# ut-amrl/nautilus

Measured on AMD Instinct MI355X. Metric: loop-closure candidate pairs/sec (1081-beam), higher is better.
Workload: dtype u16

## Files before the change

### include/nautilus_hip.h

```cpp
#ifndef NAUTILUS_HIP_H_
#define NAUTILUS_HIP_H_

#include <stddef.h>
#include <stdint.h>

#ifdef __cplusplus
extern "C" {
#endif

#define NHIP_OK 0
#define NHIP_ERR_ARG (-1)
#define NHIP_ERR_NODEV (-2)
#define NHIP_ERR_HIP (-3)
#define NHIP_ERR_ALLOC (-4)
#define NHIP_ERR_STATE (-5)

int nhip_init(int *n_devices);
int nhip_set_device(int device);
const char *nhip_last_error(void);
const char *nhip_version(void);
int nhip_dev_status(void *stream, int32_t info[4]);

typedef struct nhip_grid_spec {
  double range;
// ... 437 lines not shown
                      double max_range, int32_t min_separation, uint8_t *flags );
int nhip_lc_chi_square_gate(const double *poses, int32_t n_poses, const int32_t *pair_src, const int32_t *pair_tgt,
                            const float *cov , int32_t n_pairs, double max_score,
                            double *scores , uint8_t *flags );

int nhip_features_extract(const nhip_scans_t *scans, const nhip_feature_spec_t *spec, int32_t *planar_idx,
                          int32_t *planar_count, int32_t *edge_idx, int32_t *edge_count, double *scores);

int nhip_normals_estimate(const nhip_scans_t *scans, const nhip_normals_spec_t *spec, float *normals, int32_t *info);

int nhip_vectorize(const nhip_scans_t *scans, const double *poses, const nhip_vectorize_spec_t *spec, int32_t max_cells,
                   int32_t max_rounds, int32_t check_every, int64_t *records, int32_t *stats);

int nhip_occupancy(const nhip_scans_t *scans, const double *poses, const nhip_occupancy_spec_t *spec, int32_t *hits,
                   int32_t *misses, int8_t *grid, int64_t *stats);

int nhip_transient_filter(const nhip_scans_t *scans, const double *poses, const nhip_transient_spec_t *spec, const int32_t *hits,
                          const int32_t *misses, uint8_t *labels, float *out_xy, int32_t *out_offsets, int32_t *out_index,
                          int64_t *stats);

int nhip_map_windows(const int8_t *grid, const nhip_mapwin_spec_t *spec, const int32_t *origins, int32_t n_queries, float *out_xy,
                     int64_t capacity, int32_t *out_offsets, int64_t *stats);

int nhip_csm_freespace(const nhip_scans_t *scans, const nhip_grids_t *grids, const int32_t *pair_src, const int32_t *pair_slot,
                       const double *theta0, const int32_t *pair_origin, int32_t n_pairs, const nhip_search_t *search,
                       const nhip_match_t *matches, const nhip_freespace_spec_t *fs_spec, int32_t *counts);

int nhip_place_candidates(const nhip_scans_t *scans, const int32_t *ids, int32_t n_ids, const nhip_place_spec_t *spec,
                          int32_t *records, int64_t *stats, uint64_t *desc, int32_t *bits);

int nhip_place_seq_candidates(const nhip_scans_t *scans, const int32_t *ids, int32_t n_ids, const nhip_place_spec_t *spec,
                              const nhip_place_seq_spec_t *seq, int32_t *records, int64_t *stats);

int nhip_consistency(const double *records, int32_t M, const nhip_consistency_spec_t *spec, int32_t *members, int32_t *n_members,
                     int64_t *stats);

typedef struct nhip_csm_params {
  double scanner_range;
  double trans_range;
  double low_res;
  double high_res;
  double sigma;
  double floor_p;
  int32_t cell_bits;
  int32_t reserved;
} nhip_csm_params_t;
int nhip_csm_cache_configure(int64_t max_bytes);
int nhip_csm_cache_clear(void);
int nhip_csm_cache_stats(int64_t *entries, int64_t *bytes, int64_t *hits, int64_t *misses);
int nhip_csm_get_transformation(const nhip_csm_params_t *params, const float *pc_a, int32_t n_a, const float *pc_b,
                                int32_t n_b, double rot_a, double rot_b, double rot_restriction, double *score,
                                float *tx, float *ty, float *theta);

int nhip_resid_batch_create(int kind, const float *corr, const int32_t *block_offsets,
                            const int32_t *block_src, const int32_t *block_tgt, int32_t n_blocks,
                            int32_t n_poses, nhip_resid_batch_t **out);
int nhip_resid_batch_eval(nhip_resid_batch_t *batch, const double *poses, double *residuals,
                          double *jac_src, double *jac_tgt);
int nhip_resid_batch_eval_compact(nhip_resid_batch_t *batch, const double *poses, double *residuals,
                                  double *jac_src, double *jac_tgt_theta);
int nhip_resid_batch_eval_q(nhip_resid_batch_t *batch, const double *poses, double *residuals, double *q, double *block_consts);
int nhip_resid_jacobians_from_q(int kind, const float *corr, const double *q, const double *block_consts, int64_t n,
                                double *jac_src, double *jac_tgt);
int nhip_resid_batch_eval_block(nhip_resid_batch_t *batch, int32_t block, const double *source_pose,
                                const double *target_pose, double *residuals, double *jac_src, double *jac_tgt);
int nhip_resid_batch_free(nhip_resid_batch_t *batch);

int nhip_host_alloc(size_t bytes, void **out);
int nhip_host_free(void *p);

int nhip_resid_odometry(const float *t_odom, const float *r_odom, const int32_t *pose_i,
                        const int32_t *pose_j, int32_t n_factors, double translation_weight,
                        double rotation_weight, const double *poses, int32_t n_poses,
                        double *residuals, double *jac_i, double *jac_j);
int nhip_resid_point_to_line(const float *segments, const float *points, const int32_t *point_block,
                             int64_t n_points, const int32_t *block_pose, const int32_t *block_line,
                             int32_t n_blocks, const double *poses, int32_t n_poses,
                             const double *line_poses, int32_t n_line_poses, double *residuals,
                             double *jac_pose, double *jac_line);

int nhip_allgather_matches(void *comm, const nhip_match_t *d_local, int32_t n_local,
                           nhip_match_t *d_all, void *stream);

#ifdef __cplusplus
}
#endif
#endif
```

### nautilus_amd/_lib.py

```python
import ctypes as C
import os

_HERE = os.path.dirname(os.path.abspath(__file__))
LIB_PATH = os.environ.get("NHIP_LIB") or os.path.join(_HERE, "lib", "libnautilus_hip.so")

NHIP_OK, NHIP_ERR_ARG, NHIP_ERR_NODEV, NHIP_ERR_HIP, NHIP_ERR_ALLOC, NHIP_ERR_STATE = 0, -1, -2, -3, -4, -5
NHIP_LIDAR_NORMAL, NHIP_LIDAR_POINT = 0, 1
NHIP_SEARCH_EXHAUSTIVE, NHIP_SEARCH_DENSE, NHIP_SEARCH_SHORT_SCANS, NHIP_SEARCH_EXACT_SCORE, NHIP_SEARCH_LATENCY = 1, 2, 4, 8, 16
NHIP_SHORT_SCAN_POINTS = 1088
NHIP_FEATURE_MAX = 64
NHIP_NORMALS_MAX_BINS, NHIP_NORMALS_MAX_SAMPLES = 64, 128
NHIP_GRID_SKIP_MAP, NHIP_GRID_NO_IMAGE = 1, 2
NHIP_TIMER_CSM, NHIP_TIMER_GRID, NHIP_TIMER_RESID, NHIP_TIMER_CORR, NHIP_TIMER_NORMEQ, NHIP_TIMER_GRID_CLEAR = 0, 1, 2, 3, 4, 5
NHIP_TIMER_CSM_BOUNDS, NHIP_TIMER_CSM_CAND, NHIP_TIMER_EXACT_SCORE = 6, 7, 8
NHIP_TIMER_VEC_RASTER, NHIP_TIMER_VEC_VOTES, NHIP_TIMER_VEC_ROUNDS = 9, 10, 11
NHIP_TIMER_OCC_TRACE, NHIP_TIMER_OCC_CLASSIFY = 12, 13
NHIP_OCC_ACCUMULATE = 1
NHIP_PLACE_PAST_ONLY = 1
NHIP_PLACE_WORKSPACE_MAX = 64 << 20
NHIP_CONSISTENCY_STATE_BYTES = 8448
NHIP_LOSS_NONE, NHIP_LOSS_HUBER, NHIP_LOSS_SOFT_L1, NHIP_LOSS_CAUCHY = 0, 1, 2, 3


class NhipError(RuntimeError):
# ... 64 lines not shown
                ("reserved", C.c_int32)]


class MapwinSpec(C.Structure):
    _fields_ = [("res", C.c_double), ("cell_x0", C.c_int32), ("cell_y0", C.c_int32), ("width", C.c_int32), ("height", C.c_int32),
                ("side", C.c_int32), ("occ_min", C.c_int32), ("flags", C.c_int32), ("reserved", C.c_int32)]


class FreespaceSpec(C.Structure):
    _fields_ = [("hit_radius", C.c_int32), ("end_margin", C.c_int32), ("flags", C.c_int32), ("reserved", C.c_int32)]


class PlaceSpec(C.Structure):
    _fields_ = [("n_rings", C.c_int32), ("range_max", C.c_float), ("top_k", C.c_int32), ("min_separation", C.c_int32),
                ("max_permille", C.c_int32), ("flags", C.c_int32)]


class PlaceSeqSpec(C.Structure):
    _fields_ = [("half_window", C.c_int32), ("step", C.c_int32)]


class ConsistencySpec(C.Structure):
    _fields_ = [("t0", C.c_double), ("t_rate", C.c_double), ("t_max", C.c_double), ("r0", C.c_double), ("r_rate", C.c_double),
                ("r_max", C.c_double), ("max_steps", C.c_int32), ("flags", C.c_int32)]


class LossSpec(C.Structure):
    _fields_ = [("kind", C.c_int32), ("flags", C.c_int32), ("scale", C.c_double)]


class HitlSpec(C.Structure):
    _fields_ = [("line_a", C.c_float * 4), ("line_b", C.c_float * 4), ("line_width", C.c_double),
                ("point_threshold", C.c_int32), ("reserved", C.c_int32)]


class PcgStats(C.Structure):
    _fields_ = [("iterations", C.c_int32), ("flag", C.c_int32), ("relative_residual", C.c_double)]


class Match(C.Structure):
    _fields_ = [("itheta", C.c_int32), ("ix", C.c_int32), ("iy", C.c_int32), ("score", C.c_float)]


_vp, _i32, _i64, _f64 = C.c_void_p, C.c_int32, C.c_int64, C.c_double
_P = C.POINTER

PROTOTYPES = {
    "nhip_init": (C.c_int, [_P(C.c_int)]),
    "nhip_set_device": (C.c_int, [C.c_int]),
    "nhip_last_error": (C.c_char_p, []),
    "nhip_version": (C.c_char_p, []),
    "nhip_grid_layout": (C.c_int, [_P(GridSpec), _P(GridLayout)]),
    "nhip_grids_bytes": (_i64, [_P(GridSpec), _i64]),
    "nhip_grid_workspace_bytes": (_i64, [_P(GridSpec), _i32]),
    "nhip_grid_tables": (C.c_int, [_P(GridSpec), _vp, _vp]),
    "nhip_csm_rot0": (C.c_int, [_vp, _vp, _i32, _vp]),
    "nhip_csm_delta_table": (C.c_int, [_P(Search), _vp]),
    "nhip_match_to_transform": (C.c_int, [_P(Match), _P(GridSpec), _P(Search), _f64, _i32, _i32,
                                          _P(C.c_float), _P(C.c_float), _P(C.c_float)]),
    "nhip_score_from_sum": (_f64, [_P(GridSpec), _i64, _i32]),
    "nhip_csm_gate_floor": (C.c_int, [_P(GridSpec), _f64, _i32, _P(_i32)]),
    "nhip_dev_status": (C.c_int, [_vp, _P(_i32)]),
    "nhip_host_phases": (C.c_int, [_P(_f64)]),
    "nhip_device_pool_configure": (C.c_int, [_i64]),
    "nhip_device_pool_release": (C.c_int, []),
    "nhip_device_pool_stats": (C.c_int, [_P(_i64), _P(_i64)]),
    "nhip_grid_build_dev": (C.c_int, [_vp, _vp, _i32, _vp, _i32, _P(GridSpec), _vp, _vp, _i64, _vp]),
    "nhip_grid_rebuild_dev": (C.c_int, [_vp, _vp, _i32, _vp, _i32, _P(GridSpec), _vp, _vp, _i64, _vp]),
    "nhip_csm_match_dev": (C.c_int, [_vp, _vp, _i32, _vp, _i32, _P(GridSpec), _vp, _vp, _vp, _vp, _vp, _i32,
                                     _P(Search), _vp, _vp, _vp, _vp, _i64, _vp]),
    "nhip_csm_match_gated_dev": (C.c_int, [_vp, _vp, _i32, _vp, _i32, _P(GridSpec), _vp, _vp, _vp, _vp, _vp, _i32,
                                           _P(Search), _vp, _vp, _vp, _vp, _i64, _vp, _f64]),
    "nhip_submap_member_affines": (C.c_int, [_vp, _i32, _vp, _vp, _i32, _vp]),
    "nhip_submaps_gather_dev": (C.c_int, [_vp, _vp, _i32, _vp, _vp, _vp, _i32, _vp, _i64, _vp, _vp]),
    "nhip_grids_build_submaps": (C.c_int, [_vp, _vp, _vp, _vp, _i32, _P(GridSpec), _P(_vp)]),
    "nhip_csm_workspace_bytes": (_i64, [_i32]),
    "nhip_csm_last_launch": (C.c_int, [_P(_i32)]),
    "nhip_csm_get_transformation_info": (C.c_int, [_vp]),
    "nhip_bnb_stats": (C.c_int, [_P(C.c_uint64), _P(C.c_uint64)]),
    "nhip_bnb_stats_per_pair": (C.c_int, [_vp, _i32]),
    "nhip_bnb_timeline": (C.c_int, [_vp, _i32]),
    "nhip_bnb_timeline_candidates": (C.c_int, [_vp, _i32]),
    "nhip_bnb_stats_levels": (C.c_int, [_P(C.c_uint64)]),
    "nhip_csm_scores_dev": (C.c_int, [_vp, _vp, _i32, _vp, _i32, _P(GridSpec), _i32, _i32, _vp, _vp, _i32, _i32,
                                      _P(Search), _vp, _vp]),
    "nhip_resid_lidar_dev": (C.c_int, [C.c_int, _vp, _vp, _i64, _vp, _vp, _i32, _vp, _i32, _vp,
                                       _vp, _vp, _vp, _vp]),
    "nhip_resid_lidar_normal_eq_dev": (C.c_int, [C.c_int, _vp, _vp, _vp, _vp, _i32, _vp, _i32, _vp, _vp, _vp]),
    "nhip_pose_affines": (C.c_int, [_vp, _i32, _vp]),
    "nhip_corr_search_dev": (C.c_int, [_vp, _vp, _vp, _i32, _vp, _vp, _i32, _vp, C.c_float, _vp, _vp, _vp, _vp]),
    "nhip_corr_search_normals_dev": (C.c_int, [_vp, _vp, _vp, _i32, _vp, _vp, _i32, _vp, C.c_float, C.c_float, _vp, _vp, _vp,
                                               _vp]),
    "nhip_corr_compact_dev": (C.c_int, [_vp, _vp, _vp, _i32, _vp, _vp, _vp, _vp]),
    "nhip_resid_point_to_line_dev": (C.c_int, [_vp, _vp, _vp, _i64, _vp, _vp, _i32, _vp, _i32, _vp, _i32,
                                               _vp, _vp, _vp, _vp]),
    "nhip_resid_point_to_line_normal_eq_dev": (C.c_int, [_vp, _vp, _vp, _vp, _vp, _i32, _vp, _i32, _vp, _i32, _vp, _vp]),
    "nhip_resid_odometry_dev": (C.c_int, [_vp, _vp, _vp, _vp, _i32, _f64, _f64, _vp, _i32, _vp, _vp,
                                          _vp, _vp]),
    "nhip_resid_odometry_normal_eq_dev": (C.c_int, [_vp, _vp, _vp, _vp, _i32, _f64, _f64, _vp, _i32, _vp, _vp]),
    "nhip_resid_odometry_robust_normal_eq_dev": (C.c_int, [_vp, _vp, _vp, _vp, _i32, _f64, _f64, _P(LossSpec), _vp, _i32, _vp, _vp,
                                                           _vp]),
    "nhip_bsr_assemble_dev": (C.c_int, [_vp, _i32, _vp, _vp, _vp, _vp, _i32, _i32, _i32, _vp, _vp, _vp, _vp]),
    "nhip_bsr_pcg_workspace_bytes": (_i64, [_i32, _i32]),
    "nhip_bsr_pcg_dev": (C.c_int, [_vp, _vp, _vp, _vp, _vp, _i32, _i32, _f64, _f64, _f64, _i32, _i32, _vp, _vp, _i64,
                                   _P(PcgStats), _vp]),
    "nhip_bsr_pcg_columns_workspace_bytes": (_i64, [_i32, _i32, _i32]),
    "nhip_bsr_pcg_columns_dev": (C.c_int, [_vp, _vp, _vp, _vp, _i32, _i32, _vp, _vp, _i32, _f64, _f64, _i32, _i32, _vp, _vp, _i64,
                                           _P(PcgStats), _vp]),
    "nhip_scans_upload": (C.c_int, [_vp, _vp, _i32, _P(_vp)]),
    "nhip_scans_free": (C.c_int, [_vp]),
    "nhip_grids_build": (C.c_int, [_vp, _vp, _i32, _P(GridSpec), _P(_vp)]),
    "nhip_grids_free": (C.c_int, [_vp]),
    "nhip_grids_was_rebuilt": (C.c_int, [_vp]),
    "nhip_grids_download": (C.c_int, [_vp, _i32, _vp]),
    "nhip_grids_download_skip_map": (C.c_int, [_vp, _i32, _vp]),
    "nhip_grids_download_hi_plane": (C.c_int, [_vp, _i32, _vp]),
    "nhip_grids_download_hi_plane_copy": (C.c_int, [_vp, _i32, _i32, _vp]),
    "nhip_grids_download_tiled16": (C.c_int, [_vp, _i32, _vp]),
    "nhip_grids_download_pool": (C.c_int, [_vp, _i32, _vp]),
    "nhip_grids_download_pool4": (C.c_int, [_vp, _i32, _vp]),
    "nhip_grids_download_hits": (C.c_int, [_vp, _i32, _vp]),
    "nhip_csm_match": (C.c_int, [_vp, _vp, _vp, _vp, _vp, _vp, _i32, _P(Search), _vp, _vp]),
    "nhip_csm_match_gated": (C.c_int, [_vp, _vp, _vp, _vp, _vp, _vp, _i32, _P(Search), _vp, _vp, _f64]),
    "nhip_csm_scores": (C.c_int, [_vp, _vp, _i32, _i32, _f64, _i32, _i32, _P(Search), _vp]),
    "nhip_lc_scatter_scores_dev": (C.c_int, [_vp, _vp, _i32, _vp, _vp]),
    "nhip_lc_pair_gate_dev": (C.c_int, [_vp, _i32, _vp, _i32, _f64, _i32, _vp, _vp]),
    "nhip_lc_chi_square_gate_dev": (C.c_int, [_vp, _i32, _vp, _vp, _vp, _i32, _f64, _vp, _vp, _vp]),
    "nhip_feature_spec_default": (C.c_int, [_P(FeatureSpec)]),
    "nhip_features_extract_dev": (C.c_int, [_vp, _vp, _i32, _P(FeatureSpec), _vp, _vp, _vp, _vp, _vp, _vp]),
    "nhip_features_pack_dev": (C.c_int, [_vp, _vp, _vp, _i32, _vp, _vp, _i32, _vp, _vp, _vp, _vp]),
    "nhip_normals_spec_default": (C.c_int, [_P(NormalsSpec)]),
    "nhip_normals_estimate_dev": (C.c_int, [_vp, _vp, _i32, _P(NormalsSpec), _vp, _vp, _vp]),
    "nhip_normals_estimate": (C.c_int, [_vp, _P(NormalsSpec), _vp, _vp]),
    "nhip_vectorize_spec_default": (C.c_int, [_P(VectorizeSpec)]),
    "nhip_vectorize_tables": (C.c_int, [_P(VectorizeSpec), _vp, _vp]),
    "nhip_map_pose_affines": (C.c_int, [_vp, _i32, _vp]),
    "nhip_vectorize_workspace_bytes": (_i64, [_P(VectorizeSpec), _i32]),
    "nhip_vectorize_workspace_layout": (C.c_int, [_P(VectorizeSpec), _i32, _P(VectorizeLayout)]),
    "nhip_vectorize_dev": (C.c_int, [_vp, _vp, _vp, _i32, _P(VectorizeSpec), _i32, _i32, _i32, _vp, _vp, _vp, _i64, _vp]),
    "nhip_vectorize": (C.c_int, [_vp, _vp, _P(VectorizeSpec), _i32, _i32, _i32, _vp, _vp]),
    "nhip_vectorize_endpoints": (C.c_int, [_P(VectorizeSpec), _vp, _i32, _vp]),
    "nhip_occupancy_spec_default": (C.c_int, [_P(OccupancySpec)]),
    "nhip_occupancy_dev": (C.c_int, [_vp, _vp, _vp, _i32, _P(OccupancySpec), _vp, _vp, _vp, _vp, _vp]),
    "nhip_occupancy": (C.c_int, [_vp, _vp, _P(OccupancySpec), _vp, _vp, _vp, _vp]),
    "nhip_transient_spec_default": (C.c_int, [_P(TransientSpec)]),
    "nhip_transient_filter_dev": (C.c_int, [_vp, _vp, _i32, _i32, _vp, _P(TransientSpec), _vp, _vp, _vp, _vp, _vp, _vp, _vp, _vp]),
    "nhip_transient_filter": (C.c_int, [_vp, _vp, _P(TransientSpec), _vp, _vp, _vp, _vp, _vp, _vp, _vp]),
    "nhip_mapwin_spec_default": (C.c_int, [_P(MapwinSpec)]),
    "nhip_mapwin_origins": (C.c_int, [_vp, _i32, _f64, _vp, _vp]),
    "nhip_mapwin_workspace_bytes": (_i64, [_i32]),
    "nhip_mapwin_cells_dev": (C.c_int, [_vp, _P(MapwinSpec), _i32, _vp, _vp, _vp, _vp]),
    "nhip_mapwin_gather_dev": (C.c_int, [_vp, _vp, _P(MapwinSpec), _vp, _i32, _vp, _i64, _vp, _vp, _vp, _i64, _vp]),
    "nhip_map_windows": (C.c_int, [_vp, _P(MapwinSpec), _vp, _i32, _vp, _i64, _vp, _vp]),
    "nhip_freespace_spec_default": (C.c_int, [_P(FreespaceSpec)]),
    "nhip_freespace_planes_bytes": (_i64, [_P(GridSpec), _i64]),
    "nhip_freespace_trace_dev": (C.c_int, [_vp, _vp, _i32, _vp, _i32, _P(GridSpec), _vp, _vp, _vp]),
    "nhip_freespace_check_dev": (C.c_int, [_vp, _vp, _i32, _vp, _i32, _P(GridSpec), _vp, _vp, _vp, _vp, _vp, _i32, _P(Search),
                                           _vp, _vp, _P(FreespaceSpec), _vp, _vp]),
    "nhip_csm_freespace": (C.c_int, [_vp, _vp, _vp, _vp, _vp, _vp, _i32, _P(Search), _vp, _P(FreespaceSpec), _vp]),
    "nhip_place_spec_default": (C.c_int, [_P(PlaceSpec)]),
    "nhip_place_tables": (C.c_int, [_P(PlaceSpec), _vp, _vp]),
    "nhip_place_workspace_bytes": (_i64, [_P(PlaceSpec), _i32]),
    "nhip_place_describe_dev": (C.c_int, [_vp, _vp, _i32, _P(PlaceSpec), _vp, _vp, _vp]),
    "nhip_place_match_dev": (C.c_int, [_vp, _vp, _i32, _vp, _i32, _P(PlaceSpec), _vp, _vp, _vp, _i64, _vp]),
    "nhip_place_candidates": (C.c_int, [_vp, _vp, _i32, _P(PlaceSpec), _vp, _vp, _vp, _vp]),
    "nhip_place_seq_spec_default": (C.c_int, [_P(PlaceSeqSpec)]),
# ... 77 lines not shown
```

### nautilus_amd/csm.py

```python
import ctypes as C
import math

import numpy as np

from . import _lib
from ._lib import GridSpec, GridLayout, Search, Match, check, ptr

MATCH_DTYPE = np.dtype([("itheta", "<i4"), ("ix", "<i4"), ("iy", "<i4"), ("score", "<f4")])
assert MATCH_DTYPE.itemsize == C.sizeof(Match) == 16


def grid_spec(range_m=30.0, res=0.05, sigma=2.0, floor_p=1e-10, max_shift=40, cell_bits=16, skip_map=False, no_image=False):
    return GridSpec(float(range_m), float(res), float(sigma), float(floor_p), int(max_shift), int(cell_bits),
                    (_lib.NHIP_GRID_SKIP_MAP if skip_map else 0) | (_lib.NHIP_GRID_NO_IMAGE if no_image else 0), 0)


def search_spec(n_theta=61, nx=81, ny=81, theta_step=math.radians(1.0), exhaustive=False, dense=False, short_scans=False,
                exact_score=False, latency=False):
    flags = (_lib.NHIP_SEARCH_EXHAUSTIVE if exhaustive else 0) | (_lib.NHIP_SEARCH_DENSE if dense else 0) | \
            (_lib.NHIP_SEARCH_SHORT_SCANS if short_scans else 0) | (_lib.NHIP_SEARCH_EXACT_SCORE if exact_score else 0) | \
            (_lib.NHIP_SEARCH_LATENCY if latency else 0)
    return Search(int(n_theta), int(nx), int(ny), flags, float(theta_step))


# ... 118 lines not shown
            check(_lib.load().nhip_grids_download_pool4(self._h, int(slot), ptr(out)))
        return out

    def hits(self, slot):
        L = self.layout
        raw = np.empty(L.hits_bytes, dtype=np.uint8)
        check(_lib.load().nhip_grids_download_hits(self._h, int(slot), ptr(raw)))
        rows = raw[:L.hits_pitch * (L.side + 64)].reshape(L.side + 64, L.hits_pitch)
        bits = np.unpackbits(rows, axis=1, bitorder="little")
        return bits[32:32 + L.side, 32:32 + L.side]

    def interior(self, slot):
        L = self.layout
        return self.download(slot)[L.pad:L.pad + L.side, L.pad:L.pad + L.side]

    def close(self):
        if self._h:
            _lib.load().nhip_grids_free(self._h)
            self._h = C.c_void_p()

    __del__ = close


def submap_member_affines(poses, anchor_of_member, member_scan):
    P = np.ascontiguousarray(poses, dtype=np.float64).reshape(-1, 3)
    a = np.ascontiguousarray(anchor_of_member, dtype=np.int32)
    m = np.ascontiguousarray(member_scan, dtype=np.int32)
    if a.size != m.size:
        raise ValueError("submap_member_affines: one anchor per member")
    out = np.empty((m.size, 4), dtype=np.float32)
    check(_lib.load().nhip_submap_member_affines(ptr(P), len(P), ptr(a), ptr(m), m.size, ptr(out)))
    return out


def match_pairs(scans, grids, pair_src, pair_slot, theta0, search, pair_origin=None, min_score=None):
    pair_src = np.ascontiguousarray(pair_src, dtype=np.int32)
    pair_slot = np.ascontiguousarray(pair_slot, dtype=np.int32)
    theta0 = np.ascontiguousarray(theta0, dtype=np.float64)
    n = pair_src.size
    if pair_slot.size != n or theta0.size != n:
        raise ValueError("pair arrays differ in length")
    org = None
    if pair_origin is not None:
        org = np.ascontiguousarray(pair_origin, dtype=np.int32).reshape(n, 2)
    out = np.zeros(n, dtype=MATCH_DTYPE)
    sums = np.zeros(n, dtype=np.int32)
    if min_score is None:
        check(_lib.load().nhip_csm_match(scans._h, grids._h, ptr(pair_src), ptr(pair_slot), ptr(theta0),
                                         ptr(org), n, C.byref(search), ptr(out), ptr(sums)))
    else:
        check(_lib.load().nhip_csm_match_gated(scans._h, grids._h, ptr(pair_src), ptr(pair_slot), ptr(theta0),
                                               ptr(org), n, C.byref(search), ptr(out), ptr(sums), float(min_score)))
    return out, sums


def rejected(matches):
    return np.asarray(matches)["itheta"] < 0


def gate_floor(spec, min_score, n_points):
    out = C.c_int32(0)
    check(_lib.load().nhip_csm_gate_floor(C.byref(spec), float(min_score), int(n_points), C.byref(out)))
    return out.value


def bnb_stats():
    a, b = C.c_uint64(0), C.c_uint64(0)
    check(_lib.load().nhip_bnb_stats(C.byref(a), C.byref(b)))
    return a.value, b.value


def bnb_stats_levels():
    v = (C.c_uint64 * 24)()
    check(_lib.load().nhip_bnb_stats_levels(v))
    return {"blocks_whole": v[0], "blocks_total": v[1], "candidates_refined": v[2], "sub_blocks": v[3],
            "clk_wave_phase3": v[4], "clk_origins": v[5], "clk_sub_bounds": v[6], "clk_exact": v[7],
            "clk_slowest_wave": v[8], "clk_seeds": v[9], "clk_bounds": v[10], "clk_wave_phase3_100MHz": v[11],
            "pairs_handed_over": v[12], "clk_wave_second_kernel": v[13], "pose_evals16": v[14],
            "pairs_settled_by_gate": v[15], "passes_l2_runs": v[16], "passes_per_cell_field": v[17],
            "passes_per_cell_capacity": v[18], "edge_blocks_refined": v[19], "sub_blocks_without_pose": v[20],
            "edge_blocks_whole": v[21], "pair_passes": v[22], "pair_passes_across_blocks": v[23]}


def score_volume(scans, grids, src, slot, theta0, search, origin=(0, 0)):
    out = np.zeros((search.n_theta, search.nx, search.ny), dtype=np.int32)
    check(_lib.load().nhip_csm_scores(scans._h, grids._h, int(src), int(slot), float(theta0),
                                      int(origin[0]), int(origin[1]), C.byref(search), ptr(out)))
    return out


def match_to_transform(m, spec, search, theta0, origin=(0, 0)):
    tx = (origin[0] + int(m["ix"]) - (search.nx - 1) // 2) * spec.res
    ty = (origin[1] + int(m["iy"]) - (search.ny - 1) // 2) * spec.res
    th = theta0 + (int(m["itheta"]) - (search.n_theta - 1) // 2) * search.theta_step
    return np.float32(tx), np.float32(ty), np.float32(th)


class CorrelativeScanMatcher:

    def __init__(self, scanner_range, trans_range, low_res, high_res, sigma=2.0, cell_bits=16):
        self.params = _lib.CsmParams(float(scanner_range), float(trans_range), float(low_res), float(high_res),
                                     float(sigma), 1e-10, int(cell_bits), 0)

    def GetTransformation(self, pointcloud_a, pointcloud_b, rotation_a, rotation_b, rotation_restriction):
        a = np.ascontiguousarray(pointcloud_a, dtype=np.float32).reshape(-1, 2)
        b = np.ascontiguousarray(pointcloud_b, dtype=np.float32).reshape(-1, 2)
        score, tx, ty, th = C.c_double(0), C.c_float(0), C.c_float(0), C.c_float(0)
        check(_lib.load().nhip_csm_get_transformation(C.byref(self.params), ptr(a), len(a), ptr(b), len(b),
                                                      float(rotation_a), float(rotation_b), float(rotation_restriction),
                                                      C.byref(score), C.byref(tx), C.byref(ty), C.byref(th)))
        return score.value, ((np.float32(tx.value), np.float32(ty.value)), np.float32(th.value))


def last_launch():
    out = (C.c_int32 * 8)()
    check(_lib.load().nhip_csm_last_launch(out))
    form = {0: "fused", 1: "split, one round", 2: "split, rounds on one stream", 3: "split, rounds overlapped on the helper stream"}
    return {"form": form.get(out[0], "?"), "form_id": out[0], "pairs_per_round": out[1], "rounds_of_state": out[2],
            "rounds": out[3], "short_scans": bool(out[4]), "hand_over_kernel": bool(out[5]), "instrumented": bool(out[6] & 1),
            "l2_runs": bool(out[6] & 2), "pair_subs": bool(out[6] & 4), "n_pairs": out[7]}


def drop_in_cache_stats():
    v = [C.c_int64(0) for _ in range(4)]
    check(_lib.load().nhip_csm_cache_stats(*[C.byref(x) for x in v]))
    return dict(zip(("entries", "bytes", "hits", "misses"), (x.value for x in v)))


def drop_in_cache_clear():
    check(_lib.load().nhip_csm_cache_clear())


def drop_in_cache_configure(max_bytes):
    check(_lib.load().nhip_csm_cache_configure(int(max_bytes)))
```

### nautilus_amd/csrc/nhip_bnb.hip

```cpp
#include <atomic>
#include <mutex>
#include <type_traits>
#include <vector>

#ifndef NHIP_BNB_INSTR
#define NHIP_BNB_INSTR 0
#endif
#if NHIP_BNB_INSTR
#define csm_bnb_kernel csm_bnb_kernel_instr
#define csm_bnb_rot_kernel csm_bnb_rot_kernel_instr
#define launchers_product launchers_instr
#define BNB_STATS(P) ((P).stats)
#define BNB_TIMELINE(P) ((P).timeline)
#else
#define BNB_STATS(P) (static_cast<unsigned long long *>(nullptr))
#define BNB_TIMELINE(P) (static_cast<unsigned long long *>(nullptr))
#endif

#include "nhip_bnb_params.h"
#include "nhip_bnb_wave.h"
#include "nhip_bnb_origin.h"
#include "nhip_bnb_bounds.h"
#include "nhip_bnb_exact.h"

namespace nhip {

namespace {

using namespace bnb;

constexpr int BNB_THREADS = 64 * BNB_WAVES;

constexpr int N_WORK = 9;
struct PairCtx {
  const uint8_t *grid;
  const float2 *pts;
  int32_t n_pts, cx, cy, pair;
};

template <int CB>
__device__ __forceinline__ void process_candidate(const BnbParams &P, const PairCtx &C, int32_t k, int32_t v, int lane,
                                                  unsigned long long *best, uint32_t (&n)[N_WORK]) {
  const int Y = v / NB, X = v - NB * Y;
  const int32_t vx = block_extent(P.nx, X), vy = block_extent(P.ny, Y);
  const bool edge = vx < BNB_B || vy < BNB_B;
  float cf, sf;
  rotation_k(P, C.pair, k, &cf, &sf);
  if (P.levels >= 2) {
    const __amdgpu_buffer_rsrc_t p4 = uniform_rsrc(C.grid + P.grid_bytes + P.skip_bytes + P.pool_bytes, P.pool4_bytes);
    uint32_t sb[4];
    sub_bounds(P, p4, C.pts, C.n_pts, cf, sf, C.cx, C.cy, Y, X, lane, CB == 1 ? 1u : 257u, sb);
    n[1]++;
    n[4] += edge ? 1u : 0u;
    const uint32_t bsum = best_sum<false>(best);
    int alive = 0;
#pragma unroll
    for (int q = 0; q < 4; q++) alive += (sub_valid(vy, vx, q >> 1, q & 1) && sb[q] != 0u && sb[q] >= bsum) ? 1 : 0;
    if (alive == 0) return;
    if (alive <= 2) {
      const __amdgpu_buffer_rsrc_t rsrc = uniform_rsrc(C.grid, P.grid_bytes + P.skip_bytes);
#pragma unroll 1
      for (int q = 0; q < 4; q++) {
        const uint32_t b = q == 0 ? sb[0] : (q == 1 ? sb[1] : (q == 2 ? sb[2] : sb[3]));
        if (!sub_valid(vy, vx, q >> 1, q & 1) || b == 0u || b < best_sum<false>(best)) continue;
        const unsigned long long key = eval_sub<CB>(P, rsrc, C.pts, C.n_pts, cf, sf, C.cx, C.cy, k, Y, X, q >> 1, q & 1, lane);
        wave_atomic_max(best, key, lane);
        n[2]++;
        n[5] += sub_valid(vy, vx, q >> 1, q & 1) ? 0u : 1u;
      }
      return;
    }
  }
  const unsigned long long key = eval_block<CB>(P, C.grid, C.pts, C.n_pts, cf, sf, C.cx, C.cy, k, Y, X, lane);
  wave_atomic_max(best, key, lane);
  n[0]++;
  n[6] += edge ? 1u : 0u;
}

template <int CB, bool GLOBAL, bool PAIR>
__device__ __forceinline__ void process_candidate_c(const BnbParams &P, __amdgpu_buffer_rsrc_t rsrc, uint32_t pitch8,
                                                    __amdgpu_buffer_rsrc_t rsrc16, const uint32_t *org, int32_t nch,
                                                    int32_t n_pts, int32_t k, int32_t Y, int32_t X,
                                                    uint32_t sb0, uint32_t sb1, uint32_t sb2, uint32_t sb3, int lane,
                                                    unsigned long long *best, uint32_t &bcopy, uint32_t (&n)[N_WORK],
                                                    int t, uint32_t &mk0, uint32_t &mk1) {
  const uint32_t bsum = best_sum_cached<GLOBAL>(best, bcopy);
  const int32_t vx = block_extent(P.nx, X), vy = block_extent(P.ny, Y);
  const bool edge = vx < BNB_B || vy < BNB_B;
  n[4] += edge ? 1u : 0u;
  const bool ok0 = sub_valid(vy, vx, 0, 0), ok1 = sub_valid(vy, vx, 0, 1), ok2 = sub_valid(vy, vx, 1, 0), ok3 = sub_valid(vy, vx, 1, 1);
  const int alive = (ok0 && sb0 != 0u && sb0 >= bsum) + (ok1 && sb1 != 0u && sb1 >= bsum) + (ok2 && sb2 != 0u && sb2 >= bsum) +
                    (ok3 && sb3 != 0u && sb3 >= bsum);
  if (alive == 0) return;
  constexpr int WHOLE_MIN = 3;
  if (alive >= WHOLE_MIN) {
    int dy, dx;
    const uint32_t total = block_sums8(rsrc, pitch8, (uint32_t)P.hi_copy_bytes, org, nch, Y, X, lane, &dy, &dx);
    const int32_t ix = BNB_B * X + dx, iy = BNB_B * Y + dy;
    if (CB == 1) {
      const unsigned long long key = best_key(P, k, ix, iy, total, 32);
      wave_atomic_max(best, key, lane);
      if (GLOBAL) bcopy = max(bcopy, (uint32_t)(key >> 32));
    } else {
      n[3] += refine16<GLOBAL>(P, rsrc16, org, nch, n_pts, k, ix, iy, total, true, lane, best, bcopy);
    }
    n[0]++;
    n[6] += __ballot(ix < P.nx && iy < P.ny) != ~0ull ? 1u : 0u;
    return;
  }
  if (!PAIR) {
#pragma unroll 1
    for (int q = 0; q < 4; q++) {
      const uint32_t b = q == 0 ? sb0 : (q == 1 ? sb1 : (q == 2 ? sb2 : sb3));
      if (!sub_valid(vy, vx, q >> 1, q & 1) || b == 0u || b < best_sum_cached<GLOBAL>(best, bcopy)) continue;
      int dy, dx;
      const uint32_t total = sub_sums8(rsrc, pitch8, (uint32_t)P.hi_copy_bytes, org, nch, Y, X, q >> 1, q & 1, lane, &dy, &dx);
      const int32_t ix = BNB_B * X + BNB_B4 * (q & 1) + dx, iy = BNB_B * Y + BNB_B4 * (q >> 1) + dy;
      if (CB == 1) {
        const unsigned long long key = best_key(P, k, ix, iy, total, 8);
        wave_atomic_max(best, key, lane);
        if (GLOBAL) bcopy = max(bcopy, (uint32_t)(key >> 32));
      } else {
        n[3] += refine16<GLOBAL>(P, rsrc16, org, nch, n_pts, k, ix, iy, total, lane < 16, lane, best, bcopy);
      }
      n[2]++;
      n[5] += __ballot(ix < P.nx && iy < P.ny) == 0ull ? 1u : 0u;
    }
    return;
  }
  mk0 |= (uint32_t)((ok0 && sb0 != 0u && sb0 >= bsum) | ((ok1 && sb1 != 0u && sb1 >= bsum) << 1)) << (2 * t);
  mk1 |= (uint32_t)((ok2 && sb2 != 0u && sb2 >= bsum) | ((ok3 && sb3 != 0u && sb3 >= bsum) << 1)) << (2 * t);
}

#ifndef NHIP_BNB_PAIR_CROSS
#define NHIP_BNB_PAIR_CROSS 0
#endif
constexpr bool PAIR_CROSS = NHIP_BNB_PAIR_CROSS != 0;
__device__ __forceinline__ uint32_t pick6(const uint32_t (&r)[6], int c) {
  return c == 0 ? r[0] : (c == 1 ? r[1] : (c == 2 ? r[2] : (c == 3 ? r[3] : (c == 4 ? r[4] : r[5]))));
}
template <int CB, bool GLOBAL>
__device__ __forceinline__ void strip_sub_blocks(const BnbParams &P, __amdgpu_buffer_rsrc_t rsrc, uint32_t pitch8,
                                                 __amdgpu_buffer_rsrc_t rsrc16, const uint32_t *org, int32_t nch, int32_t n_pts,
                                                 int32_t k, int32_t Y, int32_t X0, const uint32_t (&sb)[12], uint32_t mk0,
                                                 uint32_t mk1, int lane, unsigned long long *best, uint32_t &bcopy,
                                                 uint32_t (&n)[N_WORK]) {
#pragma unroll 1
  for (int sy = 0; sy < 2; sy++) {
    uint32_t mk = sy ? mk1 : mk0;
    if (mk == 0u) continue;
    uint32_t row[6];
#pragma unroll
    for (int c = 0; c < 6; c++) row[c] = sy ? sb[4 * (c >> 1) + 2 + (c & 1)] : sb[4 * (c >> 1) + (c & 1)];
#pragma unroll 1
    while (mk != 0u) {
      const int c = (int)__builtin_ctz(mk);
      mk &= mk - 1u;
      const uint32_t bsum = best_sum_cached<GLOBAL>(best, bcopy);
      if (pick6(row, c) < bsum) continue;
      const int32_t X = X0 + (c >> 1), sx = c & 1;
      const bool two = P.pair_subs != 0 && ((mk >> (c + 1)) & 1u) != 0u && (PAIR_CROSS || sx == 0) && pick6(row, c + 1) >= bsum;
      int dy, dx;
      uint32_t total;
      if (two) {
        mk &= ~(1u << (c + 1));
        total = pair_sums8(rsrc, pitch8, (uint32_t)P.hi_copy_bytes, org, nch, Y, X, sy, sx, lane, &dy, &dx);
      } else {
        total = sub_sums8(rsrc, pitch8, (uint32_t)P.hi_copy_bytes, org, nch, Y, X, sy, sx, lane, &dy, &dx);
      }
      const int32_t ix = BNB_B * X + BNB_B4 * sx + dx, iy = BNB_B * Y + BNB_B4 * sy + dy;
      if (CB == 1) {
        const unsigned long long key = best_key(P, k, ix, iy, total, 16);
        wave_atomic_max(best, key, lane);
        if (GLOBAL) bcopy = max(bcopy, (uint32_t)(key >> 32));
      } else {
        n[3] += refine16<GLOBAL>(P, rsrc16, org, nch, n_pts, k, ix, iy, total, lane < (two ? 32 : 16), lane, best, bcopy);
      }
      const bool pose = ix < P.nx && iy < P.ny;
      if (two) {
        n[2] += 2u;
        n[5] += (__ballot(pose && dx < BNB_B4) == 0ull ? 1u : 0u) + (__ballot(pose && dx >= BNB_B4) == 0ull ? 1u : 0u);
        n[7]++;
        n[8] += (uint32_t)sx;
      } else {
        n[2]++;
        n[5] += __ballot(pose) == 0ull ? 1u : 0u;
      }
    }
  }
}

struct PhaseClocks {
  long long org, strip, eval;
  uint32_t run_passes, cell_passes_field, cell_passes_full;
};

__device__ __forceinline__ void flush_stats(unsigned long long *stats, const uint32_t *n, int32_t pair, const PhaseClocks *clk,
                                            const uint32_t *edge = nullptr) {
  if (n) {
    if (n[0]) atomicAdd(&stats[0], (unsigned long long)n[0]);
    if (n[1]) atomicAdd(&stats[2], (unsigned long long)n[1]);
    if (n[2]) atomicAdd(&stats[3], (unsigned long long)n[2]);
    if (n[3]) atomicAdd(&stats[14], (unsigned long long)n[3]);
    if (pair < BNB_STATS_PAIRS) atomicAdd(&stats[BNB_STATS_HEAD + pair], 4ull * n[0] + n[2]);
  }
  if (edge) {
    if (edge[0]) atomicAdd(&stats[19], (unsigned long long)edge[0]);
    if (edge[1]) atomicAdd(&stats[20], (unsigned long long)edge[1]);
    if (edge[2]) atomicAdd(&stats[21], (unsigned long long)edge[2]);
    if (edge[3]) atomicAdd(&stats[22], (unsigned long long)edge[3]);
    if (edge[4]) atomicAdd(&stats[23], (unsigned long long)edge[4]);
  }
  if (clk) {
    atomicAdd(&stats[5], (unsigned long long)clk->org);
    atomicAdd(&stats[6], (unsigned long long)clk->strip);
    atomicAdd(&stats[7], (unsigned long long)clk->eval);
    if (clk->run_passes) atomicAdd(&stats[16], (unsigned long long)clk->run_passes);
    if (clk->cell_passes_field) atomicAdd(&stats[17], (unsigned long long)clk->cell_passes_field);
    if (clk->cell_passes_full) atomicAdd(&stats[18], (unsigned long long)clk->cell_passes_full);
  }
}

template <int CB, bool GLOBAL, bool PAIR, bool RUNS = false>
__device__ __forceinline__ void rotation_pass(const BnbParams &P, const PairCtx &C, int32_t k, uint32_t u0, uint32_t u1,
                                              unsigned long long m0, unsigned long long m1, int lane,
                                              unsigned long long *best, uint32_t *done, uint32_t *org,
                                              uint32_t (&n_work)[N_WORK], PhaseClocks &clk, uint32_t *runs = nullptr) {
  long long t_mark = 0;
  float cf, sf;
  rotation_k(P, C.pair, k, &cf, &sf);
  if (BNB_STATS(P)) t_mark = clock64();
  int32_t nrc = RUNS_NONE;
  const int32_t nch = cache_origins<RUNS>(P, C.pts, C.n_pts, cf, sf, C.cx, C.cy, lane, org, true, runs, RUNS && P.l2_runs != 0, &nrc);
  if (BNB_STATS(P)) clk.org += clock64() - t_mark;
  if (RUNS && BNB_STATS(P)) {
    clk.run_passes += nrc > 0 ? 1u : 0u;
    clk.cell_passes_field += nrc == RUNS_FIELD ? 1u : 0u;
    clk.cell_passes_full += nrc == RUNS_FULL ? 1u : 0u;
  }
  const __amdgpu_buffer_rsrc_t rsrc16 = CB == 1 ? uniform_rsrc(C.grid, P.grid_bytes + P.skip_bytes)
                                                : uniform_rsrc(C.grid + P.hi_offset + 2 * P.hi_copy_bytes, P.t16_bytes);
  const __amdgpu_buffer_rsrc_t rsrc = uniform_rsrc(C.grid + P.hi_offset, 2 * P.hi_copy_bytes);
  const uint32_t pitch8 = (uint32_t)P.hi_tpr;
  const __amdgpu_buffer_rsrc_t p4 = uniform_rsrc(C.grid + P.grid_bytes + P.skip_bytes + P.pool_bytes, P.pool4_bytes);
  while ((m0 | m1) != 0ull) {
    const int b0 = m0 ? (int)__builtin_ctzll(m0) : 64 + (int)__builtin_ctzll(m1);
    const int Y = b0 / NB, X0 = b0 - NB * Y;
    int len = 1;
    while (len < 3 && X0 + len < NB) {
      const int b = b0 + len;
      if (!(((b < 64 ? m0 >> b : m1 >> (b - 64)) & 1ull))) break;
      len++;
    }
    uint32_t sb[12];
    uint32_t bcopy = GLOBAL ? best_sum<true>(best) : 0u;
    if (P.levels >= 2) {
      if (BNB_STATS(P)) t_mark = clock64();
      if (RUNS && nrc > 0) strip_bounds_c<RunList<RUN_CHUNKS>>(P, p4, runs + lane, nrc, Y, X0, len, CB == 1 ? 1u : 257u, sb);
      else strip_bounds_c<CellList>(P, p4, org, nch, Y, X0, len, CB == 1 ? 1u : 257u, sb);
      if (BNB_STATS(P)) clk.strip += clock64() - t_mark;
      n_work[1] += (uint32_t)len;
    } else {
#pragma unroll
      for (int q = 0; q < 12; q++) sb[q] = 0xffffffffu;
    }
    uint32_t mk0 = 0u, mk1 = 0u;
#pragma unroll 1
    for (int t = 0; t < len; t++) {
      const int b = b0 + t;
      if (b < 64) m0 &= ~(1ull << b);
      else m1 &= ~(1ull << (b - 64));
      const uint32_t ub = (uint32_t)__builtin_amdgcn_readlane((int)(b < 64 ? u0 : u1), b & 63);
      if (ub < best_sum_cached<GLOBAL>(best, bcopy)) continue;
      const uint32_t s0 = t == 0 ? sb[0] : (t == 1 ? sb[4] : sb[8]), s1 = t == 0 ? sb[1] : (t == 1 ? sb[5] : sb[9]);
      const uint32_t s2 = t == 0 ? sb[2] : (t == 1 ? sb[6] : sb[10]), s3 = t == 0 ? sb[3] : (t == 1 ? sb[7] : sb[11]);
      if (BNB_STATS(P)) t_mark = clock64();
      process_candidate_c<CB, GLOBAL, PAIR>(P, rsrc, pitch8, rsrc16, org, nch, C.n_pts, k, Y, X0 + t, s0, s1, s2, s3, lane, best,
                                      bcopy, n_work, t, mk0, mk1);
      if (BNB_STATS(P)) clk.eval += clock64() - t_mark;
      if (done && wave_leader(lane)) done[b] = 0u;
    }
    if (PAIR && (mk0 | mk1) != 0u) {
      if (BNB_STATS(P)) t_mark = clock64();
      strip_sub_blocks<CB, GLOBAL>(P, rsrc, pitch8, rsrc16, org, nch, C.n_pts, k, Y, X0, sb, mk0, mk1, lane, best, bcopy, n_work);
      if (BNB_STATS(P)) clk.eval += clock64() - t_mark;
    }
  }
}

__device__ __forceinline__ void read_entry(const RotEntry *ent, int32_t *pair, int32_t *k, unsigned long long *m0,
                                           unsigned long long *m1) {
  const unsigned long long w0 = ent->w[0], w1 = ent->w[1], w2 = ent->w[2], w3 = ent->w[3];
  *pair = (int32_t)(w0 >> 24);
  *k = (int32_t)(w0 & 0xffffffull);
  *m0 = w1 | (w2 << 41);
  *m1 = (w2 >> 23) | (w3 << 18);
}

__device__ __forceinline__ void pair_context(const BnbParams &P, int32_t pair, PairCtx *C) {
  const int32_t src = P.pair_src[pair], slot = P.pair_slot[pair];
  const int32_t beg = P.offsets[src];
  C->grid = P.grids + (size_t)slot * P.slot_bytes;
  C->pts = P.xy + beg;
  C->n_pts = P.offsets[src + 1] - beg;
  C->cx = P.pair_origin ? P.pair_origin[2 * pair] : 0;
  C->cy = P.pair_origin ? P.pair_origin[2 * pair + 1] : 0;
  C->pair = pair;
}

template <int CB, bool POOL_LDS, bool BY_ROT, bool SPLIT = false>
__global__ __launch_bounds__(SPLIT ? 64 * SPLIT_WAVES : BNB_THREADS, SPLIT ? SPLIT_WAVES / 2 : 4) void csm_bnb_kernel(BnbParams P) {
  constexpr int WAVES = SPLIT ? SPLIT_WAVES : BNB_WAVES, THREADS = 64 * WAVES;
  constexpr int QSPACE = lds_qspace(SPLIT);
  extern __shared__ __align__(16) uint8_t smem[];
  uint8_t *s_pool = smem;
  uint32_t *s_org = reinterpret_cast<uint32_t *>(smem);
  uint32_t *s_U = reinterpret_cast<uint32_t *>(smem + P.lds_first);
  unsigned long long *s_queue = reinterpret_cast<unsigned long long *>(s_U + (size_t)P.n_theta * 128);
  LdsTail *s_tail = reinterpret_cast<LdsTail *>(s_queue + QSPACE);
  unsigned long long *s_best = &s_tail->best, *s_slow = &s_tail->slow;
  uint32_t *s_cnt = s_tail->cnt, *s_qn = s_cnt + LDS_QN, *s_qhead = s_cnt + LDS_QHEAD, *s_top = &s_tail->top;
  uint32_t *s_list = reinterpret_cast<uint32_t *>(s_queue);
  static_assert(BNB_WAVES * LIST_ENTRIES * 4 <= QCAP * 4, "the run lists fit the first half of the queue");
  unsigned long long *s_kmax = s_queue + (SPLIT ? WAVES * LIST_ENTRIES / 2 : QCAP / 2);
  uint32_t *s_order = reinterpret_cast<uint32_t *>(s_kmax + MAX_ROT);
  static_assert(SPLIT_WAVES * LIST_ENTRIES * 4 + MAX_ROT * 12 <= QSPACE_SPLIT * 8 && MAX_ROT * 12 <= QCAP * 4, "lists, maxima and order fit");

  const uint32_t bid = blockIdx.x;
  const int32_t pair = (int32_t)((bid & 7u) * (uint32_t)P.pairs_per_xcd + (bid >> 3));
  if ((int32_t)(bid >> 3) >= P.pairs_per_xcd || pair >= P.n_pairs) return;
  const int lane = threadIdx.x & 63, wave = threadIdx.x >> 6;

  int32_t src = P.pair_src[pair], slot = P.pair_slot[pair];
  const bool ids_ok = pair_ids_ok(P.ids, src, slot, pair + P.pair_base, threadIdx.x == 0);
  if (!ids_ok) src = slot = 0;
  const int32_t beg = ids_ok ? P.offsets[src] : 0, n_pts = ids_ok ? P.offsets[src + 1] - beg : 0;
  const float2 *pts = P.xy + beg;
  const uint8_t *grid = P.grids + (size_t)slot * P.slot_bytes;
  const int32_t cx = P.pair_origin ? P.pair_origin[2 * pair] : 0;
  const int32_t cy = P.pair_origin ? P.pair_origin[2 * pair + 1] : 0;
  const bool centre_ok = (abs(cx) + P.hx <= P.max_shift) && (abs(cy) + P.hy <= P.max_shift);
  if (BY_ROT != (n_pts <= 64 * OCL && (uint32_t)P.rows < ORG_LIMIT && !P.general_all)) return;

  const int32_t gfloor = gate_floor(P.gate, n_pts);
  const unsigned long long fkey = gate_floor_key(gfloor);
  unsigned long long *const stats_g = NHIP_BNB_INSTR ? P.stats : nullptr;
  const long long t_start = BNB_STATS(P) ? clock64() : 0;
  if (BNB_TIMELINE(P) && threadIdx.x == 0 && pair < BNB_STATS_PAIRS) BNB_TIMELINE(P)[4 * pair] = wall_clock64();
  if (threadIdx.x == 0) {
    *s_slow = 0ull;
    *s_best = fkey;
    s_cnt[0] = s_cnt[3] = s_cnt[4] = s_cnt[5] = 0u;
    s_top[0] = 0u;
    *s_qn = 0u;
    *s_qhead = 0u;
  }
  if (!centre_ok || n_pts <= 0) {
    if (threadIdx.x == 0) P.keys[pair] = fkey;
    return;
  }
  const RotationTerms terms = rotation_terms_of_wave<WAVES>(P, pair, wave, lane);
  if (POOL_LDS) {
    const uint4 *gp = reinterpret_cast<const uint4 *>(grid + P.grid_bytes + P.skip_bytes);
    uint4 *sp = reinterpret_cast<uint4 *>(s_pool);
    const int32_t n16 = (int32_t)(P.pool_bytes / 16);
    for (int32_t i = threadIdx.x; i < n16; i += 4 * THREADS) {
      uint4 v[4];
// ... 187 lines not shown
      const int32_t k = (int32_t)((uint32_t)wbest >> 8), v = (int32_t)(wbest & 0xffu);
      const int Y = v / NB, X = v - NB * Y;
      float cf, sf;
      rotation_k(P, pair, k, &cf, &sf);
      const unsigned long long key = eval_block<CB>(P, grid, pts, n_pts, cf, sf, cx, cy, k, Y, X, lane);
      if (wave_leader(lane)) {
        atomicMax(s_best, key);
        s_U[k * 128 + v] = 0u;
      }
      n_work[0]++;
    }
    __syncthreads();
    for (int32_t k = wave; k < P.n_theta; k += BNB_WAVES) {
  #pragma unroll
      for (int i = 0; i < 2; i++) {
        const uint32_t u = s_U[k * 128 + lane + 64 * i];
        const uint32_t bsum = (uint32_t)(*(volatile unsigned long long *)s_best >> 32);
        bool cand = u != 0u && u >= bsum;
        const unsigned long long m = __ballot(cand);
        if (m == 0ull) continue;
        const uint32_t base = wave_fetch_add(s_qn, (uint32_t)__builtin_popcountll(m), lane);
        const uint32_t pos = base + (uint32_t)__builtin_popcountll(m & ((1ull << lane) - 1ull));
        const unsigned long long entry = ((unsigned long long)u << 32) | (uint32_t)((k << 8) | (lane + 64 * i));
        if (cand && pos < (uint32_t)QCAP) s_queue[pos] = entry;
        unsigned long long over = __ballot(cand && pos >= (uint32_t)QCAP);
        while (over) {
          const int j = (int)__builtin_ctzll(over);
          over &= over - 1ull;
          const uint32_t lo = (uint32_t)__builtin_amdgcn_readlane((int)(uint32_t)entry, j);
          const uint32_t hi = (uint32_t)__builtin_amdgcn_readlane((int)(uint32_t)(entry >> 32), j);
          if (hi >= best_sum<false>(s_best))
            process_candidate<CB>(P, C, (int32_t)(lo >> 8), (int32_t)(lo & 0xffu), lane, s_best, n_work);
        }
      }
    }
    __syncthreads();
    {
      const uint32_t qn = min(*s_qn, (uint32_t)QCAP);
      for (;;) {
        const uint32_t i = wave_fetch_add(s_qhead, 1u, lane);
        if (i >= qn) break;
        const unsigned long long entry = s_queue[i];
        if ((uint32_t)(entry >> 32) >= best_sum<false>(s_best))
          process_candidate<CB>(P, C, (int32_t)((uint32_t)entry >> 8), (int32_t)(entry & 0xffu), lane, s_best, n_work);
      }
    }
}
  if (stats_g && lane == 0) {
    atomicAdd(&s_cnt[0], n_work[0]);
    atomicAdd(&s_cnt[3], n_work[1]);
    atomicAdd(&s_cnt[4], n_work[2]);
    atomicAdd(&s_cnt[5], n_work[3]);
    flush_stats(stats_g, nullptr, pair, nullptr, n_work + 4);
  }
  __syncthreads();
  if (threadIdx.x == 0) {
    P.keys[pair] = *s_best;
    if (BNB_TIMELINE(P) && pair < BNB_STATS_PAIRS) {
      uint32_t hw;
      asm volatile("s_getreg_b32 %0, hwreg(HW_REG_HW_ID)" : "=s"(hw));
      uint32_t xcc;
      asm volatile("s_getreg_b32 %0, hwreg(HW_REG_XCC_ID)" : "=s"(xcc));
      BNB_TIMELINE(P)[4 * pair + 3] = (wall_clock64() & 0xfffffffffffull) | ((unsigned long long)((hw >> 8) & 0xffu) << 44) |
                                      ((unsigned long long)(xcc & 0xfu) << 52);
    }
    if (BNB_STATS(P) && BY_ROT) atomicAdd(&BNB_STATS(P)[8], *s_slow);
    if (stats_g) {
      const uint32_t n_all[4] = {s_cnt[0], s_cnt[3], s_cnt[4], s_cnt[5]};
      flush_stats(stats_g, n_all, pair, nullptr);
      atomicAdd(&stats_g[1], (unsigned long long)(P.n_theta * P.nbx * P.nby));
    }
  }
}

template <int CB>
__global__ __launch_bounds__(256, CB == 2 && !NHIP_BNB_INSTR ? 5 : 4) void csm_bnb_rot_kernel(BnbParams P) {
  const int lane = threadIdx.x & 63;
  const uint32_t xcd = blockIdx.x & 7u;
  const uint32_t filled = P.rot_count[8 * xcd];
  const uint32_t count = filled < P.rot_cap ? filled : P.rot_cap;
  const RotEntry *list = P.rot_list + (size_t)xcd * P.rot_cap;
  __shared__ uint32_t s_org2[4 * ORG_WAVE];
  __shared__ uint32_t s_run2[4 * RUN_WAVE];
  uint32_t *org = s_org2 + (threadIdx.x >> 6) * ORG_WAVE + lane;
  uint32_t *runs = s_run2 + (threadIdx.x >> 6) * RUN_WAVE;
  PhaseClocks clk = {0, 0, 0, 0u, 0u, 0u};
  const long long t0 = BNB_STATS(P) ? clock64() : 0;
  for (;;) {
    const uint32_t i = wave_fetch_add(P.rot_count + 8 * xcd + 1, 1u, lane);
    if (i >= count) break;
    int32_t pair, k;
    unsigned long long m0, m1;
    read_entry(list + i, &pair, &k, &m0, &m1);
    PairCtx C;
    pair_context(P, pair, &C);
    uint32_t n[N_WORK] = {};
    rotation_pass<CB, true, true, true>(P, C, k, 0xffffffffu, 0xffffffffu, m0, m1, lane, &P.keys[pair], nullptr, org, n, clk, runs);
    if (BNB_STATS(P) && lane == 0) flush_stats(BNB_STATS(P), n, pair, nullptr, n + 4);
  }
  if (BNB_STATS(P) && lane == 0) {
    atomicAdd(&BNB_STATS(P)[13], (unsigned long long)(clock64() - t0));
    flush_stats(BNB_STATS(P), nullptr, 0, &clk);
  }
}

constexpr int SORT_THREADS = 1024;
constexpr int SORT_BUCKETS = 16 * 21;
__device__ __forceinline__ int cand_bucket(uint32_t c) {
  if (c == 0u) return SORT_BUCKETS - 1;
  const int e = 31 - __builtin_clz(c);
  const int f = e >= 4 ? (int)((c >> (e - 4)) & 15u) : (int)((c << (4 - e)) & 15u);
  const int b = 16 * e + f;
  return b >= SORT_BUCKETS - 1 ? 0 : SORT_BUCKETS - 2 - b;
}
__device__ __forceinline__ uint32_t cand_shares(const BnbParams &P, uint32_t c) {
  const uint32_t w = 1u + c / P.split_min;
  return w < P.split_max ? w : P.split_max;
}

__global__ __launch_bounds__(SORT_THREADS) void csm_bnb_order_kernel(BnbParams P) {
  __shared__ uint32_t s_extra[SORT_BUCKETS];
  __shared__ uint32_t s_wave[SORT_THREADS / 64];
  __shared__ uint32_t s_base, s_idle;
  __shared__ int s_grant;
  const int32_t xcd = blockIdx.x;
  const int32_t lo = xcd * P.pairs_per_xcd, hi = min(lo + P.pairs_per_xcd, P.n_pairs);
  int32_t *work = P.ps_work + (size_t)xcd * P.ps_work_stride;
  for (int i = threadIdx.x; i < SORT_BUCKETS; i += SORT_THREADS) s_extra[i] = 0u;
  for (int i = threadIdx.x; i < P.ps_work_stride; i += SORT_THREADS) work[i] = -1;
  if (threadIdx.x == 0) s_base = s_idle = 0u;
  __syncthreads();
  for (int32_t p = lo + (int32_t)threadIdx.x; p < hi; p += SORT_THREADS) {
    const uint32_t c = P.ps_count[p];
    atomicAdd(&s_extra[cand_bucket(c)], cand_shares(P, c) - 1u);
  }
  __syncthreads();
  if (threadIdx.x == 0) {
    uint32_t room = (uint32_t)P.ps_work_stride - (uint32_t)(hi > lo ? hi - lo : 0);
    int grant = 0;
    while (grant < SORT_BUCKETS && s_extra[grant] <= room) room -= s_extra[grant++];
    s_grant = grant;
  }
  __syncthreads();
  const int lane = threadIdx.x & 63, wv = threadIdx.x >> 6;
  for (int pass = P.front_min ? 0 : 1; pass < 2; pass++)
  for (int32_t p0 = lo; p0 < hi; p0 += SORT_THREADS) {
    const int32_t p = p0 + (int32_t)threadIdx.x;
    const uint32_t c = p < hi ? P.ps_count[p] : 0u;
    const bool mine = P.front_min == 0u || ((c >= P.front_min) == (pass == 0));
    const uint32_t w = (c != 0u && mine) ? (cand_bucket(c) < s_grant ? cand_shares(P, c) : 1u) : 0u;
    if (p < hi && mine) P.ps_nw[p] = c != 0u ? w : 1u;
    uint32_t v = w;
#pragma unroll
    for (int off = 1; off < 64; off <<= 1) {
      const uint32_t u = (uint32_t)__shfl_up((int)v, off, 64);
      if (lane >= off) v += u;
    }
    if (lane == 63) s_wave[wv] = v;
    __syncthreads();
    uint32_t before = s_base;
    for (int q = 0; q < wv; q++) before += s_wave[q];
    const uint32_t at = before + v - w;
    for (uint32_t j = 0; j < w; j++) work[at + j] = p;
    __syncthreads();
    if (threadIdx.x == SORT_THREADS - 1) s_base = before + v;
    __syncthreads();
  }
  const uint32_t tail0 = s_base;
  for (int32_t p = lo + (int32_t)threadIdx.x; p < hi; p += SORT_THREADS)
    if (P.ps_count[p] == 0u) work[tail0 + atomicAdd(&s_idle, 1u)] = p;
}

constexpr int ORDER_THREADS = 256;
__global__ __launch_bounds__(ORDER_THREADS) void csm_bnb_order_spread_kernel(BnbParams P) {
  const int32_t p = (int32_t)(blockIdx.x * ORDER_THREADS + threadIdx.x);
  if (p >= P.n_pairs) return;
  const int32_t extra_slots = P.ps_work_stride - P.pairs_per_xcd;
  const int32_t home = p / P.pairs_per_xcd;
  P.ps_work[(size_t)home * P.ps_work_stride + extra_slots + (p - home * P.pairs_per_xcd)] = p;
  const uint32_t want = cand_shares(P, P.ps_count[p]) - 1u;
  uint32_t got = 0u;
  if (want) {
    const uint32_t t0 = atomicAdd(P.ps_ticket, want);
    for (uint32_t j = 0; j < want; j++) {
      const uint32_t e = t0 + j;
      if ((int32_t)(e >> 3) >= extra_slots) break;
      P.ps_work[(size_t)((e + (uint32_t)home + 1u) & 7u) * P.ps_work_stride + (e >> 3)] = p;
      got++;
    }
  }
  P.ps_nw[p] = 1u + got;
}

constexpr int CAND_WAVES = 4;
constexpr int CAND_THREADS = 64 * CAND_WAVES;
template <int CB>
__global__ __launch_bounds__(CAND_THREADS, CB == 2 ? 5 : 4) void csm_bnb_cand_kernel(BnbParams P) {
  __shared__ uint32_t s_org2[CAND_WAVES * ORG_WAVE];
  __shared__ uint32_t s_run2[CAND_WAVES * RUN_WAVE];
  __shared__ unsigned long long s_best2;
  __shared__ uint32_t s_next2;
  const int lane = threadIdx.x & 63;
  const uint32_t xcd = blockIdx.x & 7u, slot = blockIdx.x >> 3;
  if ((int32_t)slot >= P.ps_work_stride) return;
  const int32_t pair = P.ps_work[(size_t)xcd * P.ps_work_stride + slot];
  if (pair < 0) return;
  const uint32_t live = P.ps_live[pair];
  if (live == 0u) return;
  const bool shared = P.ps_nw[pair] > 1u;
  if (BNB_TIMELINE(P) && threadIdx.x == 0 && pair < BNB_STATS_PAIRS)
    atomicMin(&BNB_TIMELINE(P)[4 * (size_t)BNB_STATS_PAIRS + 2 + pair], wall_clock64());
  if (threadIdx.x == 0) {
    s_best2 = P.keys[pair];
    s_next2 = 0u;
  }
  __syncthreads();
  unsigned long long *best = shared ? &P.keys[pair] : &s_best2;
  uint32_t *next = shared ? &P.ps_next[pair] : &s_next2;
  const uint32_t *rows = P.ps_rows + (size_t)pair * (size_t)P.n_theta * 128u;
  uint32_t *org = s_org2 + (threadIdx.x >> 6) * ORG_WAVE + lane;
  uint32_t *runs = s_run2 + (threadIdx.x >> 6) * RUN_WAVE;
  PairCtx C;
  pair_context(P, pair, &C);
  uint32_t n_work[N_WORK] = {};
  PhaseClocks clk = {0, 0, 0, 0u, 0u, 0u};
  const long long t0 = BNB_STATS(P) ? clock64() : 0;
  for (;;) {
    const uint32_t rank = wave_fetch_add(next, 1u, lane);
    if (rank >= live) break;
    const uint32_t u0 = rows[(size_t)rank * 128u + lane], u1 = rows[(size_t)rank * 128u + 64 + lane];
    const uint32_t kmax = (uint32_t)__builtin_amdgcn_readlane((int)u1, 62);
    const int32_t k = __builtin_amdgcn_readlane((int)u1, 63);
    const uint32_t bsum = best_sum<true>(best);
    if (kmax < bsum) break;
    const unsigned long long m0 = __ballot(u0 != 0u && u0 >= bsum);
    const unsigned long long m1 = __ballot(u1 != 0u && u1 >= bsum && lane + 64 < NB * NB);
    if ((m0 | m1) == 0ull) continue;
    rotation_pass<CB, true, true, true>(P, C, k, u0, u1, m0, m1, lane, best, nullptr, org, n_work, clk, runs);
  }
  if (BNB_STATS(P) && lane == 0) {
    atomicAdd(&BNB_STATS(P)[13], (unsigned long long)(clock64() - t0));
    flush_stats(BNB_STATS(P), n_work, pair, &clk, n_work + 4);
  }
  if (BNB_TIMELINE(P) && lane == 0 && pair < BNB_STATS_PAIRS)
    atomicMax(&BNB_TIMELINE(P)[5 * (size_t)BNB_STATS_PAIRS + 2 + pair], wall_clock64());
  if (!shared) {
    __syncthreads();
    if (threadIdx.x == 0) P.keys[pair] = s_best2;
  }
}

}

namespace bnb {

namespace {
template <int CB, bool PL, bool BR, bool SP = false>
int launch_main(const BnbParams &P, const BnbPlan &plan, hipStream_t s) {
  constexpr int THREADS = SP ? 64 * SPLIT_WAVES : BNB_THREADS;
  const size_t lds = lds_bytes((size_t)plan.lds_first, P.n_theta, SP);
  const int64_t blocks = (int64_t)P.pairs_per_xcd * 8;
  constexpr int MAX_DEV = 64;
  static std::atomic<size_t> lds_set[MAX_DEV];
  int dev = 0;
  if (hipGetDevice(&dev) != hipSuccess || dev < 0 || dev >= MAX_DEV) dev = -1;
  if (dev < 0 || lds > lds_set[dev].load(std::memory_order_relaxed)) {
    NHIP_TRY_HIP(hipFuncSetAttribute(reinterpret_cast<const void *>(csm_bnb_kernel<CB, PL, BR, SP>),
                                     hipFuncAttributeMaxDynamicSharedMemorySize, (int)lds));
    if (dev >= 0) lds_set[dev].store(lds, std::memory_order_relaxed);
  }
  hipLaunchKernelGGL((csm_bnb_kernel<CB, PL, BR, SP>), dim3((uint32_t)blocks), dim3(THREADS), lds, s, P);
  return NHIP_OK;
}

template <int CB, bool PL>
int launch_split_a(const BnbParams &P, const BnbPlan &plan, hipStream_t s) {
  int rc = launch_main<CB, PL, true, true>(P, plan, s);
  if (rc) return rc;
  if (!P.short_scans && (rc = launch_main<CB, PL, false>(P, plan, s))) return rc;
  if (P.ps_ticket)
    hipLaunchKernelGGL(csm_bnb_order_spread_kernel, dim3((uint32_t)((P.n_pairs + ORDER_THREADS - 1) / ORDER_THREADS)), dim3(ORDER_THREADS), 0, s, P);
  else
    hipLaunchKernelGGL(csm_bnb_order_kernel, dim3(8), dim3(SORT_THREADS), 0, s, P);
  return NHIP_OK;
}

template <int CB, bool PL>
int launch_both(const BnbParams &P, const BnbPlan &plan, hipStream_t s) {
  if (!P.general_all) {
    int rc = launch_main<CB, PL, true>(P, plan, s);
    if (rc) return rc;
    if (P.short_scans) return NHIP_OK;
  }
  return launch_main<CB, PL, false>(P, plan, s);
}

template <class F>
int with_instantiation(const BnbPlan &plan, F f) {
  using CB1 = std::integral_constant<int, 1>;
  using CB2 = std::integral_constant<int, 2>;
  if (plan.cb == 1) return plan.pool_lds ? f(CB1{}, std::true_type{}) : f(CB1{}, std::false_type{});
  return plan.pool_lds ? f(CB2{}, std::true_type{}) : f(CB2{}, std::false_type{});
}

int launch_fused(const BnbParams &P, const BnbPlan &plan, hipStream_t s) {
  return with_instantiation(plan, [&](auto cb, auto pl) {
    const int rc = launch_both<decltype(cb)::value, decltype(pl)::value>(P, plan, s);
    if (rc) return rc;
    if (plan.second) {
      const uint32_t rot_blocks = 256 * 4;
      hipLaunchKernelGGL(csm_bnb_rot_kernel<decltype(cb)::value>, dim3(rot_blocks), dim3(256), 0, s, P);
    }
    return NHIP_OK;
  });
}

int launch_split_bounds(const BnbParams &P, const BnbPlan &plan, hipStream_t s) {
  return with_instantiation(plan, [&](auto cb, auto pl) { return launch_split_a<decltype(cb)::value, decltype(pl)::value>(P, plan, s); });
}

int launch_split_cands(const BnbParams &P, const BnbPlan &plan, hipStream_t s) {
  return with_instantiation(plan, [&](auto cb, auto) {
    hipLaunchKernelGGL(csm_bnb_cand_kernel<decltype(cb)::value>, dim3((uint32_t)(8 * P.ps_work_stride)), dim3(CAND_THREADS), 0, s, P);
    return NHIP_OK;
  });
// ... 10 lines not shown
```

### nautilus_amd/csrc/nhip_bnb_bounds.h

```cpp
#pragma once
#include <type_traits>

#include "nhip_bnb_origin.h"

namespace nhip {
namespace {

constexpr uint32_t LANE_WEIGHT = 64u;

struct PointSlots {
  float2 q0, q1;
};
__device__ __forceinline__ void prime_slots(const float2 *pts, int32_t n_pts, int lane, PointSlots &S) {
  S.q0 = S.q1 = make_float2(0.f, 0.f);
  if (n_pts > 0) {
    const int32_t last = n_pts - 1;
    S.q0 = pts[min(lane, last)];
    __builtin_amdgcn_sched_barrier(0);
    S.q1 = pts[min(64 + lane, last)];
  }
}

template <bool POOL_LDS>
__device__ __forceinline__ void coarse_rotation(const BnbParams &P, const uint8_t *pool, __amdgpu_buffer_rsrc_t prs,
// ... 145 lines not shown
      {
        float2 pt = S.q1;
        asm volatile("" : "+v"(pt.x), "+v"(pt.y));
        S.q1 = pts[min(cn + 64 + lane, last)];
        if (c + 64 < n_pts) feed(offsets(pt, c + 64), c + 64, true);
      }
    }
  }
  feed(zero_a, 0, false);
}

__device__ __forceinline__ bool slot_block(int v, int *Y, int *X) {
  const int lane = v & 63, i = v >> 6;
  const int r = 32 * i + 16 * ((lane >> 5) & 1) + 8 * ((lane >> 4) & 1) + 4 * ((lane >> 3) & 1) + 2 * ((lane >> 1) & 1) + (lane & 1);
  const int f = (lane >> 2) & 1;
  if (r >= 60) {
    *Y = 10;
    *X = r == 63 ? 1 + 2 * f : 4 * (r - 60) + 2 * f;
    return true;
  }
  const int y = r / 6, d = r % 6;
  if (d == 5 && f == 1) {
    *Y = 10;
    *X = 5 + 2 * y;
    return y < 3;
  }
  *Y = y;
  *X = d < 3 ? 4 * d + 2 * f : 4 * (d - 3) + 1 + 2 * f;
  return true;
}

__device__ __forceinline__ void sub_bounds(const BnbParams &P, __amdgpu_buffer_rsrc_t p4, const float2 *pts, int32_t n_pts,
                                           float cf, float sf, int32_t cx, int32_t cy, int32_t Y, int32_t X, int lane,
                                           uint32_t scale, uint32_t (&out)[4]) {
  const int32_t DP = P.pool4_pitch;
  uint32_t A[4] = {0u, 0u, 0u, 0u};
  constexpr int U = 4;
  for (int32_t c = 0; c < n_pts; c += 64 * U) {
    uint32_t a[U];
    u32x2 w[U];
#pragma unroll
    for (int u = 0; u < U; u++) {
      const int32_t idx = c + 64 * u + lane;
      a[u] = 0u;
      if (idx < n_pts) {
        int32_t prow, pcol;
        window_origin(pts[idx], cf, sf, P, cx, cy, &prow, &pcol);
        a[u] = (uint32_t)(((prow >> 2) + 2 * Y) * DP + 2 * ((pcol >> 2) + 2 * X));
      }
      w[u] = __builtin_amdgcn_raw_buffer_load_b64(p4, (int)(a[u] & ~3u), 0, 0);
    }
#pragma unroll
    for (int u = 0; u < U; u++) {
      const uint32_t n = idx_guard(c + 64 * u + lane < n_pts, __builtin_amdgcn_alignbit(w[u].y, w[u].x, (a[u] & 2u) * 8u));
      A[0] += n & 0xffu;
      A[2] += (n >> 8) & 0xffu;
      A[1] += (n >> 16) & 0xffu;
      A[3] += n >> 24;
    }
  }
#pragma unroll
  for (int m = 1; m < 64; m <<= 1) {
#pragma unroll
    for (int q = 0; q < 4; q++) A[q] += shfl_xor_u32(A[q], m);
  }
#pragma unroll
  for (int q = 0; q < 4; q++) out[q] = A[q] * scale;
}

struct CellList {
  static constexpr int ROUNDS = 2, H = OC / ROUNDS;
  static __device__ __forceinline__ uint32_t entry(const uint32_t *list, int c) { return origin_of(list, c); }
  static __device__ __forceinline__ uint32_t offset(uint32_t o, uint32_t DP) { return (org_row(o) >> 2) * DP + 2u * (org_col(o) >> 2); }
  static __device__ __forceinline__ uint32_t count(uint32_t o) { return org_cnt(o); }
};
template <int CHUNKS>
struct RunList {
  static constexpr int ROUNDS = 1, H = CHUNKS;
  static __device__ __forceinline__ uint32_t entry(const uint32_t *list, int c) { return list[64 * c]; }
  static __device__ __forceinline__ uint32_t offset(uint32_t e, uint32_t DP) { return run_row2(e) * DP + 2u * run_col2(e); }
  static __device__ __forceinline__ uint32_t count(uint32_t e) { return run_cnt(e); }
};

template <class LIST>
__device__ __forceinline__ void strip_sums(const BnbParams &P, __amdgpu_buffer_rsrc_t p4, const uint32_t *list, int32_t nch,
                                           int32_t Y, int32_t X0, int len, uint32_t (&E)[3], uint32_t (&O)[3]) {
  const uint32_t DP = (uint32_t)P.pool4_pitch;
  const uint32_t off = (uint32_t)(2 * Y) * DP + (uint32_t)(4 * X0);
  constexpr int ROUNDS = LIST::ROUNDS, H = LIST::H;
#pragma unroll
  for (int h = 0; h < ROUNDS; h++) {
    if (H * h >= nch) continue;
    u32x4 w[H];
    uint32_t sh[H], cn[H];
    uint32_t aa[H];
#pragma unroll
    for (int j = 0; j < H; j++) {
      const uint32_t o = LIST::entry(list, H * h + j);
      const uint32_t a = LIST::offset(o, DP) + off;
      sh[j] = (a & 2u) * 8u;
      aa[j] = a & ~3u;
      cn[j] = LIST::count(o);
    }
    if (len == 1) {
#pragma unroll
      for (int j = 0; j < H; j++) {
        const u32x2 v = __builtin_amdgcn_raw_buffer_load_b64(p4, (int)aa[j], 0, 0);
        w[j].x = v.x; w[j].y = v.y; w[j].z = 0u; w[j].w = 0u;
      }
    } else if (len == 2) {
#pragma unroll
      for (int j = 0; j < H; j++) {
        const u32x3 v = __builtin_amdgcn_raw_buffer_load_b96(p4, (int)aa[j], 0, 0);
        w[j].x = v.x; w[j].y = v.y; w[j].z = v.z; w[j].w = 0u;
      }
    } else {
#pragma unroll
      for (int j = 0; j < H; j++) w[j] = __builtin_amdgcn_raw_buffer_load_b128(p4, (int)aa[j], 0, 0);
    }
#pragma unroll
    for (int j = 0; j < H; j++) {
      const uint32_t n0 = __builtin_amdgcn_alignbit(w[j].y, w[j].x, sh[j]);
      const uint32_t n1 = __builtin_amdgcn_alignbit(w[j].z, w[j].y, sh[j]);
      const uint32_t n2 = __builtin_amdgcn_alignbit(w[j].w, w[j].z, sh[j]);
      E[0] += __umul24(n0 & M8, cn[j]); O[0] += __umul24((n0 >> 8) & M8, cn[j]);
      E[1] += __umul24(n1 & M8, cn[j]); O[1] += __umul24((n1 >> 8) & M8, cn[j]);
      E[2] += __umul24(n2 & M8, cn[j]); O[2] += __umul24((n2 >> 8) & M8, cn[j]);
    }
  }
}

template <class LIST>
__device__ __forceinline__ void strip_bounds_c(const BnbParams &P, __amdgpu_buffer_rsrc_t p4, const uint32_t *list,
                                               int32_t nch, int32_t Y, int32_t X0, int len, uint32_t scale,
                                               uint32_t (&out)[12]) {
  uint32_t E[3] = {0u, 0u, 0u}, O[3] = {0u, 0u, 0u};
  if (std::is_same<LIST, CellList>::value) {
    strip_sums<CellList>(P, p4, list, nch, Y, X0, len, E, O);
  } else {
    static_assert(RUN_CHUNKS == 8, "the rounds below cover the run list");
    if (nch <= 4) strip_sums<RunList<4>>(P, p4, list, nch, Y, X0, len, E, O);
    else if (nch == 5) strip_sums<RunList<5>>(P, p4, list, nch, Y, X0, len, E, O);
    else if (nch == 6) strip_sums<RunList<6>>(P, p4, list, nch, Y, X0, len, E, O);
    else strip_sums<RunList<8>>(P, p4, list, nch, Y, X0, len, E, O);
  }
#pragma unroll
  for (int t = 0; t < 3; t++) {
    E[t] = sum8(E[t]);
    O[t] = sum8(O[t]);
  }
#pragma unroll
  for (int t = 0; t < 3; t++) {
    out[4 * t + 0] = E[t] & 0xffffu;
    out[4 * t + 1] = E[t] >> 16;
    out[4 * t + 2] = O[t] & 0xffffu;
    out[4 * t + 3] = O[t] >> 16;
  }
#pragma unroll
  for (int q = 0; q < 12; q++) out[q] = wave_total_of8(out[q]) * scale;
}

}
}
```

### nautilus_amd/csrc/nhip_bnb_exact.h

```cpp
#pragma once
#include "nhip_bnb_origin.h"

namespace nhip {
namespace {

constexpr int SEG_CHUNKS = 32;
constexpr int EVAL_CHUNKS = 2;

template <bool GLOBAL>
__device__ __forceinline__ uint32_t best_sum(unsigned long long *best) {
  unsigned long long b;
  if (GLOBAL) b = __hip_atomic_load(best, __ATOMIC_RELAXED, __HIP_MEMORY_SCOPE_AGENT);
  else b = *(volatile unsigned long long *)best;
  return (uint32_t)__builtin_amdgcn_readfirstlane((int)(uint32_t)(b >> 32));
}
template <bool GLOBAL>
__device__ __forceinline__ uint32_t best_sum_cached(unsigned long long *best, uint32_t copy) {
  return GLOBAL ? copy : best_sum<false>(best);
}

__device__ __forceinline__ unsigned long long best_key(const BnbParams &P, int32_t k, int32_t ix, int32_t iy, uint32_t total,
                                                       int top) {
  unsigned long long key = 0ull;
  if (ix < P.nx && iy < P.ny) {
// ... 347 lines not shown
          const uint32_t n1 = __builtin_amdgcn_alignbit(w[j][y].z, w[j][y].y, sh[j]);
          E[y0 + y][0] += __umul24(n0 & M8, cn[j]); O[y0 + y][0] += __umul24(n0 >> 8, cn[j]);
          E[y0 + y][1] += __umul24(n1 & M8, cn[j]); O[y0 + y][1] += __umul24(n1 >> 8, cn[j]);
        }
    }
  }
  uint32_t R[32];
#pragma unroll
  for (int y = 0; y < 8; y++) {
    R[4 * y + 0] = E[y][0];
    R[4 * y + 1] = O[y][0] - ((E[y][0] >> 16) << 8);
    R[4 * y + 2] = E[y][1];
    R[4 * y + 3] = O[y][1] - ((E[y][1] >> 16) << 8);
  }
  rs_step<32, 1>(R, lane & 1);
  rs_step<16, 2>(R, lane & 2);
  rs_step<8, 4>(R, lane & 4);
  uint32_t V[8];
#pragma unroll
  for (int i = 0; i < 4; i++) {
    V[2 * i] = R[i] & 0xffffu;
    V[2 * i + 1] = R[i] >> 16;
  }
  rs_step<8, 8>(V, lane & 8);
  rs_step<4, 16>(V, lane & 16);
  rs_step<2, 32>(V, lane & 32);
  const int r = 8 * (2 * ((lane >> 5) & 1) + ((lane >> 4) & 1)) + 4 * ((lane >> 2) & 1) + 2 * ((lane >> 1) & 1) + (lane & 1);
  const int f = (lane >> 3) & 1, d = r & 3;
  *dy = r >> 2;
  *dx = 4 * (d >> 1) + (d & 1) + 2 * f;
  return V[0];
}

__device__ __forceinline__ uint32_t pair_sums8(__amdgpu_buffer_rsrc_t rsrc, uint32_t pitch, uint32_t copy_bytes, const uint32_t *org,
                                               int32_t nch, int32_t Y, int32_t X, int32_t sy, int32_t sx0, int lane, int *dy, int *dx) {
  const uint32_t roff = (uint32_t)(BNB_B * Y + BNB_B4 * sy), coff = (uint32_t)(BNB_B * X + BNB_B4 * sx0);
  const uint32_t wrap = pitch * HI_TILE_BYTES - HI_TILE_BYTES;
  static_assert(257u * 255u <= 0xffffu, "a packed field holds the byte sums of the 8 lanes it is reduced over");
  uint32_t E[4][2], O[4][2];
#pragma unroll
  for (int y = 0; y < 4; y++) E[y][0] = E[y][1] = O[y][0] = O[y][1] = 0u;
#pragma unroll
  for (int r = 0; r < OC; r++) {
    if (r >= nch) continue;
    const uint32_t o = origin_of(org, r);
    const uint32_t cn = org_cnt(o);
    const uint32_t row0 = org_row(o) + roff, col0 = org_col(o) + coff, col4 = col0 & ~3u;
    const uint32_t q = row0 & 7u, sh = (col0 & 3u) * 8u;
    const uint32_t g = hi_tiled(row0, col4, (col4 >> 3) & 1u, pitch, copy_bytes);
    u32x3 w[4];
#pragma unroll
    for (int y = 0; y < 4; y++)
      w[y] = __builtin_amdgcn_raw_buffer_load_b96(rsrc, (int)(g + (q + (uint32_t)y >= 8u ? wrap : 0u) + 16u * (uint32_t)y), 0, 0);
#pragma unroll
    for (int y = 0; y < 4; y++) {
      const uint32_t n0 = __builtin_amdgcn_alignbit(w[y].y, w[y].x, sh);
      const uint32_t n1 = __builtin_amdgcn_alignbit(w[y].z, w[y].y, sh);
      E[y][0] += __umul24(n0 & M8, cn); O[y][0] += __umul24(n0 >> 8, cn);
      E[y][1] += __umul24(n1 & M8, cn); O[y][1] += __umul24(n1 >> 8, cn);
    }
  }
  uint32_t R[16];
#pragma unroll
  for (int y = 0; y < 4; y++) {
    R[4 * y + 0] = E[y][0];
    R[4 * y + 1] = O[y][0] - ((E[y][0] >> 16) << 8);
    R[4 * y + 2] = E[y][1];
    R[4 * y + 3] = O[y][1] - ((E[y][1] >> 16) << 8);
  }
  rs_step<16, 1>(R, lane & 1);
  rs_step<8, 2>(R, lane & 2);
  rs_step<4, 4>(R, lane & 4);
  uint32_t V[4] = {R[0] & 0xffffu, R[0] >> 16, R[1] & 0xffffu, R[1] >> 16};
  rs_step<4, 8>(V, lane & 8);
  rs_step<2, 16>(V, lane & 16);
  V[0] = add_xor<32>(V[0]);
  const int r = 8 * ((lane >> 4) & 1) + 4 * ((lane >> 2) & 1) + 2 * ((lane >> 1) & 1) + (lane & 1);
  const int f = (lane >> 3) & 1, d = r & 3;
  *dy = r >> 2;
  *dx = 4 * (d >> 1) + (d & 1) + 2 * f;
  return V[0];
}

__device__ __forceinline__ uint32_t pose_sum16(const BnbParams &P, __amdgpu_buffer_rsrc_t rsrc16, const uint32_t *org,
                                               int32_t nch, int32_t ix, int32_t iy) {
  uint32_t acc = 0u;
#pragma unroll
  for (int c = 0; c < OCL; c++) {
    if (c >= nch) continue;
    const uint32_t o = origin_of(org, c);
    acc += org_cnt(o) * (uint32_t)__builtin_amdgcn_raw_buffer_load_b16(
                            rsrc16, (int)t16_tiled(org_row(o) + (uint32_t)iy, org_col(o) + (uint32_t)ix, (uint32_t)P.t16_tpr), 0, 0);
  }
  return wave_sum(acc);
}

template <bool GLOBAL>
__device__ __forceinline__ uint32_t refine16(const BnbParams &P, __amdgpu_buffer_rsrc_t rsrc16, const uint32_t *org,
                                             int32_t nch, int32_t n_pts, int32_t k, int32_t ix, int32_t iy, uint32_t hsum,
                                             bool mine, int lane, unsigned long long *best, uint32_t &bcopy) {
  const bool valid = mine && ix < P.nx && iy < P.ny;
  uint32_t ub = valid ? 256u * hsum + 255u * (uint32_t)n_pts : 0u;
  uint32_t n_eval = 0u;
  for (;;) {
    const uint32_t top = (uint32_t)__builtin_amdgcn_readfirstlane((int)wave_max(ub));
    if (top == 0u || top < best_sum_cached<GLOBAL>(best, bcopy)) break;
    const int j = (int)__builtin_ctzll(__ballot(ub == top));
    const int32_t jx = __builtin_amdgcn_readlane(ix, j), jy = __builtin_amdgcn_readlane(iy, j);
    const uint32_t sum = pose_sum16(P, rsrc16, org, nch, jx, jy);
    const uint32_t lin = (uint32_t)((k * P.nx + jx) * P.ny + jy);
    const unsigned long long key = ((unsigned long long)sum << 32) | (0xffffffffu - lin);
    wave_atomic_max(best, key, lane);
    if (GLOBAL) bcopy = max(bcopy, sum);
    if (lane == j) ub = 0u;
    n_eval++;
  }
  return n_eval;
}

}
}
```

### nautilus_amd/csrc/nhip_bnb_host.hip

```cpp
#include <atomic>
#include <memory>
#include <mutex>
#include <vector>

#include "nhip_bnb_params.h"

namespace nhip {

using namespace bnb;

namespace {

size_t bnb_lds_first(const GridLayout &L, bool pool_lds) {
  const size_t pool = pool_lds ? (size_t)L.pool_bytes : 0;
  return pool > (size_t)ORG_LDS ? pool : (size_t)ORG_LDS;
}
size_t bnb_lds_bytes(const GridLayout &L, const nhip_search_t *search, bool pool_lds) {
  return lds_bytes(bnb_lds_first(L, pool_lds), search->n_theta, false);
}
constexpr size_t LDS_MAX = 160 * 1024;

struct TimerScope {
  int id;
  hipStream_t s;
  TimerScope(int i, hipStream_t st) : id(i), s(st) { timer_begin(id, s); }
  ~TimerScope() { timer_end(id, s); }
};
}

bool bnb_fits(const GridLayout &L, const nhip_search_t *search) {
  const int nbx = (search->nx + BNB_B - 1) / BNB_B, nby = (search->ny + BNB_B - 1) / BNB_B;
  return nbx <= NB && nby <= NB && bnb_lds_bytes(L, search, false) <= LDS_MAX && L.pool_bytes % 16 == 0 &&
         L.pool_bytes < (1ll << RUN_SHIFT) && L.S + 2 * L.pad < 65536 && search->n_theta <= MAX_ROT;
}

static std::mutex g_instr_mu;
static unsigned long long *g_bnb_timeline = nullptr;
static unsigned long long *g_bnb_stats = nullptr;

constexpr int64_t BNB_WS_HEADER = 256;
constexpr int64_t SPLIT_PAIRS = 131072, SPLIT_MIN_PAIRS = 192, SPLIT_RING = 16;
constexpr int64_t SPREAD_BELOW_PAIRS = 4096;
constexpr int64_t SPLIT_SLOT_FIXED = 8 * 64 * 4 + 1024;
constexpr uint32_t FRONT_MIN = 64;

static int64_t split_state_bytes(int64_t pairs, int64_t batches, int32_t n_theta) {
  return batches * SPLIT_SLOT_FIXED + pairs * (16 + 6 + (int64_t)n_theta * 512);
}
static uint32_t bnb_split_max(int64_t nb) { return nb < SPREAD_BELOW_PAIRS ? 16u : (nb >= 8192 ? 4u : 8u); }

int64_t bnb_workspace_bytes_lists(int32_t n_pairs) {
  const int64_t n = n_pairs > 0 ? n_pairs : 0;
  return BNB_WS_HEADER + 8 * (((n + 7) / 8) * 16 + 64) * (int64_t)sizeof(RotEntry);
}
int64_t bnb_workspace_bytes(int32_t n_pairs) {
  const int64_t n = n_pairs > 0 ? n_pairs : 0;
  nhip_search_t any = {};
  const int64_t m = n <= SPLIT_PAIRS ? n : 2 * SPLIT_PAIRS;
  const int64_t split = bnb_plan(GridLayout(), &any, (int32_t)n, 0).sized_split
                            ? BNB_WS_HEADER + split_state_bytes(m, m / 512 + 4, 64) : 0;
  return std::max(bnb_workspace_bytes_lists(n_pairs), split);
}

BnbPlan bnb_plan(const GridLayout &L, const nhip_search_t *search, int32_t n_pairs, int64_t workspace_bytes) {
  const auto is = [](const char *v, char c) { return v && v[0] == c; };
  const auto num = [](const char *name, int unset) { const char *v = tunable(name); return v ? atoi(v) : unset; };
  const char *force = tunable("NHIP_BNB_KERNELS");
  const char *sp = tunable("NHIP_BNB_SPLIT");
  const char *sbat = tunable("NHIP_BNB_SPLIT_BATCH");
  const char *smax = tunable("NHIP_BNB_SPLIT_MAX");
  BnbPlan p = {};
  p.n_pairs = n_pairs;
  p.cb = L.cb;
  p.levels = is(tunable("NHIP_BNB_LEVELS"), '1') ? 1 : 2;
  p.l2_runs = !is(tunable("NHIP_BNB_L2_RUNS"), '0');
  p.pair_subs = !is(tunable("NHIP_BNB_PAIR_SUBS"), '0');
  p.general_all = is(tunable("NHIP_BNB_QUEUE"), '1');
  static_assert(NHIP_SHORT_SCAN_POINTS == 64 * OCL, "the header's promise is the by-rotation form's limit");
  p.short_scans = (search->flags & NHIP_SEARCH_SHORT_SCANS) != 0 && !p.general_all && (uint32_t)(L.S + 2 * L.pad) < ORG_LIMIT;
  p.instrumented = is(tunable("NHIP_BNB_INSTRUMENT"), '1');
  p.stats = p.instrumented && is(tunable("NHIP_BNB_STATS"), '1');
  p.timeline = p.instrumented && is(tunable("NHIP_BNB_TIMELINE"), '1');
  p.sized_split = n_pairs >= SPLIT_MIN_PAIRS || (n_pairs > 0 && (is(sp, '1') || sbat));
  if (workspace_bytes > 0 && n_pairs > 0 && !p.general_all && !is(sp, '0') && !is(force, '2') &&
      (n_pairs >= SPLIT_MIN_PAIRS || is(sp, '1'))) {
    p.batch = sbat && atoi(sbat) > 0 ? atoi(sbat) : SPLIT_PAIRS;
    if (p.batch > n_pairs) p.batch = n_pairs;
    for (;;) {
      p.slot_bytes = (split_state_bytes(p.batch, 1, search->n_theta) + 511) & ~(int64_t)511;
      p.slots = (workspace_bytes - BNB_WS_HEADER - 512) / p.slot_bytes;
      const int64_t rounds = (n_pairs + p.batch - 1) / p.batch;
      if (p.slots >= (rounds < 2 ? rounds : 2) || p.batch <= 512) break;
      p.batch = p.batch / 2 > 512 ? p.batch / 2 : 512;
    }
    if (p.slots > SPLIT_RING) p.slots = SPLIT_RING;
    if (p.slots < 1) p.batch = 0;
    if (!sbat && p.batch > 0 && n_pairs > p.batch && (p.slots < 2 || p.batch < SPLIT_PAIRS)) p.batch = 0;
  }
  p.rounds = p.batch > 0 ? (n_pairs + p.batch - 1) / p.batch : 1;
  if (p.batch > 0)
    p.form = !is(tunable("NHIP_BNB_SPLIT_OVERLAP"), '0') && p.slots >= 2 && n_pairs > p.batch
                 ? BNB_SPLIT_OVERLAP : (p.rounds > 1 ? BNB_SPLIT_ROUNDS : BNB_SPLIT_ONE);
  p.split_min = (uint32_t)std::max(num("NHIP_BNB_SPLIT_MIN", 300), 1);
  p.split_max = smax ? (uint32_t)std::max(atoi(smax), 1) : 0u;
  p.heavy_min = (uint32_t)num("NHIP_BNB_HEAVY_MIN", n_pairs <= 64 ? 1 : 384);
  p.keep_ranks = (uint32_t)num("NHIP_BNB_KEEP_RANKS", 8);
  const bool second = force ? force[0] == '2' : (n_pairs < 1024 && p.batch == 0 && (uint32_t)search->n_theta > p.keep_ranks);
  p.second = second && !p.general_all && workspace_bytes >= BNB_WS_HEADER + 8 * (int64_t)sizeof(RotEntry);
  if (p.second)
    p.rot_cap = (uint32_t)std::min<int64_t>((workspace_bytes - BNB_WS_HEADER) / (int64_t)sizeof(RotEntry) / 8, 0x0fffffff);
  p.pool_lds = bnb_lds_bytes(L, search, true) <= LDS_MAX;
  p.lds_first = (int64_t)bnb_lds_first(L, p.pool_lds);
  return p;
}

struct SplitSet {
  int device = -1;
  hipStream_t stream = nullptr;
  hipEvent_t ea[SPLIT_RING], eb[SPLIT_RING];
};
static std::mutex g_split_mu;
static std::vector<SplitSet *> g_split_free;

static int split_set_acquire(SplitSet **out) {
  int dev = -1;
  NHIP_TRY_HIP(hipGetDevice(&dev));
  {
    std::lock_guard<std::mutex> lock(g_split_mu);
    for (size_t i = 0; i < g_split_free.size(); i++)
      if (g_split_free[i]->device == dev) {
        *out = g_split_free[i];
        g_split_free.erase(g_split_free.begin() + (long)i);
        return NHIP_OK;
      }
  }
  SplitSet *n = new SplitSet();
  n->device = dev;
  hipError_t e = hipStreamCreateWithFlags(&n->stream, hipStreamNonBlocking);
  for (int i = 0; i < SPLIT_RING && e == hipSuccess; i++) {
    e = hipEventCreateWithFlags(&n->ea[i], hipEventDisableTiming);
    if (e == hipSuccess) e = hipEventCreateWithFlags(&n->eb[i], hipEventDisableTiming);
  }
  if (e != hipSuccess) {
    delete n;
    return hip_fail(e, "split form: helper stream / events", __FILE__, __LINE__);
  }
  *out = n;
  return NHIP_OK;
}
static void split_set_release(SplitSet *set) {
  if (!set) return;
  std::lock_guard<std::mutex> lock(g_split_mu);
  g_split_free.push_back(set);
}

static thread_local BnbPlan t_last_plan = {};
void bnb_last_launch(int32_t out[8]) {
  const BnbPlan &p = t_last_plan;
  const int32_t info[8] = {p.form, (int32_t)p.batch, (int32_t)p.slots, (int32_t)p.rounds, p.short_scans, p.second,
                           (int32_t)p.instrumented | ((int32_t)p.l2_runs << 1) | ((int32_t)p.pair_subs << 2), p.n_pairs};
  memcpy(out, info, sizeof(info));
}

static void fill_bnb_params(BnbParams &P, const MatchJob &job, const BnbPlan &plan) {
  const GridLayout &L = *job.L;
  fill_job_params(P, job);
  P.pair_kbase = job.pair_kbase;
  P.keys = reinterpret_cast<unsigned long long *>(job.keys);
  P.gate = job_gate(job);
  P.nbx = (P.nx + BNB_B - 1) / BNB_B;
  P.nby = (P.ny + BNB_B - 1) / BNB_B;
  P.pool_pitch = L.pool_pitch;
  P.pool_rows = L.pool_rows;
  P.pairs_per_xcd = (plan.n_pairs + 7) / 8;
  P.skip_bytes = L.skip_bytes;
  P.pool_bytes = L.pool_bytes;
  P.pool4_bytes = L.pool4_bytes;
  P.pool4_pitch = L.pool4_pitch;
  P.hi_offset = L.hi_offset;
  P.hi_bytes = L.hi_bytes;
  P.hi_pitch = L.hi_pitch;
  P.hi_tpr = L.hi_tpr;
  P.hi_copy_bytes = L.hi_copy_bytes;
  P.t16_bytes = L.t16_bytes;
  P.t16_tpr = L.t16_tpr;
  P.inv_res_f = (float)P.inv_res;
  P.levels = plan.levels;
  P.l2_runs = plan.l2_runs;
  P.pair_subs = plan.pair_subs;
  P.general_all = plan.general_all;
  P.short_scans = plan.short_scans;
  P.heavy_min = plan.heavy_min;
  P.keep_ranks = plan.keep_ranks;
  P.rot_cap = plan.rot_cap;
  P.lds_first = (int32_t)plan.lds_first;
}

static int instr_buffers(const BnbPlan &plan, BnbParams &P, hipStream_t s) {
  if (!plan.stats && !plan.timeline) return NHIP_OK;
  std::lock_guard<std::mutex> lock(g_instr_mu);
  if (plan.stats) {
    if (!g_bnb_stats) {
      NHIP_TRY_HIP(hipMalloc(reinterpret_cast<void **>(&g_bnb_stats), 8 * (BNB_STATS_HEAD + (size_t)BNB_STATS_PAIRS)));
      NHIP_TRY_HIP(hipMemset(g_bnb_stats, 0, 8 * (BNB_STATS_HEAD + (size_t)BNB_STATS_PAIRS)));
    }
    P.stats = g_bnb_stats;
  }
  if (plan.timeline) {
    if (!g_bnb_timeline) NHIP_TRY_HIP(hipMalloc(reinterpret_cast<void **>(&g_bnb_timeline), 48 * (size_t)BNB_STATS_PAIRS + 16));
    P.timeline = g_bnb_timeline;
    NHIP_TRY_HIP(hipMemsetAsync(g_bnb_timeline + 4 * (size_t)BNB_STATS_PAIRS + 2, 0xff, 8 * (size_t)BNB_STATS_PAIRS, s));
    NHIP_TRY_HIP(hipMemsetAsync(g_bnb_timeline + 5 * (size_t)BNB_STATS_PAIRS + 2, 0, 8 * (size_t)BNB_STATS_PAIRS, s));
    const unsigned long long init[2] = {~0ull, 0ull};
    NHIP_TRY_HIP(hipMemcpyAsync(g_bnb_timeline + 4 * (size_t)BNB_STATS_PAIRS, init, 16, hipMemcpyHostToDevice, s));
  }
  return NHIP_OK;
}

static int run_rounds(const BnbParams &P, const BnbPlan &plan, const BnbLaunchers &K, void *d_workspace,
                      int64_t workspace_bytes, hipStream_t s) {
  const bool overlap = plan.form == BNB_SPLIT_OVERLAP;
  SplitSet *set = nullptr;
  if (overlap) {
    const int rc = split_set_acquire(&set);
    if (rc) return rc;
  }
  std::unique_ptr<SplitSet, void (*)(SplitSet *)> set_guard(set, split_set_release);
  hipStream_t s2 = overlap ? set->stream : s;
  uint8_t *base = static_cast<uint8_t *>(d_workspace) + BNB_WS_HEADER;
  base += (512 - (reinterpret_cast<uintptr_t>(base) & 511)) & 511;
  int64_t round = 0;
  for (int64_t b0 = 0; b0 < plan.n_pairs; b0 += plan.batch, round++) {
    const int32_t nb = (int32_t)(plan.n_pairs - b0 < plan.batch ? plan.n_pairs - b0 : plan.batch);
    BnbParams Q = P;
    Q.pair_src += b0;
    Q.pair_slot += b0;
    Q.rot0_cs += 2 * b0;
    if (Q.pair_origin) Q.pair_origin += 2 * b0;
    Q.keys += b0;
    Q.pair_base = (int32_t)b0;
    Q.n_pairs = nb;
    Q.pairs_per_xcd = (nb + 7) / 8;
    Q.ps_work_stride = Q.pairs_per_xcd + (Q.pairs_per_xcd / 2 > 64 ? Q.pairs_per_xcd / 2 : 64);
    Q.split_min = plan.split_min;
    Q.split_max = plan.split_max ? plan.split_max : bnb_split_max(nb);
    Q.front_min = FRONT_MIN;
    uint8_t *w = base + (round % plan.slots) * plan.slot_bytes;
    Q.ps_count = reinterpret_cast<uint32_t *>(w);
    Q.ps_live = Q.ps_count + nb;
    Q.ps_next = Q.ps_live + nb;
    Q.ps_nw = Q.ps_next + nb;
    const bool spread = nb < SPREAD_BELOW_PAIRS;
    Q.ps_ticket = spread ? Q.ps_nw + nb : nullptr;
    Q.ps_work = reinterpret_cast<int32_t *>(Q.ps_nw + nb + 4);
    const uintptr_t rows = (reinterpret_cast<uintptr_t>(Q.ps_work + 8 * (size_t)Q.ps_work_stride) + 511) & ~(uintptr_t)511;
    Q.ps_rows = reinterpret_cast<uint32_t *>(rows);
    NHIP_REQUIRE((int64_t)(rows - reinterpret_cast<uintptr_t>(w)) + (int64_t)nb * P.n_theta * 512 <= plan.slot_bytes &&
                     w + plan.slot_bytes <= static_cast<uint8_t *>(d_workspace) + workspace_bytes,
                 "csm_bnb: workspace accounting");
    if (overlap && round >= plan.slots) NHIP_TRY_HIP(hipStreamWaitEvent(s, set->eb[(round - plan.slots) % SPLIT_RING], 0));
    NHIP_TRY_HIP(hipMemsetAsync(w, 0, 16 * (size_t)nb + 16, s));
    if (spread) NHIP_TRY_HIP(hipMemsetAsync(Q.ps_work, 0xff, 32 * (size_t)Q.ps_work_stride, s));
    {
      TimerScope t_a(NHIP_TIMER_CSM_BOUNDS, s);
      const int rc = K.split_a(Q, plan, s);
      if (rc) return rc;
    }
    if (overlap) {
      NHIP_TRY_HIP(hipEventRecord(set->ea[round % SPLIT_RING], s));
      NHIP_TRY_HIP(hipStreamWaitEvent(s2, set->ea[round % SPLIT_RING], 0));
    }
    {
      TimerScope t_b(NHIP_TIMER_CSM_CAND, s2);
      const int rc = K.split_b(Q, plan, s2);
      if (rc) return rc;
    }
    if (overlap) NHIP_TRY_HIP(hipEventRecord(set->eb[round % SPLIT_RING], s2));
  }
  if (overlap) NHIP_TRY_HIP(hipStreamWaitEvent(s, set->eb[(round - 1) % SPLIT_RING], 0));
  return NHIP_OK;
}

int launch_csm_bnb(const MatchJob &job) {
  const GridLayout &L = *job.L;
  const hipStream_t s = job.stream;
  NHIP_REQUIRE(bnb_fits(L, job.search), "csm_match: lattice %d x %d x %d beyond the branch-and-bound matcher's envelope",
               job.search->n_theta, job.search->nx, job.search->ny);
  if (job.n_pairs == 0) return NHIP_OK;
  const BnbPlan plan = bnb_plan(L, job.search, job.n_pairs, job.workspace ? job.workspace_bytes : 0);
  NHIP_REQUIRE(L.has_image || plan.short_scans, "csm_match: grids built with NHIP_GRID_NO_IMAGE serve lists whose scans all have at most %d "
               "points, and the caller must say so (NHIP_SEARCH_SHORT_SCANS; the handle API sets it itself)", NHIP_SHORT_SCAN_POINTS);
  BnbParams P;
  fill_bnb_params(P, job, plan);
  int rc = instr_buffers(plan, P, s);
  if (rc) return rc;
  if (plan.second) {
    P.rot_count = static_cast<uint32_t *>(job.workspace);
    P.rot_list = reinterpret_cast<RotEntry *>(static_cast<uint8_t *>(job.workspace) + BNB_WS_HEADER);
    NHIP_TRY_HIP(hipMemsetAsync(job.workspace, 0, BNB_WS_HEADER, s));
  }
  const BnbLaunchers K = plan.instrumented ? launchers_instr() : launchers_product();
  t_last_plan = plan;
  {
    TimerScope t_all(NHIP_TIMER_CSM, s);
    rc = plan.form == BNB_FUSED ? K.fused(P, plan, s) : run_rounds(P, plan, K, job.workspace, job.workspace_bytes, s);
  }
  if (rc) return rc;
  NHIP_TRY_HIP(hipGetLastError());
  launch_csm_finalize(job);
  NHIP_TRY_HIP(hipGetLastError());
  return NHIP_OK;
}

int bnb_stats_per_pair(unsigned long long *out, int32_t n) {
  if (!g_bnb_stats || n <= 0) return NHIP_OK;
  NHIP_TRY_HIP(hipMemcpy(out, g_bnb_stats + BNB_STATS_HEAD, 8 * (size_t)(n < BNB_STATS_PAIRS ? n : BNB_STATS_PAIRS), hipMemcpyDeviceToHost));
  return NHIP_OK;
}

int bnb_timeline_read(unsigned long long *out, int32_t n) {
  if (!g_bnb_timeline || n <= 0) return NHIP_OK;
  if (n > BNB_STATS_PAIRS) n = BNB_STATS_PAIRS;
  NHIP_TRY_HIP(hipMemcpy(out, g_bnb_timeline, 32 * (size_t)n, hipMemcpyDeviceToHost));
  NHIP_TRY_HIP(hipMemcpy(out + 4 * (size_t)n, g_bnb_timeline + 4 * (size_t)BNB_STATS_PAIRS, 16, hipMemcpyDeviceToHost));
  return NHIP_OK;
}

int bnb_timeline_cand_read(unsigned long long *out, int32_t n) {
  if (!g_bnb_timeline || n <= 0) return NHIP_OK;
  if (n > BNB_STATS_PAIRS) n = BNB_STATS_PAIRS;
  NHIP_TRY_HIP(hipMemcpy(out, g_bnb_timeline + 4 * (size_t)BNB_STATS_PAIRS + 2, 8 * (size_t)n, hipMemcpyDeviceToHost));
  NHIP_TRY_HIP(hipMemcpy(out + n, g_bnb_timeline + 5 * (size_t)BNB_STATS_PAIRS + 2, 8 * (size_t)n, hipMemcpyDeviceToHost));
  return NHIP_OK;
}

int bnb_stats_read(unsigned long long out[24]) {
  static_assert(BNB_STATS_HEAD == 24, "the head is what nhip_bnb_stats_levels hands out");
  for (int i = 0; i < BNB_STATS_HEAD; i++) out[i] = 0;
  if (!g_bnb_stats) return NHIP_OK;
  NHIP_TRY_HIP(hipMemcpy(out, g_bnb_stats, 8 * BNB_STATS_HEAD, hipMemcpyDeviceToHost));
  NHIP_TRY_HIP(hipMemset(g_bnb_stats, 0, 8 * BNB_STATS_HEAD));
  return NHIP_OK;
}


}
```

### nautilus_amd/csrc/nhip_bnb_origin.h

```cpp
#pragma once
#include "nhip_bnb_params.h"
#include "nhip_bnb_wave.h"

namespace nhip {
namespace {

using namespace bnb;

template <bool LEAN = false>
__device__ __forceinline__ void window_origin(float2 q, float cf, float sf, const BnbParams &P, int32_t cx, int32_t cy,
                                              int32_t *prow, int32_t *pcol) {
  const float xr = __fsub_rn(__fmul_rn(cf, q.x), __fmul_rn(sf, q.y));
  const float yr = __fadd_rn(__fmul_rn(sf, q.x), __fmul_rn(cf, q.y));
  const int32_t half = P.S / 2;
  const bool finite __attribute__((unused)) = (fabsf(xr) < 1e9f) && (fabsf(yr) < 1e9f);
  int32_t ix, iy;
  const float mx = __fmul_rn(xr, P.inv_res_f), my = __fmul_rn(yr, P.inv_res_f);
  const float fx = floorf(mx), fy = floorf(my);
  if (LEAN) {
    const float rx = __fsub_rn(mx, fx), ry = __fsub_rn(my, fy);
    const float dx = fminf(rx, __fsub_rn(1.0f, rx)), dy = fminf(ry, __fsub_rn(1.0f, ry));
    const float tx = __fmul_rn(fabsf(mx), 0x1p-22f), ty = __fmul_rn(fabsf(my), 0x1p-22f);
    const unsigned long long slow = __builtin_amdgcn_fcmpf(dx, tx, 13 ) | __builtin_amdgcn_fcmpf(dy, ty, 13 );
    ix = (int32_t)fx;
// ... 35 lines not shown
  ix = min(max(ix, -P.hx - 1 - half - cx), P.S + P.hx - half - cx);
  iy = min(max(iy, -P.hy - 1 - half - cy), P.S + P.hy - half - cy);
  const int32_t col = finite ? half + ix + cx : -P.hx - 1, row = finite ? half + iy + cy : -P.hy - 1;
  *pcol = col - P.hx + P.pad;
  *prow = row - P.hy + P.pad;
}

typedef uint32_t u32x2 __attribute__((ext_vector_type(2)));
typedef uint32_t u32x3 __attribute__((ext_vector_type(3)));
typedef uint32_t u32x4 __attribute__((ext_vector_type(4)));

__device__ __forceinline__ __amdgpu_buffer_rsrc_t uniform_rsrc(const void *base, int64_t bytes) {
  const uint64_t a = reinterpret_cast<uint64_t>(base);
  const uint32_t lo = (uint32_t)__builtin_amdgcn_readfirstlane((int)(uint32_t)a);
  const uint32_t hi = (uint32_t)__builtin_amdgcn_readfirstlane((int)(uint32_t)(a >> 32));
  const int n = __builtin_amdgcn_readfirstlane((int)(bytes < 0x7fffffffll ? bytes : 0x7fffffffll));
  return __builtin_amdgcn_make_buffer_rsrc(reinterpret_cast<void *>(((uint64_t)hi << 32) | lo), 0, n, 0x00020000);
}

__device__ __forceinline__ uint32_t idx_guard(bool live, uint32_t v) { return live ? v : 0u; }

struct RotationTerms {
  double c0, s0, cd, sd;
};
__device__ __forceinline__ RotationTerms rotation_terms(const BnbParams &P, int32_t pair, int32_t k) {
  RotationTerms T;
  T.c0 = P.rot0_cs[2 * pair];
  T.s0 = P.rot0_cs[2 * pair + 1];
  const int32_t kd = k + (P.pair_kbase ? P.pair_kbase[pair] : 0);
  T.cd = P.delta_cs[2 * kd];
  T.sd = P.delta_cs[2 * kd + 1];
  return T;
}
__device__ __forceinline__ void rotation_of(const RotationTerms &T, float *cf, float *sf) {
  *cf = __double2float_rn(__dsub_rn(__dmul_rn(T.c0, T.cd), __dmul_rn(T.s0, T.sd)));
  *sf = __double2float_rn(__dadd_rn(__dmul_rn(T.s0, T.cd), __dmul_rn(T.c0, T.sd)));
}
__device__ __forceinline__ void rotation_k(const BnbParams &P, int32_t pair, int32_t k, float *cf, float *sf) {
  rotation_of(rotation_terms(P, pair, k), cf, sf);
}

template <int WAVES>
__device__ __forceinline__ RotationTerms rotation_terms_of_wave(const BnbParams &P, int32_t pair, int32_t wave, int lane) {
  static_assert(MAX_ROT <= 64 * WAVES, "a wave's rotations fit its lanes");
  RotationTerms T = {1.0, 0.0, 1.0, 0.0};
  if (wave < P.n_theta) {
    const int32_t mine = (P.n_theta - 1 - wave) / WAVES + 1;
    T = rotation_terms(P, pair, wave + WAVES * min(lane, mine - 1));
  }
  return T;
}

__device__ __forceinline__ void patch_origin(const BnbParams &P, bool live, float2 q, float cf, float sf, int32_t cx,
                                             int32_t cy, int32_t Y, int32_t X, uint32_t *g, uint32_t *sh) {
  *g = 0u;
  *sh = 0u;
  if (live) {
    int32_t prow, pcol;
    window_origin(q, cf, sf, P, cx, cy, &prow, &pcol);
    const int32_t col = pcol + BNB_B * X;
    *g = (uint32_t)((prow + BNB_B * Y) * P.pitch + (col & ~3));
    *sh = (uint32_t)(col & 3) * 8u;
  }
}


constexpr int ORG_COL_SHIFT = 6, ORG_ROW_SHIFT = 19;
__device__ __forceinline__ uint32_t org_row(uint32_t o) { return o >> ORG_ROW_SHIFT; }
__device__ __forceinline__ uint32_t org_col(uint32_t o) { return (o >> ORG_COL_SHIFT) & (ORG_LIMIT - 1u); }
__device__ __forceinline__ uint32_t org_cnt(uint32_t o) { return (o & 63u) + 1u; }

__device__ __forceinline__ uint32_t origin_of(const uint32_t *org, int c) { return c < OCL ? org[64 * c] : 0u; }

constexpr uint32_t RUN_KEY_MASK = (~0u << (ORG_ROW_SHIFT + 2)) | (((ORG_LIMIT >> 2) - 1u) << (ORG_COL_SHIFT + 2));
__device__ __forceinline__ uint32_t run_row2(uint32_t e) { return e >> (ORG_ROW_SHIFT + 2); }
__device__ __forceinline__ uint32_t run_col2(uint32_t e) { return (e >> (ORG_COL_SHIFT + 2)) & ((ORG_LIMIT >> 2) - 1u); }
__device__ __forceinline__ uint32_t run_cnt(uint32_t e) { return e & 127u; }
enum : int32_t { RUNS_NONE = 0, RUNS_FIELD = -1, RUNS_FULL = -2 };

template <bool RUNS = false, bool RING = RUNS>
__device__ __forceinline__ int32_t cache_origins(const BnbParams &P, const float2 *pts, int32_t n_pts, float cf, float sf,
                                                 int32_t cx, int32_t cy, int lane, uint32_t *org, bool merged,
                                                 uint32_t *runs = nullptr, bool want_runs = false,
                                                 int32_t *run_chunks = nullptr) {
  uint32_t *base = org - lane;
  const bool with_runs = RUNS && want_runs;
  if (RUNS) *run_chunks = RUNS_NONE;
  for (int merge = merged ? 1 : 0; merge >= 0; merge--) {
    constexpr int D = 3;
    uint32_t tail = 0u;
    uint32_t rtail = 0u;
    auto chunk = [&](float2 pt, int c) {
      const int32_t idx = 64 * c + lane;
      const bool live = idx < n_pts;
      uint32_t o = 0u;
      if (live) {
        int32_t prow, pcol;
        window_origin(pt, cf, sf, P, cx, cy, &prow, &pcol);
        o = ((uint32_t)prow << ORG_ROW_SHIFT) | ((uint32_t)pcol << ORG_COL_SHIFT);
      }
      const uint32_t prev = (uint32_t)__builtin_amdgcn_update_dpp((int)o, (int)o, 0x138 , 0xF, 0xF, false);
      const bool head = live && (lane == 0 || o != prev || merge == 0);
      const unsigned long long H = __ballot(head), L = __ballot(live);
      const unsigned long long rest = ((H | ~L) >> lane) >> 1;
      const uint32_t cnt = rest ? (uint32_t)__builtin_ctzll(rest) + 1u : (uint32_t)(64 - lane);
      if (head) {
        const uint32_t before = __builtin_amdgcn_mbcnt_hi((uint32_t)(H >> 32), __builtin_amdgcn_mbcnt_lo((uint32_t)H, 0u));
        base[tail + before] = o | (cnt - 1u);
      }
      tail += (uint32_t)__builtin_popcountll(H);
      if (RUNS && with_runs && merge) {
        const bool head2 = live && (lane == 0 || ((o ^ prev) & RUN_KEY_MASK) != 0u);
        const unsigned long long H2 = __ballot(head2);
        const unsigned long long rest2 = ((H2 | ~L) >> lane) >> 1;
        const uint32_t cnt2 = rest2 ? (uint32_t)__builtin_ctzll(rest2) + 1u : (uint32_t)(64 - lane);
        const uint32_t at = rtail + __builtin_amdgcn_mbcnt_hi((uint32_t)(H2 >> 32), __builtin_amdgcn_mbcnt_lo((uint32_t)H2, 0u));
        if (head2 && at < (uint32_t)RUN_WAVE) runs[at] = (o & RUN_KEY_MASK) | cnt2;
        rtail += (uint32_t)__builtin_popcountll(H2);
      }
    };
    const int32_t n_in = min(n_pts, 64 * OCL);
    if (RING) {
      constexpr int R = 6;
      float px[R], py[R];
#pragma unroll
      for (int d = 0; d < R; d++) {
        const float2 q = 64 * d + lane < n_pts ? pts[64 * d + lane] : make_float2(0.f, 0.f);
        px[d] = q.x;
        py[d] = q.y;
      }
#pragma unroll 1
      for (int c = 0; c < OCL; c++) {
        const int32_t idx = 64 * c + lane;
        if (64 * c >= n_pts) break;
        const float2 pt = make_float2(px[0], py[0]);
        const float2 qn = idx + 64 * R < n_pts ? pts[idx + 64 * R] : make_float2(0.f, 0.f);
#pragma unroll
        for (int d = 0; d < R - 1; d++) {
          px[d] = px[d + 1];
          py[d] = py[d + 1];
        }
        px[R - 1] = qn.x;
        py[R - 1] = qn.y;
        chunk(pt, c);
      }
    } else if (n_in > 0) {
      const uint32_t last = 8u * (uint32_t)(n_in - 1);
      auto point_at = [&](int32_t i) {
        return *reinterpret_cast<const float2 *>(reinterpret_cast<const char *>(pts) + min(8u * (uint32_t)i, last));
      };
      float2 q[D];
#pragma unroll
      for (int d = 0; d < D; d++) {
        int32_t i = 64 * d + lane;
        asm volatile("" : "+v"(i));
        q[d] = point_at(i);
        __builtin_amdgcn_sched_barrier(0);
      }
#pragma unroll 1
      for (int c = 0; 64 * c < n_in; c += D) {
#pragma unroll
        for (int d = 0; d < D; d++) {
          float2 pt = q[d];
          asm volatile("" : "+v"(pt.x), "+v"(pt.y));
          q[d] = point_at(64 * (c + d + D) + lane);
          if (d == 0 || 64 * (c + d) < n_in) chunk(pt, c + d);
        }
      }
    }
    const int32_t nch = (int32_t)((tail + 63u) >> 6);
    for (uint32_t e = tail + (uint32_t)lane; e < (uint32_t)ORG_WAVE; e += 64u) base[e] = 0u;
    if (RUNS && with_runs && merge)
      for (uint32_t e = rtail + (uint32_t)lane; e < (uint32_t)RUN_WAVE; e += 64u) runs[e] = 0u;
    __builtin_amdgcn_fence(__ATOMIC_RELEASE, "wavefront");
    __builtin_amdgcn_wave_barrier();
    if (merge == 0) {
      if (RUNS && with_runs) *run_chunks = RUNS_FIELD;
      return nch;
    }
    uint32_t w = 0u;
    for (int c = 0; c < nch; c++) {
      const uint32_t e = org[64 * c];
      w += 64u * (uint32_t)c + (uint32_t)lane < tail ? org_cnt(e) : 0u;
    }
    w = sum8(w);
    if (__ballot(w > 257u) == 0ull) {
      if (RUNS && with_runs) {
        const int32_t nrc = (int32_t)((rtail + 63u) >> 6);
        uint32_t w2 = 0u;
        if (rtail <= (uint32_t)RUN_WAVE)
          for (int c = 0; c < nrc; c++) w2 += run_cnt(runs[64 * c + lane]);
        w2 = sum8(w2);
        *run_chunks = rtail > (uint32_t)RUN_WAVE ? RUNS_FULL : (__ballot(w2 > 257u) != 0ull ? RUNS_FIELD : nrc);
      }
      return nch;
    }
    __builtin_amdgcn_wave_barrier();
  }
  return 0;
}
// ... 4 lines not shown
```

### nautilus_amd/csrc/nhip_bnb_params.h

```cpp
#pragma once
#include "nhip_common.h"
#include "nhip_csm_shared.h"

namespace nhip {
namespace bnb {

constexpr int BNB_WAVES = 8;
constexpr int NB = BNB_MAX_NB;
constexpr int MAX_ROT = 340;
constexpr int QCAP = 1024;
constexpr int SPLIT_WAVES = 8;
constexpr int LIST_ENTRIES = 128;
constexpr int RUN_SHIFT = 25;
constexpr int OC = 18;
constexpr int OCL = 17;
constexpr int ORG_WAVE = OCL * 64;
constexpr int ORG_LDS = BNB_WAVES * ORG_WAVE * 4;
constexpr uint32_t ORG_LIMIT = 1u << 13;
constexpr int RUN_CHUNKS = 8;
constexpr int RUN_WAVE = RUN_CHUNKS * 64;

constexpr int QSPACE_SPLIT = (SPLIT_WAVES * LIST_ENTRIES * 4 + MAX_ROT * 12 + 15) / 16 * 2;
constexpr int lds_qspace(bool split) { return split ? QSPACE_SPLIT : QCAP; }
static_assert(QSPACE_SPLIT <= QCAP, "the split form's LDS must not exceed the fused form's, which bnb_fits() checks");
struct LdsTail {
  unsigned long long best;
  uint32_t cnt[6];
  unsigned long long slow;
  uint32_t top;
};
constexpr int LDS_QN = 1, LDS_QHEAD = 2, LDS_TAIL_BYTES = 64;
static_assert(sizeof(LdsTail) <= LDS_TAIL_BYTES, "the tail fits its 64 bytes");
constexpr size_t lds_bytes(size_t first, int32_t n_theta, bool split) {
  return first + (size_t)n_theta * 128 * 4 + (size_t)lds_qspace(split) * 8 + LDS_TAIL_BYTES;
}

constexpr int BNB_STATS_PAIRS = 1 << 20;
constexpr int BNB_STATS_HEAD = 24;

struct RotEntry {
  unsigned long long w[4];
};

struct BnbParams {
  const float2 *xy;
  const int32_t *offsets;
  const uint8_t *grids;
  const int32_t *pair_src;
  const int32_t *pair_slot;
  IdBounds ids;
  const double *rot0_cs;
  const double *delta_cs;
  const int32_t *pair_origin;
  const int32_t *pair_kbase;
  unsigned long long *keys;
  unsigned long long *timeline;
  unsigned long long *stats;
  RotEntry *rot_list;
  uint32_t *rot_count;
  uint32_t rot_cap;
  uint32_t heavy_min;
  uint32_t keep_ranks;
  uint32_t *ps_rows;
  uint32_t *ps_count;
  uint32_t *ps_live;
  uint32_t *ps_next;
  uint32_t *ps_nw;
  int32_t *ps_work;
  uint32_t *ps_ticket;
  int32_t ps_work_stride;
  uint32_t split_min;
  uint32_t split_max;
  uint32_t front_min;
  int32_t pair_base;
  int32_t n_pairs, n_theta, nx, ny, hx, hy, nbx, nby;
  int32_t S, pad, pitch, rows, max_shift;
  int32_t pool_pitch, pool_rows, pairs_per_xcd;
  int32_t pool4_pitch;
  int32_t lds_first;
  int32_t general_all;
  int32_t short_scans;
  int32_t levels;
  int64_t grid_bytes, skip_bytes, slot_bytes, pool_bytes, pool4_bytes;
  int64_t hi_offset, hi_bytes;
  int32_t hi_pitch;
  int32_t hi_tpr;
  int64_t hi_copy_bytes;
  int64_t t16_bytes;
  int32_t t16_tpr;
  double res, inv_res;
  float inv_res_f;
  ScoreGate gate;
  int32_t l2_runs;
  int32_t pair_subs;
};

using BnbLaunch = int (*)(const BnbParams &P, const BnbPlan &plan, hipStream_t s);
struct BnbLaunchers { BnbLaunch fused, split_a, split_b; };
BnbLaunchers launchers_product();
BnbLaunchers launchers_instr();

}
}
```

### nautilus_amd/csrc/nhip_bnb_wave.h

```cpp
#pragma once
#include <hip/hip_runtime.h>

#include <cstdint>

namespace nhip {
namespace {

constexpr uint32_t M8 = 0x00ff00ffu;

__device__ __forceinline__ uint32_t shfl_xor_u32(uint32_t v, int m) { return (uint32_t)__shfl_xor((int)v, m, 64); }

__device__ __forceinline__ unsigned long long shfl_xor_u64b(unsigned long long v, int m) {
  uint32_t lo = (uint32_t)v, hi = (uint32_t)(v >> 32);
  lo = shfl_xor_u32(lo, m);
  hi = shfl_xor_u32(hi, m);
  return ((unsigned long long)hi << 32) | lo;
}

__device__ __forceinline__ bool wave_leader(int lane) {
  asm volatile("" : "+v"(lane));
  return lane == 0;
}
__device__ __forceinline__ uint32_t wave_fetch_add(uint32_t *p, uint32_t v, int lane) {
  uint32_t r = 0u;
// ... 15 lines not shown
__device__ __forceinline__ uint32_t rs_pair(uint32_t x, uint32_t y, bool bit) {
  if (MASK == 4) {
    uint32_t r;
    asm volatile("s_nop 1\n\tv_add_u32_dpp %0, %1, %1 row_ror:12 row_mask:0xf bank_mask:0x5\n\t"
                 "v_add_u32_dpp %0, %2, %2 row_ror:4 row_mask:0xf bank_mask:0xa"
                 : "=&v"(r) : "v"(x), "v"(y));
    return r;
  }
  if (MASK == 8) {
    uint32_t r;
    asm volatile("s_nop 1\n\tv_add_u32_dpp %0, %1, %1 row_ror:8 row_mask:0xf bank_mask:0x3\n\t"
                 "v_add_u32_dpp %0, %2, %2 row_ror:8 row_mask:0xf bank_mask:0xc"
                 : "=&v"(r) : "v"(x), "v"(y));
    return r;
  }
  if (MASK == 16) {
    const auto sw = __builtin_amdgcn_permlane16_swap(x, y, false, false);
    return sw[0] + sw[1];
  }
  if (MASK == 32) {
    const auto sw = __builtin_amdgcn_permlane32_swap(x, y, false, false);
    return sw[0] + sw[1];
  }
  const uint32_t keep = bit ? y : x, send = bit ? x : y;
  return keep + shfl_xor_c<MASK>(send);
}

template <int N, int MASK, int CAP>
__device__ __forceinline__ void rs_step(uint32_t (&R)[CAP], bool bit) {
  static_assert(N <= CAP, "rs_step: more registers than the array holds");
#pragma unroll
  for (int i = 0; i < N / 2; i++) R[i] = rs_pair<MASK>(R[2 * i], R[2 * i + 1], bit);
}

template <int MASK>
__device__ __forceinline__ uint32_t add_xor(uint32_t v) {
  if (MASK == 16) {
    const auto sw = __builtin_amdgcn_permlane16_swap(v, v, false, false);
    return sw[0] + sw[1];
  }
  if (MASK == 32) {
    const auto sw = __builtin_amdgcn_permlane32_swap(v, v, false, false);
    return sw[0] + sw[1];
  }
  return v + shfl_xor_u32(v, MASK);
}

__device__ __forceinline__ uint32_t mad24(uint32_t a, uint32_t b, uint32_t acc) {
  uint32_t r;
  asm("v_mad_u32_u24 %0, %1, %2, %3" : "=v"(r) : "v"(a), "v"(b), "v"(acc));
  return r;
}

__device__ __forceinline__ uint32_t sum8(uint32_t v) {
  v += (uint32_t)__builtin_amdgcn_update_dpp(0, (int)v, 0xB1, 0xF, 0xF, false);
  v += (uint32_t)__builtin_amdgcn_update_dpp(0, (int)v, 0x4E, 0xF, 0xF, false);
  return v + (uint32_t)__builtin_amdgcn_update_dpp(0, (int)v, 0x141, 0xF, 0xF, false);
}
__device__ __forceinline__ uint32_t wave_total_of8(uint32_t v) {
  v += (uint32_t)__builtin_amdgcn_update_dpp(0, (int)v, 0x140, 0xF, 0xF, false);
  v += (uint32_t)__builtin_amdgcn_update_dpp(0, (int)v, 0x142, 0xF, 0xF, false);
  v += (uint32_t)__builtin_amdgcn_update_dpp(0, (int)v, 0x143, 0xF, 0xF, false);
  return (uint32_t)__builtin_amdgcn_readlane((int)v, 63);
}

__device__ __forceinline__ uint32_t wave_sum(uint32_t v) {
  v += (uint32_t)__builtin_amdgcn_update_dpp(0, (int)v, 0xB1, 0xF, 0xF, false);
  v += (uint32_t)__builtin_amdgcn_update_dpp(0, (int)v, 0x4E, 0xF, 0xF, false);
  v += (uint32_t)__builtin_amdgcn_update_dpp(0, (int)v, 0x124, 0xF, 0xF, false);
  v += (uint32_t)__builtin_amdgcn_update_dpp(0, (int)v, 0x128, 0xF, 0xF, false);
  v = add_xor<16>(v);
  return add_xor<32>(v);
}
__device__ __forceinline__ uint32_t wave_max(uint32_t v) {
  v = max(v, (uint32_t)__builtin_amdgcn_update_dpp(0, (int)v, 0xB1, 0xF, 0xF, false));
  v = max(v, (uint32_t)__builtin_amdgcn_update_dpp(0, (int)v, 0x4E, 0xF, 0xF, false));
  v = max(v, (uint32_t)__builtin_amdgcn_update_dpp(0, (int)v, 0x124, 0xF, 0xF, false));
  v = max(v, (uint32_t)__builtin_amdgcn_update_dpp(0, (int)v, 0x128, 0xF, 0xF, false));
  const auto s16 = __builtin_amdgcn_permlane16_swap(v, v, false, false);
  v = max(s16[0], s16[1]);
  const auto s32 = __builtin_amdgcn_permlane32_swap(v, v, false, false);
  return max(s32[0], s32[1]);
}
template <int CTRL>
__device__ __forceinline__ unsigned long long max_dpp_u64(unsigned long long v) {
  const uint32_t lo = (uint32_t)__builtin_amdgcn_update_dpp(0, (int)(uint32_t)v, CTRL, 0xF, 0xF, false);
  const uint32_t hi = (uint32_t)__builtin_amdgcn_update_dpp(0, (int)(uint32_t)(v >> 32), CTRL, 0xF, 0xF, false);
  const unsigned long long o = ((unsigned long long)hi << 32) | lo;
  return o > v ? o : v;
}
__device__ __forceinline__ unsigned long long wave_max_u64(unsigned long long v) {
  v = max_dpp_u64<0xB1>(v);
  v = max_dpp_u64<0x4E>(v);
  v = max_dpp_u64<0x124>(v);
  v = max_dpp_u64<0x128>(v);
  {
    const auto l = __builtin_amdgcn_permlane16_swap((uint32_t)v, (uint32_t)v, false, false);
    const auto h = __builtin_amdgcn_permlane16_swap((uint32_t)(v >> 32), (uint32_t)(v >> 32), false, false);
    const unsigned long long a = ((unsigned long long)h[0] << 32) | l[0], b = ((unsigned long long)h[1] << 32) | l[1];
    v = a > b ? a : b;
  }
  const auto l = __builtin_amdgcn_permlane32_swap((uint32_t)v, (uint32_t)v, false, false);
  const auto h = __builtin_amdgcn_permlane32_swap((uint32_t)(v >> 32), (uint32_t)(v >> 32), false, false);
  const unsigned long long a = ((unsigned long long)h[0] << 32) | l[0], b = ((unsigned long long)h[1] << 32) | l[1];
  return a > b ? a : b;
}

}
}
```

### nautilus_amd/csrc/nhip_common.h

```cpp
#pragma once
#include <hip/hip_runtime.h>

#include <cmath>
#include <cstdint>
#include <cstdio>
#include <cstring>
#include <string>
#include <vector>

#include "../../include/nautilus_hip_debug.h"

namespace nhip {

void set_error(const char *fmt, ...);
int hip_fail(hipError_t e, const char *what, const char *file, int line);

#define NHIP_TRY_HIP(expr)                                            \
  do {                                                                \
    hipError_t _e = (expr);                                           \
    if (_e != hipSuccess) return ::nhip::hip_fail(_e, #expr, __FILE__, __LINE__); \
  } while (0)

#define NHIP_REQUIRE(cond, ...)          \
  do {                                   \
// ... 66 lines not shown
  int64_t pool_offset;
  int64_t pool4_offset;
  int64_t hi_offset;
  int64_t t16_offset;
  int64_t hits_offset;
  int32_t pool_pitch, pool_rows;
  int32_t pool4_pitch, pool4_rows;
  double Lf, step;
};
constexpr uint32_t HI_TILE_BYTES = 128u;
__host__ __device__ __forceinline__ uint32_t hi_tiled(uint32_t row, uint32_t col, uint32_t cp, uint32_t tpr, uint32_t copy_bytes) {
  const uint32_t c = col + 8u * cp;
  return cp * copy_bytes + ((row >> 3) * tpr + (c >> 4)) * HI_TILE_BYTES + (row & 7u) * 16u + (c & 15u);
}

__host__ __device__ __forceinline__ uint32_t t16_tiled(uint32_t row, uint32_t col, uint32_t tpr) {
  return ((row >> 3) * tpr + (col >> 3)) * HI_TILE_BYTES + (row & 7u) * 16u + (col & 7u) * 2u;
}

constexpr int HIT_PAD = 32;

constexpr int BNB_B = 8;
constexpr int BNB_POOL = 2 * BNB_B - 1;
constexpr int BNB_MAX_NB = 11;
constexpr int BNB_B4 = 4;
constexpr int BNB_POOL4 = 2 * BNB_B4 - 1;
constexpr int CSM_WAVE_ROWS = 21;
constexpr int CSM_ROW_DW = 21;
#ifdef __HIPCC__
__device__ __forceinline__ double floor_quotient(double v, double res, double inv_res) {
  const double m = __dmul_rn(v, inv_res);
  double f = floor(m);
  const double frac = __dsub_rn(m, f);
  const double tol = __dmul_rn(fabs(m), 0x1p-50);
  if (frac <= tol || __dsub_rn(1.0, frac) <= tol) f = floor(__ddiv_rn(v, res));
  return f;
}
#endif

constexpr int64_t GRID_WS_HEADER = 256;
constexpr int64_t GRID_WS_THR16 = 65536 * 4;
constexpr int GRID_WS_MASK_WORDS = 5;
inline int64_t grid_ws_per_target(int32_t S) {
  const int64_t tiles = (S + 63) / 64;
  return (5 + 4 * GRID_WS_MASK_WORDS) * tiles * tiles;
}
__host__ __device__ constexpr int32_t skip_pitch(int32_t pitch) { return ((pitch / 4 + 63) / 64) * 8; }
int make_layout(const nhip_grid_spec_t *spec, GridLayout *L);

struct GridTables {
  int32_t taps[129];
  uint32_t thr[256];
  const uint32_t *thr16 = nullptr;
};
int make_tables(const nhip_grid_spec_t *spec, const GridLayout &L, GridTables *T);

void timer_begin(int id, hipStream_t s);
void timer_end(int id, hipStream_t s);

int launch_grid_build(const float *d_xy, const int32_t *d_offsets, int32_t n_scans, const int32_t *d_target_ids,
                      int32_t n_targets, const nhip_grid_spec_t *spec, const GridLayout &L,
                      uint8_t *d_grids, void *d_ws, int64_t ws_bytes, hipStream_t s, bool incremental = false);

enum MatchForm : int32_t {
  MATCH_BNB,
  MATCH_POSES,
  MATCH_STRIPS8,
  MATCH_STRIPS16,
};
struct MatchPlan {
  MatchForm form = MATCH_BNB;
  int32_t tile_rows = 0, n_tiles = 0;
  bool keys_zeroed = false, keys_undecoded = false;
};
MatchPlan csm_plan(const GridLayout &L, const nhip_search_t *search, int32_t n_pairs);

enum BnbForm : int32_t { BNB_FUSED, BNB_SPLIT_ONE, BNB_SPLIT_ROUNDS, BNB_SPLIT_OVERLAP };
struct BnbPlan {
  BnbForm form;
  int32_t n_pairs, cb, levels;
  bool second, general_all, short_scans, pool_lds, instrumented, stats, timeline;
  bool l2_runs;
  bool pair_subs;
  bool sized_split;
  uint32_t rot_cap, heavy_min, keep_ranks, split_min, split_max;
  int64_t batch, slots, slot_bytes, rounds;
  int64_t lds_first;
};
BnbPlan bnb_plan(const GridLayout &L, const nhip_search_t *search, int32_t n_pairs, int64_t workspace_bytes);

struct MatchJob {
  const float *xy = nullptr;
  const int32_t *offsets = nullptr;
  IdBounds ids = {0, 0, nullptr};
  const uint8_t *grids = nullptr;
  const nhip_grid_spec_t *spec = nullptr;
  const GridLayout *L = nullptr;
  const int32_t *pair_src = nullptr, *pair_slot = nullptr;
  const double *rot0_cs = nullptr;
  const double *delta_cs = nullptr;
  const int32_t *pair_origin = nullptr, *pair_kbase = nullptr;
  int32_t n_pairs = 0;
  const nhip_search_t *search = nullptr;
  double min_score = -INFINITY;
  uint64_t *keys = nullptr;
  nhip_match_t *out = nullptr;
  int32_t *sums = nullptr;
  hipStream_t stream = nullptr;
  void *workspace = nullptr;
  int64_t workspace_bytes = 0;
};

int launch_csm_match(const MatchJob &job, const MatchPlan &plan);

int launch_csm_bnb(const MatchJob &job);
int64_t bnb_workspace_bytes(int32_t n_pairs);
int64_t bnb_workspace_bytes_lists(int32_t n_pairs);
void bnb_last_launch(int32_t out[8]);
bool bnb_fits(const GridLayout &L, const nhip_search_t *search);
int bnb_stats_read(unsigned long long out[24]);
int bnb_timeline_read(unsigned long long *out, int32_t n);
int bnb_timeline_cand_read(unsigned long long *out, int32_t n);
int bnb_stats_per_pair(unsigned long long *out, int32_t n);
void launch_csm_finalize(const MatchJob &job);

int launch_csm_scores(const MatchJob &job, int32_t src, int32_t slot, int32_t origin_x, int32_t origin_y, int32_t *d_volume);

int launch_csm_exact_score(const MatchJob &job, const MatchPlan &plan);
bool csm_small_plane_fits(const nhip_search_t *search);
bool csm_small_tiled_fits(const nhip_search_t *search, int32_t n_pairs, int32_t *tile_rows, int32_t *n_tiles);
int launch_csm_small_match(const MatchJob &job, const MatchPlan &plan);
int launch_skipmap_build(uint8_t *d_grids, int32_t n_grids, const GridLayout &L, hipStream_t s);

int launch_resid_lidar(int kind, const float *d_corr, const int32_t *d_corr_block, int64_t n_corr,
                       const int32_t *d_block_src, const int32_t *d_block_tgt, int32_t n_blocks,
                       const double *d_poses, int32_t n_poses, double *d_block_consts,
                       double *d_res, double *d_jsrc, double *d_jtgt, hipStream_t s, double *d_jtgt_theta = nullptr,
                       int32_t block_base = 0, double *d_q = nullptr);

int launch_resid_normal_eq(int kind, const float *d_corr, const int32_t *d_block_offsets,
                           const int32_t *d_block_src, const int32_t *d_block_tgt, int32_t n_blocks,
                           const double *d_poses, int32_t n_poses, double *d_block_consts, double *d_out,
                           hipStream_t s);

int launch_corr_search(const float *d_xy, const float *d_normals, const int32_t *d_offsets, int32_t n_scans,
                       const int32_t *d_block_src, const int32_t *d_block_tgt, int32_t n_blocks,
                       const float *d_pose_aff, float thr, float min_cos, bool gate, const int64_t *d_cap_offsets,
                       float *d_corr_padded, int32_t *d_counts, hipStream_t s);

int launch_corr_compact(const float *d_corr_padded, const int64_t *d_cap_offsets,
                        const int32_t *d_counts, int32_t n_blocks, int32_t *d_block_offsets,
                        float *d_corr, int32_t *d_corr_block, hipStream_t s);

int launch_lc_scatter_scores(const float *d_xy, const int32_t *d_offsets, int32_t n_scans, double *d_scores, hipStream_t s);
int launch_lc_chi_square(const double *d_poses, int32_t n_poses, const int32_t *d_src, const int32_t *d_tgt, const float *d_cov,
                         int32_t n, double max_score, double *d_scores, uint8_t *d_flags, hipStream_t s);
int launch_lc_pair_gate(const double *d_poses, int32_t n_poses, const int32_t *d_cand, int32_t n, double max_range,
                        int32_t min_sep, uint8_t *d_flags, hipStream_t s);

int launch_round_norm(const float *d_dx, const float *d_dy, int64_t n, int32_t root_only, float *d_out, hipStream_t s);

int launch_feat_extract(const float *d_xy, const int32_t *d_offsets, int32_t n_scans, const nhip_feature_spec_t &spec,
                        int32_t *d_planar_idx, int32_t *d_planar_count, int32_t *d_edge_idx, int32_t *d_edge_count,
                        double *d_scores, hipStream_t s);
int launch_feat_pack(const float *d_xy, const float *d_normals, const int32_t *d_offsets, int32_t n_scans, const int32_t *d_idx,
                     const int32_t *d_count, int32_t cap, float *d_xy_out, float *d_normals_out, int32_t *d_offsets_out,
                     hipStream_t s);

int launch_submap_gather(const float *d_xy, const int32_t *d_offsets, int32_t n_scans, const int32_t *d_member_scan,
                         const float *d_member_affine, const int32_t *d_member_offsets, int32_t n_targets, float *d_out_xy,
                         int64_t out_capacity, int32_t *d_out_offsets, hipStream_t s);

int launch_normals_estimate(const float *d_xy, const int32_t *d_offsets, int32_t n_scans, const nhip_normals_spec_t &spec,
                            int32_t sample_limit, float *d_normals, int32_t *d_info, hipStream_t s);

struct VecState {
  int32_t stats[8];
  int32_t end;
  int32_t peak_t, peak_b, peak_votes;
  int32_t action;
  int32_t n_band;
};
enum { VEC_RETIRE = 1, VEC_COMMIT = 2 };
struct VecLayout {
  int64_t state, counts, cells, votes, live, row_off, tables, partial, bits, run_of_bin, run_lo, run_hi, run_slot, band_list, bytes;
  int32_t n_rho, n_along, bit_words, max_runs;
};
void vec_layout(const nhip_vectorize_spec_t &spec, int32_t max_cells, VecLayout *L);
struct VecParams {
  int32_t width, height, cell_x0, cell_y0, n_theta, n_rho, n_along, min_hits, min_votes, band_q, gap1, min_length, max_segments,
      max_cells, max_rounds, n_scans;
  double res, inv_res;
  VecState *st;
  int32_t *counts, *cells, *votes, *row_off, *run_of_bin, *run_lo, *run_hi, *run_slot, *band_list;
  const int32_t *C, *S;
  uint8_t *live;
  unsigned long long *partial;
  uint32_t *bits;
  long long *records;
  uint32_t *status;
};
int launch_vec_front(const VecParams &P, const float *d_xy, const int32_t *d_offsets, const float *d_affines, hipStream_t s);
int launch_vec_rounds(const VecParams &P, int32_t n, hipStream_t s);
// ... 171 lines not shown
```

### nautilus_amd/csrc/nhip_host_csm.hip

```cpp
#include "nhip_common.h"
#include "nhip_host.h"

using namespace nhip;

static uint64_t grids_shape(const nhip_grid_spec_t *spec, int32_t n_targets) {
  uint64_t h = 0xcbf29ce484222325ull;
  const unsigned char *b = reinterpret_cast<const unsigned char *>(spec);
  for (size_t i = 0; i < sizeof(*spec); i++) h = (h ^ b[i]) * 0x100000001b3ull;
  for (int i = 0; i < 4; i++) h = (h ^ (uint64_t)((uint32_t)n_targets >> (8 * i) & 0xffu)) * 0x100000001b3ull;
  return h >> 1;
}

int nhip::ensure_skip_maps(const nhip_grids_t *grids, const MatchPlan &plan) {
  nhip_grids *g = const_cast<nhip_grids *>(grids);
  if (plan.form != MATCH_STRIPS16 || g->n == 0 || !g->L.has_image) return NHIP_OK;
  std::lock_guard<std::mutex> lock(g->mu);
  if (g->spec.flags & NHIP_GRID_SKIP_MAP) return NHIP_OK;
  g->dirty = true;
  int rc = launch_skipmap_build(g->grids.as<uint8_t>(), g->n, g->L, nullptr);
  if (rc) return rc;
  NHIP_TRY_HIP(hipStreamSynchronize(nullptr));
  g->spec.flags |= NHIP_GRID_SKIP_MAP;
  return NHIP_OK;
}
// ... 495 lines not shown
  job.keys = d_keys.as<uint64_t>();
  job.out = d_out.as<nhip_match_t>();
  job.sums = d_sums.as<int32_t>();
  job.workspace = d_ws.p;
  job.workspace_bytes = ws_bytes;
  PhaseClock pc_enq(PH_ENQUEUE);
  InFlight inflight;
  rc = launch_csm_match(job, plan);
  if (rc) return rc;
  {
    PhaseClock pc(PH_WAIT);
    NHIP_TRY_HIP(hipStreamSynchronize(nullptr));
    InFlight::done();
  }
  {
    PhaseClock pc(PH_DOWNLOAD);
    NHIP_TRY_HIP(hipMemcpy(out, d_out.p, sizeof(nhip_match_t) * (size_t)n_pairs, hipMemcpyDeviceToHost));
    if (out_sums) NHIP_TRY_HIP(hipMemcpy(out_sums, d_sums.p, sizeof(int32_t) * (size_t)n_pairs, hipMemcpyDeviceToHost));
  }
  return NHIP_OK;
}

int nhip_csm_scores(const nhip_scans_t *scans, const nhip_grids_t *grids, int32_t src, int32_t slot,
                    double theta0, int32_t origin_x, int32_t origin_y, const nhip_search_t *search,
                    int32_t *out_sums) {
  int rc = require_device();
  if (rc) return rc;
  NHIP_REQUIRE(scans && grids && search && out_sums, "csm_scores: bad arguments");
  NHIP_REQUIRE(src >= 0 && src < scans->n_scans && slot >= 0 && slot < grids->n, "csm_scores: index out of range");
  {
    nhip_search_t ex = *search;
    ex.flags = (ex.flags | NHIP_SEARCH_EXHAUSTIVE) & ~NHIP_SEARCH_LATENCY;
    if ((rc = ensure_skip_maps(grids, csm_plan(grids->L, &ex, 1)))) return rc;
  }
  double rot0[2];
  std::vector<double> delta(2 * (size_t)search->n_theta);
  if ((rc = nhip_csm_rot0(&theta0, nullptr, 1, rot0))) return rc;
  if ((rc = nhip_csm_delta_table(search, delta.data()))) return rc;
  const size_t vol = (size_t)search->n_theta * search->nx * search->ny;
  Staged st;
  MatchJob job = job_on(scans->xy, scans->offsets, *grids, grids->spec);
  job.rot0_cs = st.in(rot0, 2);
  job.delta_cs = st.in(delta.data(), delta.size());
  job.search = search;
  int32_t *d_vol = st.out<int32_t>(vol);
  if (st.ok()) st.launched(launch_csm_scores(job, src, slot, origin_x, origin_y, d_vol));
  st.fetch(out_sums, d_vol, vol);
  return st.finish();
}

int nhip_bnb_stats_per_pair(uint64_t *evaluated, int32_t n_pairs) {
  NHIP_REQUIRE(evaluated && n_pairs >= 0, "bnb_stats_per_pair: bad arguments");
  return bnb_stats_per_pair(reinterpret_cast<unsigned long long *>(evaluated), n_pairs);
}

int nhip_bnb_timeline(uint64_t *ticks, int32_t n_pairs) {
  NHIP_REQUIRE(ticks && n_pairs >= 0, "bnb_timeline: bad arguments");
  return bnb_timeline_read(reinterpret_cast<unsigned long long *>(ticks), n_pairs);
}

int nhip_bnb_timeline_candidates(uint64_t *ticks, int32_t n_pairs) {
  NHIP_REQUIRE(ticks && n_pairs >= 0, "bnb_timeline_candidates: bad arguments");
  return bnb_timeline_cand_read(reinterpret_cast<unsigned long long *>(ticks), n_pairs);
}

int nhip_bnb_stats(uint64_t *evaluated, uint64_t *total) {
  unsigned long long v[24];
  int rc = bnb_stats_read(v);
  if (rc) return rc;
  if (evaluated) *evaluated = v[0] + (v[3] + 3) / 4;
  if (total) *total = v[1];
  return NHIP_OK;
}

int nhip_bnb_stats_levels(uint64_t out[24]) {
  NHIP_REQUIRE(out != nullptr, "bnb_stats_levels: null out");
  unsigned long long v[24];
  int rc = bnb_stats_read(v);
  if (rc) return rc;
  for (int i = 0; i < 24; i++) out[i] = v[i];
  return NHIP_OK;
}

}
```

Before: 1.818 million.

## Skip all-zero origin chunks in BnB block and pose sums via strip-bound notes

While computing strip bounds from run lists, the kernel now records per-run nibble flags showing which sub-block fields have nonzero pooled counts, plus a span byte mapping each run to its origin chunks. Block, pair, sub-block and pose-level sums then build a wave-wide chunk mask and read only chunks that can contribute. The goal is fewer grid reads on chunks whose points land in empty cells. It costs extra LDS (note and span arrays), the bookkeeping and wave_or reductions, and possible occupancy pressure, and adds chunk-visit counters and a stats API. It is on by default through NHIP_BNB_ZERO_CHUNKS.

```diff
diff --git a/include/nautilus_hip.h b/include/nautilus_hip.h
--- a/include/nautilus_hip.h
+++ b/include/nautilus_hip.h
@@ -543,6 +543,8 @@
 int nhip_allgather_matches(void *comm, const nhip_match_t *d_local, int32_t n_local,
                            nhip_match_t *d_all, void *stream);
 
+int nhip_bnb_stats_chunks(uint64_t out[4]);
+
 #ifdef __cplusplus
 }
 #endif
diff --git a/nautilus_amd/_lib.py b/nautilus_amd/_lib.py
--- a/nautilus_amd/_lib.py
+++ b/nautilus_amd/_lib.py
@@ -170,6 +170,7 @@
     "nhip_bnb_timeline": (C.c_int, [_vp, _i32]),
     "nhip_bnb_timeline_candidates": (C.c_int, [_vp, _i32]),
     "nhip_bnb_stats_levels": (C.c_int, [_P(C.c_uint64)]),
+    "nhip_bnb_stats_chunks": (C.c_int, [_P(C.c_uint64)]),
     "nhip_csm_scores_dev": (C.c_int, [_vp, _vp, _i32, _vp, _i32, _P(GridSpec), _i32, _i32, _vp, _vp, _i32, _i32,
                                       _P(Search), _vp, _vp]),
     "nhip_resid_lidar_dev": (C.c_int, [C.c_int, _vp, _vp, _i64, _vp, _vp, _i32, _vp, _i32, _vp,
diff --git a/nautilus_amd/csm.py b/nautilus_amd/csm.py
--- a/nautilus_amd/csm.py
+++ b/nautilus_amd/csm.py
@@ -224,6 +224,12 @@
             "edge_blocks_whole": v[21], "pair_passes": v[22], "pair_passes_across_blocks": v[23]}
 
 
+def bnb_stats_chunks():
+    v = (C.c_uint64 * 4)()
+    check(_lib.load().nhip_bnb_stats_chunks(v))
+    return {"chunk_visits_full": v[0], "chunk_visits": v[1], "pose_chunk_visits_full": v[2], "pose_chunk_visits": v[3]}
+
+
 def score_volume(scans, grids, src, slot, theta0, search, origin=(0, 0)):
     out = np.zeros((search.n_theta, search.nx, search.ny), dtype=np.int32)
     check(_lib.load().nhip_csm_scores(scans._h, grids._h, int(src), int(slot), float(theta0),
@@ -260,7 +266,8 @@
     form = {0: "fused", 1: "split, one round", 2: "split, rounds on one stream", 3: "split, rounds overlapped on the helper stream"}
     return {"form": form.get(out[0], "?"), "form_id": out[0], "pairs_per_round": out[1], "rounds_of_state": out[2],
             "rounds": out[3], "short_scans": bool(out[4]), "hand_over_kernel": bool(out[5]), "instrumented": bool(out[6] & 1),
-            "l2_runs": bool(out[6] & 2), "pair_subs": bool(out[6] & 4), "n_pairs": out[7]}
+            "l2_runs": bool(out[6] & 2), "pair_subs": bool(out[6] & 4), "zero_chunks": bool(out[6] & 8),
+            "n_pairs": out[7]}
 
 
 def drop_in_cache_stats():
diff --git a/nautilus_amd/csrc/nhip_bnb.hip b/nautilus_amd/csrc/nhip_bnb.hip
--- a/nautilus_amd/csrc/nhip_bnb.hip
+++ b/nautilus_amd/csrc/nhip_bnb.hip
@@ -31,12 +31,30 @@
 
 constexpr int BNB_THREADS = 64 * BNB_WAVES;
 
-constexpr int N_WORK = 9;
+constexpr int N_WORK = 13;
 struct PairCtx {
   const uint8_t *grid;
   const float2 *pts;
   int32_t n_pts, cx, cy, pair;
 };
+
+struct ChunkNotes {
+  const uint16_t *note;
+  const uint8_t *span;
+  int32_t nrc;
+  uint32_t full;
+};
+__device__ __forceinline__ uint32_t chunk_mask(const ChunkNotes &N, uint32_t fields) {
+  if (N.nrc <= 0) return N.full;
+  uint32_t acc = 0u;
+#pragma unroll
+  for (int j = 0; j < RUN_CHUNKS; j++) {
+    const uint32_t f = N.note[64 * j], s = N.span[64 * j];
+    const uint32_t chunks = (1u + ((s >> 5) << 1)) << (s & 31u);
+    acc |= (j < N.nrc && (f & fields) != 0u) ? chunks : 0u;
+  }
+  return wave_or(acc) & N.full;
+}
 
 template <int CB>
 __device__ __forceinline__ void process_candidate(const BnbParams &P, const PairCtx &C, int32_t k, int32_t v, int lane,
@@ -77,13 +95,14 @@
   n[6] += edge ? 1u : 0u;
 }
 
-template <int CB, bool GLOBAL, bool PAIR>
+template <int CB, bool GLOBAL, bool PAIR, bool ZC = false>
 __device__ __forceinline__ void process_candidate_c(const BnbParams &P, __amdgpu_buffer_rsrc_t rsrc, uint32_t pitch8,
                                                     __amdgpu_buffer_rsrc_t rsrc16, const uint32_t *org, int32_t nch,
                                                     int32_t n_pts, int32_t k, int32_t Y, int32_t X,
                                                     uint32_t sb0, uint32_t sb1, uint32_t sb2, uint32_t sb3, int lane,
                                                     unsigned long long *best, uint32_t &bcopy, uint32_t (&n)[N_WORK],
-                                                    int t, uint32_t &mk0, uint32_t &mk1) {
+                                                    int t, uint32_t &mk0, uint32_t &mk1,
+                                                    const ChunkNotes &CN = ChunkNotes()) {
   const uint32_t bsum = best_sum_cached<GLOBAL>(best, bcopy);
   const int32_t vx = block_extent(P.nx, X), vy = block_extent(P.ny, Y);
   const bool edge = vx < BNB_B || vy < BNB_B;
@@ -95,14 +114,25 @@
   constexpr int WHOLE_MIN = 3;
   if (alive >= WHOLE_MIN) {
     int dy, dx;
-    const uint32_t total = block_sums8(rsrc, pitch8, (uint32_t)P.hi_copy_bytes, org, nch, Y, X, lane, &dy, &dx);
+    const uint32_t visit = ZC ? chunk_mask(CN, 0xfu << (4 * t)) : 0u;
+    const uint32_t total = ZC ? block_sums8_masked(rsrc, pitch8, (uint32_t)P.hi_copy_bytes, org, visit, Y, X, lane, &dy, &dx)
+                              : block_sums8(rsrc, pitch8, (uint32_t)P.hi_copy_bytes, org, nch, Y, X, lane, &dy, &dx);
     const int32_t ix = BNB_B * X + dx, iy = BNB_B * Y + dy;
+    if (ZC) {
+      n[9] += (uint32_t)nch;
+      n[10] += (uint32_t)__builtin_popcount(visit);
+    }
     if (CB == 1) {
       const unsigned long long key = best_key(P, k, ix, iy, total, 32);
       wave_atomic_max(best, key, lane);
       if (GLOBAL) bcopy = max(bcopy, (uint32_t)(key >> 32));
     } else {
-      n[3] += refine16<GLOBAL>(P, rsrc16, org, nch, n_pts, k, ix, iy, total, true, lane, best, bcopy);
+      const uint32_t read = refine16<GLOBAL, ZC>(P, rsrc16, org, nch, n_pts, k, ix, iy, total, true, lane, best, bcopy, visit);
+      n[3] += read;
+      if (ZC) {
+        n[11] += read * (uint32_t)nch;
+        n[12] += read * (uint32_t)__builtin_popcount(visit);
+      }
     }
     n[0]++;
     n[6] += __ballot(ix < P.nx && iy < P.ny) != ~0ull ? 1u : 0u;
@@ -144,7 +174,7 @@
                                                  __amdgpu_buffer_rsrc_t rsrc16, const uint32_t *org, int32_t nch, int32_t n_pts,
                                                  int32_t k, int32_t Y, int32_t X0, const uint32_t (&sb)[12], uint32_t mk0,
                                                  uint32_t mk1, int lane, unsigned long long *best, uint32_t &bcopy,
-                                                 uint32_t (&n)[N_WORK]) {
+                                                 uint32_t (&n)[N_WORK], const ChunkNotes &CN) {
 #pragma unroll 1
   for (int sy = 0; sy < 2; sy++) {
     uint32_t mk = sy ? mk1 : mk0;
@@ -162,11 +192,15 @@
       const bool two = P.pair_subs != 0 && ((mk >> (c + 1)) & 1u) != 0u && (PAIR_CROSS || sx == 0) && pick6(row, c + 1) >= bsum;
       int dy, dx;
       uint32_t total;
+      const uint32_t field = 1u << (4 * (c >> 1) + sy + 2 * sx);
+      const uint32_t visit = two ? (sx == 0 ? chunk_mask(CN, field | (field << 2)) : CN.full) : chunk_mask(CN, field);
+      n[9] += (uint32_t)nch;
+      n[10] += (uint32_t)__builtin_popcount(visit);
       if (two) {
         mk &= ~(1u << (c + 1));
-        total = pair_sums8(rsrc, pitch8, (uint32_t)P.hi_copy_bytes, org, nch, Y, X, sy, sx, lane, &dy, &dx);
+        total = pair_sums8_masked(rsrc, pitch8, (uint32_t)P.hi_copy_bytes, org, visit, Y, X, sy, sx, lane, &dy, &dx);
       } else {
-        total = sub_sums8(rsrc, pitch8, (uint32_t)P.hi_copy_bytes, org, nch, Y, X, sy, sx, lane, &dy, &dx);
+        total = sub_sums8_masked(rsrc, pitch8, (uint32_t)P.hi_copy_bytes, org, visit, Y, X, sy, sx, lane, &dy, &dx);
       }
       const int32_t ix = BNB_B * X + BNB_B4 * sx + dx, iy = BNB_B * Y + BNB_B4 * sy + dy;
       if (CB == 1) {
@@ -174,7 +208,10 @@
         wave_atomic_max(best, key, lane);
         if (GLOBAL) bcopy = max(bcopy, (uint32_t)(key >> 32));
       } else {
-        n[3] += refine16<GLOBAL>(P, rsrc16, org, nch, n_pts, k, ix, iy, total, lane < (two ? 32 : 16), lane, best, bcopy);
+        const uint32_t read = refine16<GLOBAL, true>(P, rsrc16, org, nch, n_pts, k, ix, iy, total, lane < (two ? 32 : 16), lane, best, bcopy, visit);
+        n[3] += read;
+        n[11] += read * (uint32_t)nch;
+        n[12] += read * (uint32_t)__builtin_popcount(visit);
       }
       const bool pose = ix < P.nx && iy < P.ny;
       if (two) {
@@ -196,13 +233,18 @@
 };
 
 __device__ __forceinline__ void flush_stats(unsigned long long *stats, const uint32_t *n, int32_t pair, const PhaseClocks *clk,
-                                            const uint32_t *edge = nullptr) {
+                                            const uint32_t *edge = nullptr, bool chunks = false) {
   if (n) {
     if (n[0]) atomicAdd(&stats[0], (unsigned long long)n[0]);
     if (n[1]) atomicAdd(&stats[2], (unsigned long long)n[1]);
     if (n[2]) atomicAdd(&stats[3], (unsigned long long)n[2]);
     if (n[3]) atomicAdd(&stats[14], (unsigned long long)n[3]);
     if (pair < BNB_STATS_PAIRS) atomicAdd(&stats[BNB_STATS_HEAD + pair], 4ull * n[0] + n[2]);
+  }
+  if (edge && chunks) {
+    unsigned long long *at = stats + BNB_STATS_HEAD + (size_t)BNB_STATS_PAIRS;
+    for (int i = 0; i < BNB_STATS_CHUNKS; i++)
+      if (edge[5 + i]) atomicAdd(&at[i], (unsigned long long)edge[5 + i]);
   }
   if (edge) {
     if (edge[0]) atomicAdd(&stats[19], (unsigned long long)edge[0]);
@@ -225,13 +267,15 @@
 __device__ __forceinline__ void rotation_pass(const BnbParams &P, const PairCtx &C, int32_t k, uint32_t u0, uint32_t u1,
                                               unsigned long long m0, unsigned long long m1, int lane,
                                               unsigned long long *best, uint32_t *done, uint32_t *org,
-                                              uint32_t (&n_work)[N_WORK], PhaseClocks &clk, uint32_t *runs = nullptr) {
+                                              uint32_t (&n_work)[N_WORK], PhaseClocks &clk, uint32_t *runs = nullptr,
+                                              uint16_t *note = nullptr, uint8_t *span = nullptr) {
   long long t_mark = 0;
   float cf, sf;
   rotation_k(P, C.pair, k, &cf, &sf);
   if (BNB_STATS(P)) t_mark = clock64();
   int32_t nrc = RUNS_NONE;
-  const int32_t nch = cache_origins<RUNS>(P, C.pts, C.n_pts, cf, sf, C.cx, C.cy, lane, org, true, runs, RUNS && P.l2_runs != 0, &nrc);
+  const int32_t nch = cache_origins<RUNS>(P, C.pts, C.n_pts, cf, sf, C.cx, C.cy, lane, org, true, runs, RUNS && P.l2_runs != 0, &nrc, span);
+  const ChunkNotes CN = {note + lane, span + lane, RUNS && P.zero_chunks != 0 && P.levels >= 2 ? nrc : 0, (1u << nch) - 1u};
   if (BNB_STATS(P)) clk.org += clock64() - t_mark;
   if (RUNS && BNB_STATS(P)) {
     clk.run_passes += nrc > 0 ? 1u : 0u;
@@ -256,7 +300,7 @@
     uint32_t bcopy = GLOBAL ? best_sum<true>(best) : 0u;
     if (P.levels >= 2) {
       if (BNB_STATS(P)) t_mark = clock64();
-      if (RUNS && nrc > 0) strip_bounds_c<RunList<RUN_CHUNKS>>(P, p4, runs + lane, nrc, Y, X0, len, CB == 1 ? 1u : 257u, sb);
+      if (RUNS && nrc > 0) strip_bounds_c<RunList<RUN_CHUNKS>, RUNS>(P, p4, runs + lane, nrc, Y, X0, len, CB == 1 ? 1u : 257u, sb, note + lane);
       else strip_bounds_c<CellList>(P, p4, org, nch, Y, X0, len, CB == 1 ? 1u : 257u, sb);
       if (BNB_STATS(P)) clk.strip += clock64() - t_mark;
       n_work[1] += (uint32_t)len;
@@ -275,14 +319,14 @@
       const uint32_t s0 = t == 0 ? sb[0] : (t == 1 ? sb[4] : sb[8]), s1 = t == 0 ? sb[1] : (t == 1 ? sb[5] : sb[9]);
       const uint32_t s2 = t == 0 ? sb[2] : (t == 1 ? sb[6] : sb[10]), s3 = t == 0 ? sb[3] : (t == 1 ? sb[7] : sb[11]);
       if (BNB_STATS(P)) t_mark = clock64();
-      process_candidate_c<CB, GLOBAL, PAIR>(P, rsrc, pitch8, rsrc16, org, nch, C.n_pts, k, Y, X0 + t, s0, s1, s2, s3, lane, best,
-                                      bcopy, n_work, t, mk0, mk1);
+      process_candidate_c<CB, GLOBAL, PAIR, RUNS>(P, rsrc, pitch8, rsrc16, org, nch, C.n_pts, k, Y, X0 + t, s0, s1, s2, s3, lane, best,
+                                            bcopy, n_work, t, mk0, mk1, CN);
       if (BNB_STATS(P)) clk.eval += clock64() - t_mark;
       if (done && wave_leader(lane)) done[b] = 0u;
     }
     if (PAIR && (mk0 | mk1) != 0u) {
       if (BNB_STATS(P)) t_mark = clock64();
-      strip_sub_blocks<CB, GLOBAL>(P, rsrc, pitch8, rsrc16, org, nch, C.n_pts, k, Y, X0, sb, mk0, mk1, lane, best, bcopy, n_work);
+      strip_sub_blocks<CB, GLOBAL>(P, rsrc, pitch8, rsrc16, org, nch, C.n_pts, k, Y, X0, sb, mk0, mk1, lane, best, bcopy, n_work, CN);
       if (BNB_STATS(P)) clk.eval += clock64() - t_mark;
     }
   }
@@ -636,8 +680,12 @@
   const RotEntry *list = P.rot_list + (size_t)xcd * P.rot_cap;
   __shared__ uint32_t s_org2[4 * ORG_WAVE];
   __shared__ uint32_t s_run2[4 * RUN_WAVE];
+  __shared__ uint16_t s_note2[4 * RUN_WAVE];
+  __shared__ uint8_t s_span2[4 * RUN_WAVE];
   uint32_t *org = s_org2 + (threadIdx.x >> 6) * ORG_WAVE + lane;
   uint32_t *runs = s_run2 + (threadIdx.x >> 6) * RUN_WAVE;
+  uint16_t *note = s_note2 + (threadIdx.x >> 6) * RUN_WAVE;
+  uint8_t *span = s_span2 + (threadIdx.x >> 6) * RUN_WAVE;
   PhaseClocks clk = {0, 0, 0, 0u, 0u, 0u};
   const long long t0 = BNB_STATS(P) ? clock64() : 0;
   for (;;) {
@@ -649,8 +697,8 @@
     PairCtx C;
     pair_context(P, pair, &C);
     uint32_t n[N_WORK] = {};
-    rotation_pass<CB, true, true, true>(P, C, k, 0xffffffffu, 0xffffffffu, m0, m1, lane, &P.keys[pair], nullptr, org, n, clk, runs);
-    if (BNB_STATS(P) && lane == 0) flush_stats(BNB_STATS(P), n, pair, nullptr, n + 4);
+    rotation_pass<CB, true, true, true>(P, C, k, 0xffffffffu, 0xffffffffu, m0, m1, lane, &P.keys[pair], nullptr, org, n, clk, runs, note, span);
+    if (BNB_STATS(P) && lane == 0) flush_stats(BNB_STATS(P), n, pair, nullptr, n + 4, true);
   }
   if (BNB_STATS(P) && lane == 0) {
     atomicAdd(&BNB_STATS(P)[13], (unsigned long long)(clock64() - t0));
@@ -752,6 +800,9 @@
 __global__ __launch_bounds__(CAND_THREADS, CB == 2 ? 5 : 4) void csm_bnb_cand_kernel(BnbParams P) {
   __shared__ uint32_t s_org2[CAND_WAVES * ORG_WAVE];
   __shared__ uint32_t s_run2[CAND_WAVES * RUN_WAVE];
+  __shared__ uint16_t s_note2[CAND_WAVES * RUN_WAVE];
+  __shared__ uint8_t s_span2[CAND_WAVES * RUN_WAVE];
+  static_assert(CAND_WAVES * (ORG_WAVE * 4 + RUN_WAVE * 4 + RUN_NOTE_BYTES) + 16 <= 32 * 1024, "five workgroups per CU");
   __shared__ unsigned long long s_best2;
   __shared__ uint32_t s_next2;
   const int lane = threadIdx.x & 63;
@@ -774,6 +825,8 @@
   const uint32_t *rows = P.ps_rows + (size_t)pair * (size_t)P.n_theta * 128u;
   uint32_t *org = s_org2 + (threadIdx.x >> 6) * ORG_WAVE + lane;
   uint32_t *runs = s_run2 + (threadIdx.x >> 6) * RUN_WAVE;
+  uint16_t *note = s_note2 + (threadIdx.x >> 6) * RUN_WAVE;
+  uint8_t *span = s_span2 + (threadIdx.x >> 6) * RUN_WAVE;
   PairCtx C;
   pair_context(P, pair, &C);
   uint32_t n_work[N_WORK] = {};
@@ -790,11 +843,11 @@
     const unsigned long long m0 = __ballot(u0 != 0u && u0 >= bsum);
     const unsigned long long m1 = __ballot(u1 != 0u && u1 >= bsum && lane + 64 < NB * NB);
     if ((m0 | m1) == 0ull) continue;
-    rotation_pass<CB, true, true, true>(P, C, k, u0, u1, m0, m1, lane, best, nullptr, org, n_work, clk, runs);
+    rotation_pass<CB, true, true, true>(P, C, k, u0, u1, m0, m1, lane, best, nullptr, org, n_work, clk, runs, note, span);
   }
   if (BNB_STATS(P) && lane == 0) {
     atomicAdd(&BNB_STATS(P)[13], (unsigned long long)(clock64() - t0));
-    flush_stats(BNB_STATS(P), n_work, pair, &clk, n_work + 4);
+    flush_stats(BNB_STATS(P), n_work, pair, &clk, n_work + 4, true);
   }
   if (BNB_TIMELINE(P) && lane == 0 && pair < BNB_STATS_PAIRS)
     atomicMax(&BNB_TIMELINE(P)[5 * (size_t)BNB_STATS_PAIRS + 2 + pair], wall_clock64());
diff --git a/nautilus_amd/csrc/nhip_bnb_bounds.h b/nautilus_amd/csrc/nhip_bnb_bounds.h
--- a/nautilus_amd/csrc/nhip_bnb_bounds.h
+++ b/nautilus_amd/csrc/nhip_bnb_bounds.h
@@ -251,9 +251,15 @@
   static __device__ __forceinline__ uint32_t count(uint32_t e) { return run_cnt(e); }
 };
 
-template <class LIST>
+__device__ __forceinline__ uint32_t nonzero_bytes(uint32_t n) {
+  const uint32_t t = ((((n & 0x7f7f7f7fu) + 0x7f7f7f7fu) | n) & 0x80808080u) >> 7;
+  return (t * 0x01020408u) >> 24;
+}
+
+template <class LIST, bool NOTE = false>
 __device__ __forceinline__ void strip_sums(const BnbParams &P, __amdgpu_buffer_rsrc_t p4, const uint32_t *list, int32_t nch,
-                                           int32_t Y, int32_t X0, int len, uint32_t (&E)[3], uint32_t (&O)[3]) {
+                                           int32_t Y, int32_t X0, int len, uint32_t (&E)[3], uint32_t (&O)[3],
+                                           uint16_t *note = nullptr) {
   const uint32_t DP = (uint32_t)P.pool4_pitch;
   const uint32_t off = (uint32_t)(2 * Y) * DP + (uint32_t)(4 * X0);
   constexpr int ROUNDS = LIST::ROUNDS, H = LIST::H;
@@ -295,23 +301,27 @@
       E[0] += __umul24(n0 & M8, cn[j]); O[0] += __umul24((n0 >> 8) & M8, cn[j]);
       E[1] += __umul24(n1 & M8, cn[j]); O[1] += __umul24((n1 >> 8) & M8, cn[j]);
       E[2] += __umul24(n2 & M8, cn[j]); O[2] += __umul24((n2 >> 8) & M8, cn[j]);
-    }
-  }
-}
-
-template <class LIST>
+      if (NOTE) {
+        const uint32_t f = nonzero_bytes(n0) | (nonzero_bytes(n1) << 4) | (nonzero_bytes(n2) << 8);
+        note[64 * (H * h + j)] = (uint16_t)(cn[j] != 0u ? f : 0u);
+      }
+    }
+  }
+}
+
+template <class LIST, bool NOTE = false>
 __device__ __forceinline__ void strip_bounds_c(const BnbParams &P, __amdgpu_buffer_rsrc_t p4, const uint32_t *list,
                                                int32_t nch, int32_t Y, int32_t X0, int len, uint32_t scale,
-                                               uint32_t (&out)[12]) {
+                                               uint32_t (&out)[12], uint16_t *note = nullptr) {
   uint32_t E[3] = {0u, 0u, 0u}, O[3] = {0u, 0u, 0u};
   if (std::is_same<LIST, CellList>::value) {
     strip_sums<CellList>(P, p4, list, nch, Y, X0, len, E, O);
   } else {
     static_assert(RUN_CHUNKS == 8, "the rounds below cover the run list");
-    if (nch <= 4) strip_sums<RunList<4>>(P, p4, list, nch, Y, X0, len, E, O);
-    else if (nch == 5) strip_sums<RunList<5>>(P, p4, list, nch, Y, X0, len, E, O);
-    else if (nch == 6) strip_sums<RunList<6>>(P, p4, list, nch, Y, X0, len, E, O);
-    else strip_sums<RunList<8>>(P, p4, list, nch, Y, X0, len, E, O);
+    if (nch <= 4) strip_sums<RunList<4>, NOTE>(P, p4, list, nch, Y, X0, len, E, O, note);
+    else if (nch == 5) strip_sums<RunList<5>, NOTE>(P, p4, list, nch, Y, X0, len, E, O, note);
+    else if (nch == 6) strip_sums<RunList<6>, NOTE>(P, p4, list, nch, Y, X0, len, E, O, note);
+    else strip_sums<RunList<8>, NOTE>(P, p4, list, nch, Y, X0, len, E, O, note);
   }
 #pragma unroll
   for (int t = 0; t < 3; t++) {
diff --git a/nautilus_amd/csrc/nhip_bnb_exact.h b/nautilus_amd/csrc/nhip_bnb_exact.h
--- a/nautilus_amd/csrc/nhip_bnb_exact.h
+++ b/nautilus_amd/csrc/nhip_bnb_exact.h
@@ -453,6 +453,190 @@
   return V[0];
 }
 
+__device__ __forceinline__ int next_chunk(uint32_t &mask) {
+  const int c = (int)__builtin_ctz(mask);
+  mask &= mask - 1u;
+  return c;
+}
+
+__device__ __forceinline__ uint32_t sub_sums8_masked(__amdgpu_buffer_rsrc_t rsrc, uint32_t pitch, uint32_t copy_bytes, const uint32_t *org,
+                                                     uint32_t mask, int32_t Y, int32_t X, int32_t sy, int32_t sx, int lane, int *dy, int *dx) {
+  const uint32_t roff = (uint32_t)(BNB_B * Y + BNB_B4 * sy), coff = (uint32_t)(BNB_B * X + BNB_B4 * sx);
+  const uint32_t wrap = pitch * HI_TILE_BYTES - HI_TILE_BYTES;
+  uint32_t E[4] = {0u, 0u, 0u, 0u}, O[4] = {0u, 0u, 0u, 0u};
+  auto load = [&](int c, u32x2 (&w)[4], uint32_t &sh, uint32_t &cn) {
+    const uint32_t o = org[64 * c];
+    cn = org_cnt(o);
+    const uint32_t row0 = org_row(o) + roff, col0 = org_col(o) + coff, col4 = col0 & ~3u;
+    const uint32_t cp = (col4 >> 3) & 1u, q = row0 & 7u;
+    const uint32_t v0 = hi_tiled(row0, col4, cp, pitch, copy_bytes);
+    sh = (col0 & 3u) * 8u;
+#pragma unroll
+    for (int y = 0; y < 4; y++)
+      w[y] = __builtin_amdgcn_raw_buffer_load_b64(rsrc, (int)(v0 + (q + (uint32_t)y >= 8u ? wrap : 0u) + 16u * (uint32_t)y), 0, 0);
+  };
+  auto add = [&](const u32x2 (&w)[4], uint32_t sh, uint32_t cn) {
+#pragma unroll
+    for (int y = 0; y < 4; y++) {
+      const uint32_t n = __builtin_amdgcn_alignbit(w[y].y, w[y].x, sh);
+      E[y] += __umul24(n & M8, cn);
+      O[y] += __umul24(n >> 8, cn);
+    }
+  };
+#pragma unroll 1
+  while ((mask & (mask - 1u)) != 0u) {
+    u32x2 wa[4], wb[4];
+    uint32_t sa, sb, ca, cb;
+    load(next_chunk(mask), wa, sa, ca);
+    load(next_chunk(mask), wb, sb, cb);
+    add(wa, sa, ca);
+    add(wb, sb, cb);
+  }
+  if (mask != 0u) {
+    u32x2 wa[4];
+    uint32_t sa, ca;
+    load(next_chunk(mask), wa, sa, ca);
+    add(wa, sa, ca);
+  }
+  uint32_t R[8];
+#pragma unroll
+  for (int y = 0; y < 4; y++) {
+    R[2 * y] = E[y];
+    R[2 * y + 1] = O[y] - ((E[y] >> 16) << 8);
+  }
+  rs_step<8, 1>(R, lane & 1);
+  rs_step<4, 2>(R, lane & 2);
+  rs_step<2, 4>(R, lane & 4);
+  uint32_t V[2] = {R[0] & 0xffffu, R[0] >> 16};
+  rs_step<2, 8>(V, lane & 8);
+  V[0] = add_xor<16>(V[0]);
+  V[0] = add_xor<32>(V[0]);
+  *dy = ((lane >> 1) & 1) + 2 * ((lane >> 2) & 1);
+  *dx = (lane & 1) + 2 * ((lane >> 3) & 1);
+  return V[0];
+}
+
+__device__ __forceinline__ uint32_t block_sums8_masked(__amdgpu_buffer_rsrc_t rsrc, uint32_t pitch, uint32_t copy_bytes, const uint32_t *org,
+                                                       uint32_t mask, int32_t Y, int32_t X, int lane, int *dy, int *dx) {
+  const uint32_t roff = (uint32_t)(BNB_B * Y), coff = (uint32_t)(BNB_B * X);
+  const uint32_t wrap = pitch * HI_TILE_BYTES - HI_TILE_BYTES;
+  uint32_t E[8][2], O[8][2];
+#pragma unroll
+  for (int y = 0; y < 8; y++) E[y][0] = E[y][1] = O[y][0] = O[y][1] = 0u;
+#pragma unroll 1
+  while (mask != 0u) {
+    constexpr int ROWS = 4;
+    const uint32_t o = org[64 * next_chunk(mask)];
+    const uint32_t cn = org_cnt(o);
+    const uint32_t row0 = org_row(o) + roff, col0 = org_col(o) + coff, col4 = col0 & ~3u;
+    const uint32_t q = row0 & 7u, sh = (col0 & 3u) * 8u;
+    const uint32_t g = hi_tiled(row0, col4, (col4 >> 3) & 1u, pitch, copy_bytes);
+#pragma unroll
+    for (int y0 = 0; y0 < 8; y0 += ROWS) {
+      u32x3 w[ROWS];
+#pragma unroll
+      for (int y = 0; y < ROWS; y++)
+        w[y] = __builtin_amdgcn_raw_buffer_load_b96(rsrc, (int)(g + (q + (uint32_t)(y0 + y) >= 8u ? wrap : 0u) + 16u * (uint32_t)(y0 + y)), 0, 0);
+#pragma unroll
+      for (int y = 0; y < ROWS; y++) {
+        const uint32_t n0 = __builtin_amdgcn_alignbit(w[y].y, w[y].x, sh);
+        const uint32_t n1 = __builtin_amdgcn_alignbit(w[y].z, w[y].y, sh);
+        E[y0 + y][0] += __umul24(n0 & M8, cn); O[y0 + y][0] += __umul24(n0 >> 8, cn);
+        E[y0 + y][1] += __umul24(n1 & M8, cn); O[y0 + y][1] += __umul24(n1 >> 8, cn);
+      }
+    }
+  }
+  uint32_t R[32];
+#pragma unroll
+  for (int y = 0; y < 8; y++) {
+    R[4 * y + 0] = E[y][0];
+    R[4 * y + 1] = O[y][0] - ((E[y][0] >> 16) << 8);
+    R[4 * y + 2] = E[y][1];
+    R[4 * y + 3] = O[y][1] - ((E[y][1] >> 16) << 8);
+  }
+  rs_step<32, 1>(R, lane & 1);
+  rs_step<16, 2>(R, lane & 2);
+  rs_step<8, 4>(R, lane & 4);
+  uint32_t V[8];
+#pragma unroll
+  for (int i = 0; i < 4; i++) {
+    V[2 * i] = R[i] & 0xffffu;
+    V[2 * i + 1] = R[i] >> 16;
+  }
+  rs_step<8, 8>(V, lane & 8);
+  rs_step<4, 16>(V, lane & 16);
+  rs_step<2, 32>(V, lane & 32);
+  const int r = 8 * (2 * ((lane >> 5) & 1) + ((lane >> 4) & 1)) + 4 * ((lane >> 2) & 1) + 2 * ((lane >> 1) & 1) + (lane & 1);
+  const int f = (lane >> 3) & 1, d = r & 3;
+  *dy = r >> 2;
+  *dx = 4 * (d >> 1) + (d & 1) + 2 * f;
+  return V[0];
+}
+
+__device__ __forceinline__ uint32_t pair_sums8_masked(__amdgpu_buffer_rsrc_t rsrc, uint32_t pitch, uint32_t copy_bytes, const uint32_t *org,
+                                                      uint32_t mask, int32_t Y, int32_t X, int32_t sy, int32_t sx0, int lane, int *dy, int *dx) {
+  const uint32_t roff = (uint32_t)(BNB_B * Y + BNB_B4 * sy), coff = (uint32_t)(BNB_B * X + BNB_B4 * sx0);
+  const uint32_t wrap = pitch * HI_TILE_BYTES - HI_TILE_BYTES;
+  uint32_t E[4][2], O[4][2];
+#pragma unroll
+  for (int y = 0; y < 4; y++) E[y][0] = E[y][1] = O[y][0] = O[y][1] = 0u;
+  auto load = [&](int c, u32x3 (&w)[4], uint32_t &sh, uint32_t &cn) {
+    const uint32_t o = org[64 * c];
+    cn = org_cnt(o);
+    const uint32_t row0 = org_row(o) + roff, col0 = org_col(o) + coff, col4 = col0 & ~3u;
+    const uint32_t q = row0 & 7u;
+    sh = (col0 & 3u) * 8u;
+    const uint32_t g = hi_tiled(row0, col4, (col4 >> 3) & 1u, pitch, copy_bytes);
+#pragma unroll
+    for (int y = 0; y < 4; y++)
+      w[y] = __builtin_amdgcn_raw_buffer_load_b96(rsrc, (int)(g + (q + (uint32_t)y >= 8u ? wrap : 0u) + 16u * (uint32_t)y), 0, 0);
+  };
+  auto add = [&](const u32x3 (&w)[4], uint32_t sh, uint32_t cn) {
+#pragma unroll
+    for (int y = 0; y < 4; y++) {
+      const uint32_t n0 = __builtin_amdgcn_alignbit(w[y].y, w[y].x, sh);
+      const uint32_t n1 = __builtin_amdgcn_alignbit(w[y].z, w[y].y, sh);
+      E[y][0] += __umul24(n0 & M8, cn); O[y][0] += __umul24(n0 >> 8, cn);
+      E[y][1] += __umul24(n1 & M8, cn); O[y][1] += __umul24(n1 >> 8, cn);
+    }
+  };
+#pragma unroll 1
+  while ((mask & (mask - 1u)) != 0u) {
+    u32x3 wa[4], wb[4];
+    uint32_t sa, sb, ca, cb;
+    load(next_chunk(mask), wa, sa, ca);
+    load(next_chunk(mask), wb, sb, cb);
+    add(wa, sa, ca);
+    add(wb, sb, cb);
+  }
+  if (mask != 0u) {
+    u32x3 wa[4];
+    uint32_t sa, ca;
+    load(next_chunk(mask), wa, sa, ca);
+    add(wa, sa, ca);
+  }
+  uint32_t R[16];
+#pragma unroll
+  for (int y = 0; y < 4; y++) {
+    R[4 * y + 0] = E[y][0];
+    R[4 * y + 1] = O[y][0] - ((E[y][0] >> 16) << 8);
+    R[4 * y + 2] = E[y][1];
+    R[4 * y + 3] = O[y][1] - ((E[y][1] >> 16) << 8);
+  }
+  rs_step<16, 1>(R, lane & 1);
+  rs_step<8, 2>(R, lane & 2);
+  rs_step<4, 4>(R, lane & 4);
+  uint32_t V[4] = {R[0] & 0xffffu, R[0] >> 16, R[1] & 0xffffu, R[1] >> 16};
+  rs_step<4, 8>(V, lane & 8);
+  rs_step<2, 16>(V, lane & 16);
+  V[0] = add_xor<32>(V[0]);
+  const int r = 8 * ((lane >> 4) & 1) + 4 * ((lane >> 2) & 1) + 2 * ((lane >> 1) & 1) + (lane & 1);
+  const int f = (lane >> 3) & 1, d = r & 3;
+  *dy = r >> 2;
+  *dx = 4 * (d >> 1) + (d & 1) + 2 * f;
+  return V[0];
+}
+
 __device__ __forceinline__ uint32_t pose_sum16(const BnbParams &P, __amdgpu_buffer_rsrc_t rsrc16, const uint32_t *org,
                                                int32_t nch, int32_t ix, int32_t iy) {
   uint32_t acc = 0u;
@@ -465,11 +649,24 @@
   }
   return wave_sum(acc);
 }
-
-template <bool GLOBAL>
+__device__ __forceinline__ uint32_t pose_sum16_masked(const BnbParams &P, __amdgpu_buffer_rsrc_t rsrc16, const uint32_t *org,
+                                                      uint32_t mask, int32_t ix, int32_t iy) {
+  uint32_t acc = 0u;
+#pragma unroll
+  for (int c = 0; c < OCL; c++) {
+    if (((mask >> c) & 1u) == 0u) continue;
+    const uint32_t o = origin_of(org, c);
+    acc += org_cnt(o) * (uint32_t)__builtin_amdgcn_raw_buffer_load_b16(
+                            rsrc16, (int)t16_tiled(org_row(o) + (uint32_t)iy, org_col(o) + (uint32_t)ix, (uint32_t)P.t16_tpr), 0, 0);
+  }
+  return wave_sum(acc);
+}
+
+template <bool GLOBAL, bool MASKED = false>
 __device__ __forceinline__ uint32_t refine16(const BnbParams &P, __amdgpu_buffer_rsrc_t rsrc16, const uint32_t *org,
                                              int32_t nch, int32_t n_pts, int32_t k, int32_t ix, int32_t iy, uint32_t hsum,
-                                             bool mine, int lane, unsigned long long *best, uint32_t &bcopy) {
+                                             bool mine, int lane, unsigned long long *best, uint32_t &bcopy,
+                                             uint32_t mask = 0u) {
   const bool valid = mine && ix < P.nx && iy < P.ny;
   uint32_t ub = valid ? 256u * hsum + 255u * (uint32_t)n_pts : 0u;
   uint32_t n_eval = 0u;
@@ -478,7 +675,7 @@
     if (top == 0u || top < best_sum_cached<GLOBAL>(best, bcopy)) break;
     const int j = (int)__builtin_ctzll(__ballot(ub == top));
     const int32_t jx = __builtin_amdgcn_readlane(ix, j), jy = __builtin_amdgcn_readlane(iy, j);
-    const uint32_t sum = pose_sum16(P, rsrc16, org, nch, jx, jy);
+    const uint32_t sum = MASKED ? pose_sum16_masked(P, rsrc16, org, mask, jx, jy) : pose_sum16(P, rsrc16, org, nch, jx, jy);
     const uint32_t lin = (uint32_t)((k * P.nx + jx) * P.ny + jy);
     const unsigned long long key = ((unsigned long long)sum << 32) | (0xffffffffu - lin);
     wave_atomic_max(best, key, lane);
diff --git a/nautilus_amd/csrc/nhip_bnb_host.hip b/nautilus_amd/csrc/nhip_bnb_host.hip
--- a/nautilus_amd/csrc/nhip_bnb_host.hip
+++ b/nautilus_amd/csrc/nhip_bnb_host.hip
@@ -75,6 +75,7 @@
   p.levels = is(tunable("NHIP_BNB_LEVELS"), '1') ? 1 : 2;
   p.l2_runs = !is(tunable("NHIP_BNB_L2_RUNS"), '0');
   p.pair_subs = !is(tunable("NHIP_BNB_PAIR_SUBS"), '0');
+  p.zero_chunks = !is(tunable("NHIP_BNB_ZERO_CHUNKS"), '0');
   p.general_all = is(tunable("NHIP_BNB_QUEUE"), '1');
   static_assert(NHIP_SHORT_SCAN_POINTS == 64 * OCL, "the header's promise is the by-rotation form's limit");
   p.short_scans = (search->flags & NHIP_SEARCH_SHORT_SCANS) != 0 && !p.general_all && (uint32_t)(L.S + 2 * L.pad) < ORG_LIMIT;
@@ -158,7 +159,8 @@
 void bnb_last_launch(int32_t out[8]) {
   const BnbPlan &p = t_last_plan;
   const int32_t info[8] = {p.form, (int32_t)p.batch, (int32_t)p.slots, (int32_t)p.rounds, p.short_scans, p.second,
-                           (int32_t)p.instrumented | ((int32_t)p.l2_runs << 1) | ((int32_t)p.pair_subs << 2), p.n_pairs};
+                           (int32_t)p.instrumented | ((int32_t)p.l2_runs << 1) | ((int32_t)p.pair_subs << 2) |
+                               ((int32_t)p.zero_chunks << 3), p.n_pairs};
   memcpy(out, info, sizeof(info));
 }
 
@@ -188,6 +190,7 @@
   P.levels = plan.levels;
   P.l2_runs = plan.l2_runs;
   P.pair_subs = plan.pair_subs;
+  P.zero_chunks = plan.zero_chunks;
   P.general_all = plan.general_all;
   P.short_scans = plan.short_scans;
   P.heavy_min = plan.heavy_min;
@@ -201,8 +204,8 @@
   std::lock_guard<std::mutex> lock(g_instr_mu);
   if (plan.stats) {
     if (!g_bnb_stats) {
-      NHIP_TRY_HIP(hipMalloc(reinterpret_cast<void **>(&g_bnb_stats), 8 * (BNB_STATS_HEAD + (size_t)BNB_STATS_PAIRS)));
-      NHIP_TRY_HIP(hipMemset(g_bnb_stats, 0, 8 * (BNB_STATS_HEAD + (size_t)BNB_STATS_PAIRS)));
+      NHIP_TRY_HIP(hipMalloc(reinterpret_cast<void **>(&g_bnb_stats), 8 * (BNB_STATS_HEAD + (size_t)BNB_STATS_PAIRS + BNB_STATS_CHUNKS)));
+      NHIP_TRY_HIP(hipMemset(g_bnb_stats, 0, 8 * (BNB_STATS_HEAD + (size_t)BNB_STATS_PAIRS + BNB_STATS_CHUNKS)));
     }
     P.stats = g_bnb_stats;
   }
@@ -343,5 +346,13 @@
   return NHIP_OK;
 }
 
-
-}
+int bnb_stats_chunks_read(unsigned long long out[4]) {
+  for (int i = 0; i < BNB_STATS_CHUNKS; i++) out[i] = 0;
+  if (!g_bnb_stats) return NHIP_OK;
+  unsigned long long *at = g_bnb_stats + BNB_STATS_HEAD + (size_t)BNB_STATS_PAIRS;
+  NHIP_TRY_HIP(hipMemcpy(out, at, 8 * BNB_STATS_CHUNKS, hipMemcpyDeviceToHost));
+  NHIP_TRY_HIP(hipMemset(at, 0, 8 * BNB_STATS_CHUNKS));
+  return NHIP_OK;
+}
+
+}
diff --git a/nautilus_amd/csrc/nhip_bnb_origin.h b/nautilus_amd/csrc/nhip_bnb_origin.h
--- a/nautilus_amd/csrc/nhip_bnb_origin.h
+++ b/nautilus_amd/csrc/nhip_bnb_origin.h
@@ -141,7 +141,7 @@
 __device__ __forceinline__ int32_t cache_origins(const BnbParams &P, const float2 *pts, int32_t n_pts, float cf, float sf,
                                                  int32_t cx, int32_t cy, int lane, uint32_t *org, bool merged,
                                                  uint32_t *runs = nullptr, bool want_runs = false,
-                                                 int32_t *run_chunks = nullptr) {
+                                                 int32_t *run_chunks = nullptr, uint8_t *run_span = nullptr) {
   uint32_t *base = org - lane;
   const bool with_runs = RUNS && want_runs;
   if (RUNS) *run_chunks = RUNS_NONE;
@@ -175,6 +175,14 @@
         const uint32_t cnt2 = rest2 ? (uint32_t)__builtin_ctzll(rest2) + 1u : (uint32_t)(64 - lane);
         const uint32_t at = rtail + __builtin_amdgcn_mbcnt_hi((uint32_t)(H2 >> 32), __builtin_amdgcn_mbcnt_lo((uint32_t)H2, 0u));
         if (head2 && at < (uint32_t)RUN_WAVE) runs[at] = (o & RUN_KEY_MASK) | cnt2;
+        if (run_span) {
+          const uint32_t below = __builtin_amdgcn_mbcnt_hi((uint32_t)(H >> 32), __builtin_amdgcn_mbcnt_lo((uint32_t)H, 0u));
+          const uint32_t first = tail - (uint32_t)__builtin_popcountll(H) + below;
+          const uint32_t end = (uint32_t)lane + cnt2;
+          const unsigned long long upto = end >= 64u ? H : H & ((1ull << end) - 1ull);
+          const uint32_t last = first + (uint32_t)__builtin_popcountll(upto) - below - 1u;
+          if (head2 && at < (uint32_t)RUN_WAVE) run_span[at] = (uint8_t)((first >> 6) | ((last >> 6) != (first >> 6) ? 32u : 0u));
+        }
         rtail += (uint32_t)__builtin_popcountll(H2);
       }
     };
diff --git a/nautilus_amd/csrc/nhip_bnb_params.h b/nautilus_amd/csrc/nhip_bnb_params.h
--- a/nautilus_amd/csrc/nhip_bnb_params.h
+++ b/nautilus_amd/csrc/nhip_bnb_params.h
@@ -19,6 +19,7 @@
 constexpr uint32_t ORG_LIMIT = 1u << 13;
 constexpr int RUN_CHUNKS = 8;
 constexpr int RUN_WAVE = RUN_CHUNKS * 64;
+constexpr int RUN_NOTE_BYTES = RUN_WAVE * 3;
 
 constexpr int QSPACE_SPLIT = (SPLIT_WAVES * LIST_ENTRIES * 4 + MAX_ROT * 12 + 15) / 16 * 2;
 constexpr int lds_qspace(bool split) { return split ? QSPACE_SPLIT : QCAP; }
@@ -37,6 +38,7 @@
 
 constexpr int BNB_STATS_PAIRS = 1 << 20;
 constexpr int BNB_STATS_HEAD = 24;
+constexpr int BNB_STATS_CHUNKS = 4;
 
 struct RotEntry {
   unsigned long long w[4];
@@ -93,6 +95,7 @@
   ScoreGate gate;
   int32_t l2_runs;
   int32_t pair_subs;
+  int32_t zero_chunks;
 };
 
 using BnbLaunch = int (*)(const BnbParams &P, const BnbPlan &plan, hipStream_t s);
diff --git a/nautilus_amd/csrc/nhip_bnb_wave.h b/nautilus_amd/csrc/nhip_bnb_wave.h
--- a/nautilus_amd/csrc/nhip_bnb_wave.h
+++ b/nautilus_amd/csrc/nhip_bnb_wave.h
@@ -121,6 +121,16 @@
   const auto s32 = __builtin_amdgcn_permlane32_swap(v, v, false, false);
   return max(s32[0], s32[1]);
 }
+__device__ __forceinline__ uint32_t wave_or(uint32_t v) {
+  v |= (uint32_t)__builtin_amdgcn_update_dpp(0, (int)v, 0xB1, 0xF, 0xF, false);
+  v |= (uint32_t)__builtin_amdgcn_update_dpp(0, (int)v, 0x4E, 0xF, 0xF, false);
+  v |= (uint32_t)__builtin_amdgcn_update_dpp(0, (int)v, 0x124, 0xF, 0xF, false);
+  v |= (uint32_t)__builtin_amdgcn_update_dpp(0, (int)v, 0x128, 0xF, 0xF, false);
+  const auto s16 = __builtin_amdgcn_permlane16_swap(v, v, false, false);
+  v = s16[0] | s16[1];
+  const auto s32 = __builtin_amdgcn_permlane32_swap(v, v, false, false);
+  return (uint32_t)__builtin_amdgcn_readfirstlane((int)(s32[0] | s32[1]));
+}
 template <int CTRL>
 __device__ __forceinline__ unsigned long long max_dpp_u64(unsigned long long v) {
   const uint32_t lo = (uint32_t)__builtin_amdgcn_update_dpp(0, (int)(uint32_t)v, CTRL, 0xF, 0xF, false);
diff --git a/nautilus_amd/csrc/nhip_common.h b/nautilus_amd/csrc/nhip_common.h
--- a/nautilus_amd/csrc/nhip_common.h
+++ b/nautilus_amd/csrc/nhip_common.h
@@ -172,6 +172,7 @@
   bool second, general_all, short_scans, pool_lds, instrumented, stats, timeline;
   bool l2_runs;
   bool pair_subs;
+  bool zero_chunks;
   bool sized_split;
   uint32_t rot_cap, heavy_min, keep_ranks, split_min, split_max;
   int64_t batch, slots, slot_bytes, rounds;
@@ -209,6 +210,7 @@
 void bnb_last_launch(int32_t out[8]);
 bool bnb_fits(const GridLayout &L, const nhip_search_t *search);
 int bnb_stats_read(unsigned long long out[24]);
+int bnb_stats_chunks_read(unsigned long long out[4]);
 int bnb_timeline_read(unsigned long long *out, int32_t n);
 int bnb_timeline_cand_read(unsigned long long *out, int32_t n);
 int bnb_stats_per_pair(unsigned long long *out, int32_t n);
diff --git a/nautilus_amd/csrc/nhip_host_csm.hip b/nautilus_amd/csrc/nhip_host_csm.hip
--- a/nautilus_amd/csrc/nhip_host_csm.hip
+++ b/nautilus_amd/csrc/nhip_host_csm.hip
@@ -601,4 +601,13 @@
   return NHIP_OK;
 }
 
-}
+int nhip_bnb_stats_chunks(uint64_t out[4]) {
+  NHIP_REQUIRE(out != nullptr, "bnb_stats_chunks: null out");
+  unsigned long long v[4];
+  int rc = bnb_stats_chunks_read(v);
+  if (rc) return rc;
+  for (int i = 0; i < 4; i++) out[i] = v[i];
+  return NHIP_OK;
+}
+
+}
```

Result: faster. 1.935 million, median of 6 (+6.4%).
